# fhausmann/deepgrp

Measured on AMD Instinct MI355X. Metric: Mbp/sec predicted (whole node) at window=200 stride=50, 5-class, higher is better.
Workload: dtype f16

## Files before the change

deepgrp_amd/_lib.py:

```python
from __future__ import annotations

import ctypes as C
import os

_HERE = os.path.dirname(os.path.abspath(__file__))
LIB_PATH = os.path.join(_HERE, "libdeepgrp_hip.so")

i64, i32, vp, cint = C.c_int64, C.c_int32, C.c_void_p, C.c_int


class DgrpError(RuntimeError):
    """A libdeepgrp_hip call failed (message from dgrp_last_error())."""


class Segment(C.Structure):
    _fields_ = [("start", C.c_int64), ("end", C.c_int64), ("label", C.c_int32), ("contig", C.c_int32)]


class TrainJob(C.Structure):
    _fields_ = [("T", cint), ("u", cint), ("C", cint), ("attention", cint), ("d_params", vp), ("d_idx", vp), ("d_truth", vp),
                ("n", i64), ("d_starts", vp), ("B", i64), ("d_masks", vp), ("d_loss", vp), ("d_grads", vp), ("d_work", vp),
                ("work_bytes", i64)]


class InflateStreamStats(C.Structure):
    _fields_ = [(k, C.c_int64) for k in ("spans", "candidates", "repaired", "rounds", "longest_span", "false_starts", "chunks", "reserved")]

    def as_dict(self):
        return {k: int(getattr(self, k)) for k, _ in self._fields_ if k != "reserved"}


TRAIN_MAX_JOBS = 8

_SIGNATURES = {
    "dgrp_abi_version": (cint, []),
    "dgrp_last_error": (C.c_char_p, []),
    "dgrp_device_info": (cint, [C.c_char_p, C.c_size_t, C.POINTER(cint), C.POINTER(i64)]),
    "dgrp_strip_n": (cint, [vp, i64, C.POINTER(i64), C.POINTER(i64)]),
    "dgrp_encode": (cint, [vp, i64, vp, vp]),
    "dgrp_onehot": (cint, [vp, i64, vp, vp]),
    "dgrp_fasta_workspace_bytes": (i64, [i64]),
    "dgrp_fasta_encode": (cint, [vp, i64, vp, C.POINTER(i64), vp, i64, vp]),
    "dgrp_fasta_batch_workspace_bytes": (i64, [i64, i64]),
    "dgrp_fasta_encode_batch": (cint, [vp, i64, vp, vp, vp, vp, vp, i64, vp]),
    "dgrp_fasta_chunks_workspace_bytes": (i64, [i64]),
    "dgrp_fasta_chunks": (cint, [vp, i64, i64, vp, vp, C.POINTER(i64), vp, i64, vp]),
    "dgrp_fasta_mask_workspace_bytes": (i64, [i64, i64, i64]),
    "dgrp_fasta_mask_batch": (cint, [vp, i64, vp, vp, vp, vp, cint, C.c_uint64, vp, vp, i64, vp]),
    "dgrp_fasta_extract_workspace_bytes": (i64, [i64, i64, i64]),
    "dgrp_fasta_extract_batch": (cint, [vp, i64, vp, vp, vp, vp, vp, vp, i64, cint, C.c_uint64, vp, i64, C.POINTER(i64), vp, C.POINTER(i64),
                                        vp, i64, vp]),
    "dgrp_repeat_summary_workspace_bytes": (i64, [i64, i64, i64]),
    "dgrp_repeat_summary_batch": (cint, [vp, i64, vp, vp, vp, vp, cint, i64, vp, vp, vp, vp, vp, i64, vp]),
    "dgrp_twobit_workspace_bytes": (i64, [i64]),
    "dgrp_twobit_encode_batch": (cint, [vp, i64, i64, vp, vp, vp, vp, i64, vp, vp, i64, vp, i64, vp]),
    "dgrp_twobit_text_batch": (cint, [vp, i64, i64, vp, vp, vp, vp, vp, vp, i64, vp, vp, i64, vp, vp, i64, vp, i64, vp]),
    "dgrp_twobit_pack_workspace_bytes": (i64, [i64, i64]),
    "dgrp_twobit_pack_batch": (cint, [vp, i64, vp, vp, vp, i64, i64, vp, vp, vp, i64, vp]),
    "dgrp_format_rows_bound": (i64, [i64, i64]),
    "dgrp_format_rows": (cint, [vp, vp, i64, cint, vp, i64, vp, i64, C.POINTER(i64)]),
    "dgrp_track_workspace_bytes": (i64, [i64, i64]),
    "dgrp_track_text": (cint, [vp, i64, cint, cint, cint, i64, i64, C.c_char_p, i64, vp, i64, C.POINTER(i64), vp, i64, vp]),
    "dgrp_track_batch_workspace_bytes": (i64, [i64, vp, vp, i64, cint, i64]),
    "dgrp_track_text_batch": (cint, [vp, cint, i64, vp, vp, vp, C.c_char_p, vp, vp, cint, cint, i64, vp, i64, vp, vp, i64, vp]),
    "dgrp_track_index_workspace_bytes": (i64, [i64, vp, vp, i64, cint, i64]),
    "dgrp_track_index_batch": (cint, [vp, cint, i64, vp, vp, vp, C.c_char_p, vp, vp, cint, cint, i64, vp, i64, vp, vp, i64, vp, i64, vp]),
    "dgrp_track_sections_workspace_bytes": (i64, [i64, vp, vp, i64, cint]),
    "dgrp_track_sections_batch": (cint, [vp, cint, i64, vp, vp, vp, vp, cint, cint, i64, i64, vp, i64, vp, vp, i64, vp, vp, i64, vp]),
    "dgrp_track_zoom_workspace_bytes": (i64, [i64, vp, vp, i64, cint]),
    "dgrp_track_zoom_batch": (cint, [vp, cint, i64, vp, vp, vp, vp, cint, cint, i64, i64, vp, i64, vp, vp, i64, vp, vp, vp, i64, vp]),
    "dgrp_zlib_bound": (i64, [i64, i64]),
    "dgrp_zlib_workspace_bytes": (i64, [i64, cint]),
    "dgrp_zlib_compress_batch": (cint, [vp, i64, vp, i64, i64, cint, vp, i64, vp, C.POINTER(i64), vp, i64, vp]),
    "dgrp_zlib_compress_host": (cint, [vp, i64, vp, i64, i64, cint, vp, i64, vp, C.POINTER(i64)]),
    "dgrp_window_count":(i64, [i64, i64, i64]),
    "dgrp_windows_onehot": (cint, [vp, i64, i64, i64, i64, i64, cint, vp, vp]),
    "dgrp_model_create": (cint, [C.POINTER(vp), cint, cint, cint, cint, vp, vp, vp, vp, vp, vp]),
    "dgrp_model_create_lstm": (cint, [C.POINTER(vp), cint, cint, cint, vp, vp, vp, vp, vp]),
    "dgrp_model_destroy": (cint, [vp]),
    "dgrp_model_dims": (cint, [vp, C.POINTER(cint), C.POINTER(cint), C.POINTER(cint), C.POINTER(cint)]),
    "dgrp_model_flags": (cint, [vp]),
    "dgrp_model_set_precision": (cint, [vp, cint]),
    "dgrp_model_view": (cint, [vp, cint, C.POINTER(vp)]),
    "dgrp_model_plan": (cint, [vp, cint, i64, C.POINTER(cint), C.POINTER(i64), C.POINTER(cint), C.POINTER(cint)]),
    "dgrp_forward_workspace_bytes": (i64, [vp, i64]),
    "dgrp_forward_window_chunk": (i64, [vp]),
    "dgrp_forward_windows": (cint, [vp, vp, i64, i64, i64, i64, vp, vp, i64, vp]),
    "dgrp_forward_merge": (cint, [vp, vp, i64, i64, i64, i64, i64, vp, vp, i64, vp]),
    "dgrp_forward_merge_record": (cint, [vp, vp, i64, i64, i64, vp, vp, i64, vp]),
    "dgrp_forward_merge_record_workspace_bytes": (i64, [vp, i64, i64]),
    "dgrp_forward_reference_workspace_bytes": (i64, [vp, i64]),
    "dgrp_forward_windows_reference": (cint, [vp, vp, i64, i64, i64, i64, vp, vp, i64, vp]),
    "dgrp_get_max": (cint, [vp, i64, vp, i64, i64, i64, i64, vp]),
    "dgrp_scores": (cint, [vp, i64, cint, vp, vp, vp]),
    "dgrp_softmax_labels": (cint, [vp, i64, cint, vp, vp, vp, i64, vp]),
    "dgrp_mss_workspace_bytes": (i64, [i64]),
    "dgrp_mss_labels": (cint, [vp, vp, i64, cint, cint, cint, vp, vp, vp, i64, vp]),
    "dgrp_mss_segments_host": (cint, [vp, i64, vp, i64, C.POINTER(i64)]),
    "dgrp_mss_batch_workspace_bytes": (i64, [i64, i64]),
    "dgrp_mss_labels_batch": (cint, [vp, vp, i64, i64, vp, cint, cint, cint, vp, vp, i64, vp]),
    "dgrp_segments_workspace_bytes": (i64, [i64]),
    "dgrp_segments": (cint, [vp, i64, i64, i32, vp, i64, vp, vp, i64, vp]),
    "dgrp_record_workspace_bytes": (i64, [vp, i64, i64, cint]),
    "dgrp_predict_record": (cint, [vp, vp, i64, i64, i64, cint, cint, cint, i64, i32, vp, i64, C.POINTER(i64), vp, i64, vp]),
    "dgrp_batch_workspace_bytes": (i64, [vp, i64, vp, i64]),
    "dgrp_predict_batch": (cint, [vp, vp, i64, vp, vp, vp, vp, i64, i64, cint, cint, vp, i64, C.POINTER(i64), vp, i64, vp]),
    "dgrp_batch_rows": (i64, [i64, vp]),
    "dgrp_predict_batch_probs": (cint, [vp, vp, i64, vp, vp, vp, vp, i64, i64, cint, cint, vp, i64, C.POINTER(i64), vp, i64, vp, vp]),
    "dgrp_confusion_matrix": (cint, [vp, vp, i64, cint, vp, vp, vp]),
    "dgrp_filter_segments": (cint, [vp, vp, i64, i64, vp]),
    "dgrp_eval_workspace_bytes": (i64, [i64, i64]),
    "dgrp_paint_rows_batch": (cint, [vp, i64, vp, vp, vp, vp, vp, vp, i64, vp]),
    "dgrp_row_hits_batch": (cint, [vp, i64, vp, vp, vp, vp, vp, vp, vp, i64, vp]),
    "dgrp_row_scores_workspace_bytes": (i64, [i64, i64]),
    "dgrp_row_scores_batch": (cint, [vp, cint, i64, vp, vp, vp, vp, vp, vp, vp, i64, vp]),
    "dgrp_prob_hist_workspace_bytes": (i64, [i64, cint, cint]),
    "dgrp_prob_hist_batch": (cint, [vp, cint, i64, vp, vp, vp, vp, cint, vp, vp, vp, i64, vp]),
    "dgrp_row_detect_workspace_bytes": (i64, [i64, i64]),
    "dgrp_paint_row_keys_batch": (cint, [vp, i64, vp, vp, vp, vp, vp, vp, vp, i64, vp]),
    "dgrp_row_detect_batch": (cint, [vp, i64, vp, vp, vp, vp, vp, vp, vp, vp, i64, vp]),
    "dgrp_format_bed_bound": (i64, [i64, i64]),
    "dgrp_format_bed_rows": (cint, [vp, vp, i64, cint, vp, vp, i64, cint, vp, i64, C.POINTER(i64)]),
    "dgrp_bed_text_workspace_bytes": (i64, [i64, i64, i64]),
    "dgrp_bed_text_batch": (cint, [vp, vp, i64, cint, vp, vp, i64, cint, vp, i64, C.POINTER(i64), vp, i64, vp]),
    "dgrp_bed_index_workspace_bytes": (i64, [i64, i64, i64, i64]),
    "dgrp_bed_index_batch": (cint, [vp, vp, i64, cint, vp, vp, i64, cint, i64, vp, vp, i64, C.POINTER(i64), vp, i64, vp, vp, i64, vp]),
    "dgrp_gff_text_workspace_bytes": (i64, [i64, i64, i64, i64, i64]),
    "dgrp_gff_text_batch": (cint, [vp, vp, i64, cint, vp, vp, i64, vp, vp, i64, cint, i64, vp, i64, C.POINTER(i64), C.POINTER(i64), vp, i64,
                                   vp]),
    "dgrp_gff_index_workspace_bytes": (i64, [i64, i64, i64, i64, i64, i64]),
    "dgrp_gff_index_batch": (cint, [vp, vp, i64, cint, vp, vp, i64, vp, vp, i64, cint, i64, i64, vp, vp, i64, C.POINTER(i64), vp, i64, vp, vp,
                                    i64, vp]),
    "dgrp_bed_blocks_workspace_bytes": (i64, [i64, i64, vp]),
    "dgrp_bed_blocks_batch": (cint, [cint, vp, vp, i64, cint, i64, vp, i64, vp, i64, C.POINTER(i64), vp, i64, C.POINTER(i64), C.POINTER(i64),
                                     vp, i64, vp]),
    "dgrp_bed_zoom_workspace_bytes": (i64, [i64, i64, vp]),
    "dgrp_bed_zoom_batch": (cint, [cint, vp, vp, i64, cint, i64, vp, i64, vp, i64, vp, vp, i64, vp, vp, vp, i64, vp]),
    "dgrp_inflate_raw_host": (cint, [vp, i64, vp, i64, C.POINTER(i64), C.POINTER(i64), C.POINTER(cint)]),
    "dgrp_inflate_workspace_bytes": (i64, [i64]),
    "dgrp_inflate_batch": (cint, [vp, i64, i64, vp, vp, vp, vp, i64, C.POINTER(i64), C.POINTER(cint), vp, i64, vp]),
    "dgrp_inflate_stream_host": (cint, [vp, i64, i64, i64, cint, vp, i64, C.POINTER(i64), C.POINTER(i64), vp, C.POINTER(cint)]),
    "dgrp_inflate_stream_workspace_bytes": (i64, [i64, i64]),
    "dgrp_inflate_stream_scan": (cint, [vp, i64, i64, i64, i64, cint, C.POINTER(i64), vp, C.POINTER(cint), vp, i64, vp]),
    "dgrp_inflate_stream_write": (cint, [vp, i64, i64, i64, vp, vp, i64, C.POINTER(C.c_uint32), C.POINTER(i64), C.POINTER(cint), vp, i64,
                                         vp]),
    "dgrp_bgzf_bound": (i64, [i64, cint]),
    "dgrp_bgzf_workspace_bytes": (i64, [i64]),
    "dgrp_bgzf_compress": (cint, [vp, i64, vp, i64, C.POINTER(i64), cint, vp, i64, vp]),
    "dgrp_bgzf_compress_host": (cint, [vp, i64, vp, i64, C.POINTER(i64), cint]),
    "dgrp_bgzf_workspace_bytes_level": (i64, [i64, cint]),
    "dgrp_bgzf_compress_level": (cint, [vp, i64, vp, i64, C.POINTER(i64), cint, cint, vp, i64, vp]),
    "dgrp_bgzf_compress_host_level": (cint, [vp, i64, vp, i64, C.POINTER(i64), cint, cint]),
    "dgrp_train_param_count": (i64, [cint, cint, cint]),
    "dgrp_train_workspace_bytes": (i64, [cint, cint, cint, cint, i64]),
    "dgrp_train_step": (cint, [cint, cint, cint, cint, vp, vp, vp, i64, vp, i64, vp, vp, vp, vp, i64, vp]),
    "dgrp_train_step_multi": (cint, [C.POINTER(TrainJob), cint, vp]),
    "dgrp_optimizer_step": (cint, [cint, vp, vp, vp, vp, i64, C.c_double, C.c_double, C.c_double, C.c_double, i64, vp]),
    "dgrp_truth_workspace_bytes": (i64, [i64, i64]),
    "dgrp_truth_multihot_batch": (cint, [vp, cint, i64, i64, vp, vp, vp, vp, vp, vp, i64, vp]),
    "dgrp_class_starts_workspace_bytes": (i64, [i64, i64]),
    "dgrp_class_window_starts": (cint, [vp, i64, i64, vp, vp, cint, vp, i64, C.POINTER(i64), vp, i64, vp]),
    "dgrp_train_resolve_starts": (cint, [vp, i64, vp, vp, cint, vp, vp, i64, vp, vp]),
    "dgrp_rm_parse_workspace_bytes": (i64, [i64]),
    "dgrp_rm_parse": (cint, [vp, i64, vp, vp, cint, vp, cint, vp, vp, vp, vp, vp, vp, vp, i64, vp, vp, i64, vp]),
    "dgrp_rm_parse_fields": (cint, [vp, i64, vp, vp, cint, vp, cint, vp, vp, vp, vp, vp, vp, vp, vp, i64, vp, vp, i64, vp]),
    "dgrp_paint_strata_batch": (cint, [vp, i64, vp, vp, vp, vp, vp, vp, vp, i64, vp]),
    "dgrp_prob_hist_strata_workspace_bytes": (i64, [i64]),
    "dgrp_prob_hist_strata_batch": (cint, [vp, cint, i64, vp, vp, vp, vp, cint, cint, vp, vp, vp, i64, vp]),
    "dgrp_rm_parse_all_workspace_bytes": (i64, [i64]),
    "dgrp_rm_parse_all": (cint, [vp, i64, vp, vp, cint, vp, cint, vp, vp, vp, vp, vp, vp, vp, vp, vp, vp, vp, vp, i64, vp, vp, i64, vp]),
    "dgrp_rows_parse_workspace_bytes": (i64, [i64]),
    "dgrp_rows_parse": (cint, [vp, i64, cint, vp, vp, vp, vp, vp, vp, vp, vp, vp, i64, vp, vp, i64, vp]),
    "dgrp_token_ids_workspace_bytes": (i64, [i64, i64]),
    "dgrp_token_ids": (cint, [vp, i64, i64, vp, vp, vp, vp, vp, vp, i64, vp, vp, vp, i64, vp]),
    "dgrp_paint_keys_batch": (cint, [vp, i64, vp, vp, vp, vp, vp, vp, vp, i64, vp]),
    "dgrp_key_crosstab_batch": (cint, [vp, vp, i64, cint, i64, vp, vp, vp]),
    "dgrp_row_key_classes_batch": (cint, [vp, i64, vp, vp, vp, vp, vp, vp, vp, i64, vp]),
    "dgrp_row_bounds_workspace_bytes": (i64, [i64, i64]),
    "dgrp_row_bounds_batch": (cint, [vp, i64, vp, vp, vp, vp, vp, cint, vp, vp, i64, vp]),
    "dgrp_bound_hist_workspace_bytes": (i64, [i64]),
    "dgrp_bound_hist_batch": (cint, [i64, vp, vp, vp, vp, vp, vp, vp, cint, cint, vp, vp, vp, vp, vp, i64, vp]),
    "dgrp_kernel_timer_enable": (cint, [cint]),
    "dgrp_kernel_timer_read": (cint, [C.POINTER(C.c_double), C.POINTER(i64), C.POINTER(i64)]),
}

_lib = None


def lib() -> C.CDLL:
    global _lib
    if _lib is None:
        if not os.path.exists(LIB_PATH):
            raise ImportError(
                f"{LIB_PATH} is missing: build it with `make -C deepgrp_amd/csrc` (hipcc, gfx950) "
                "or `python -c 'import __graft_entry__ as g; g.build()'`. There is no CPU fallback.")
        import torch
        L = C.CDLL(LIB_PATH)
        for name, (res, args) in _SIGNATURES.items():
            f = getattr(L, name)
            f.restype = res
            f.argtypes = args
        if L.dgrp_abi_version() != 1:
            raise ImportError("libdeepgrp_hip.so ABI version mismatch")
        _lib = L
    return _lib


def check(rc: int, what: str = "") -> None:
    if rc != 0:
        msg = lib().dgrp_last_error().decode("utf-8", "replace")
        raise DgrpError(f"{what or 'libdeepgrp_hip'} failed (code {rc}): {msg}")


def name_blob(names):
    import numpy as np
    raw = [nm if isinstance(nm, bytes) else nm.encode("utf-8", "surrogateescape") for nm in names]
    off = np.zeros(len(raw) + 1, np.int64)
    np.cumsum([len(x) for x in raw], out=off[1:])
    return raw, b"".join(raw), off


def exported_symbols():
    return sorted(_SIGNATURES)
```

deepgrp_amd/csrc/api.hip:

```cpp
#include "dgrp_model.h"

#include <stdarg.h>
#include <string.h>

#include <algorithm>
#include <vector>
#include <mutex>

static thread_local char g_err[512] = "";

void dgrp_set_error(const char *fmt, ...)
{
    va_list ap;
    va_start(ap, fmt);
    vsnprintf(g_err, sizeof(g_err), fmt, ap);
    va_end(ap);
}

DGRP_EXPORT int dgrp_abi_version(void) { return DGRP_ABI_VERSION; }
DGRP_EXPORT const char *dgrp_last_error(void) { return g_err; }

DGRP_EXPORT int dgrp_device_info(char *name, size_t name_cap, int *cu_count, int64_t *hbm_bytes)
{
    int dev = 0;
// ... 504 lines not shown

DGRP_EXPORT int dgrp_model_destroy(dgrp_model *m)
{
    if (!m) return DGRP_OK;
    if (m->is_view) { delete m; return DGRP_OK; }
    if (m->d_pack) (void)hipFree(m->d_pack);
    if (m->d_ffb) (void)hipFree(m->d_ffb);
    if (m->d_scale) (void)hipFree(m->d_scale);
    if (m->d_wtop) (void)hipFree(m->d_wtop);
    if (m->d_raw) (void)hipFree(m->d_raw);
    if (m->d_pack_lo) (void)hipFree(m->d_pack_lo);
    if (m->d_pack16) (void)hipFree(m->d_pack16);
    if (m->d_xtab) (void)hipFree(m->d_xtab);
    if (m->d_stream) (void)hipFree(m->d_stream);
    if (m->d_packw) (void)hipFree(m->d_packw);
    if (m->d_xtabw) (void)hipFree(m->d_xtabw);
    delete m;
    return DGRP_OK;
}

DGRP_EXPORT int dgrp_model_dims(const dgrp_model *m, int *T, int *u, int *C, int *attention)
{
    DGRP_REQUIRE(m, "dgrp_model_dims: NULL model");
    if (T) *T = m->T;
    if (u) *u = m->u;
    if (C) *C = m->C;
    if (attention) *attention = m->attention;
    return DGRP_OK;
}

DGRP_EXPORT int dgrp_model_flags(const dgrp_model *m)
{
    DGRP_REQUIRE(m, "dgrp_model_flags: NULL model");
    return (m->onercp ? 1 : 0) | (m->precision == 1 ? 2 : 0) | (m->ref_only ? 4 : 0);
}

static_assert((int)dgrp_kernel::none == DGRP_KERNEL_NONE && (int)dgrp_kernel::wave == DGRP_KERNEL_WAVE &&
              (int)dgrp_kernel::split2 == DGRP_KERNEL_SPLIT2 && (int)dgrp_kernel::stream64 == DGRP_KERNEL_STREAM64 &&
              (int)dgrp_kernel::stream == DGRP_KERNEL_STREAM && (int)dgrp_kernel::split == DGRP_KERNEL_SPLIT &&
              (int)dgrp_kernel::lstm == DGRP_KERNEL_LSTM && (int)dgrp_kernel::fused == DGRP_KERNEL_FUSED,
              "DGRP_KERNEL_* (deepgrp_hip.h) follow dgrp_kernel (dgrp_model.h)");

DGRP_EXPORT int dgrp_model_plan(const dgrp_model *m, int mode, int64_t step, int *kernel, int64_t *lds_bytes, int *ospan, int *avg_up)
{
    DGRP_REQUIRE(m, "dgrp_model_plan: NULL model");
    DGRP_REQUIRE(kernel && lds_bytes && ospan && avg_up, "dgrp_model_plan: NULL output pointer");
    DGRP_REQUIRE(mode >= 0 && mode <= 2, "dgrp_model_plan: mode %d (0 merged, 1 window probabilities, 2 attention pre-pass)", mode);
    DGRP_REQUIRE(step >= 1, "dgrp_model_plan: step %lld < 1", (long long)step);
    DGRP_REQUIRE(mode != 2 || m->attention, "dgrp_model_plan: mode 2 on a model without attention");
    if (m->ref_only) {
        *kernel = DGRP_KERNEL_FP32; *lds_bytes = 0; *ospan = 0; *avg_up = 0;
        return DGRP_OK;
    }
    const dgrp_gru_plan plan = dgrp_gru_plan_for(m, mode, step);
    *kernel = (int)plan.kernel; *lds_bytes = (int64_t)plan.lds; *ospan = plan.ospan; *avg_up = plan.avg_up;
    return DGRP_OK;
}

DGRP_EXPORT int dgrp_model_set_precision(dgrp_model *m, int level)
{
    DGRP_REQUIRE(m, "dgrp_model_set_precision: NULL model");
    DGRP_REQUIRE(level == 0 || level == 1, "dgrp_model_set_precision: level must be 0 (fp16 operands) or 1 (split operands)");
    if (m->ref_only) return DGRP_OK;
    DGRP_REQUIRE(level == 0 || m->d_pack_lo || m->d_stream, "dgrp_model_set_precision: this model has no split-operand kernel");
    m->precision = level;
    return DGRP_OK;
}

static int64_t ref_sub_windows(const dgrp_model *m)
{
    const int64_t per = 2 * (int64_t)m->T * m->u * 4 + (int64_t)m->T * (m->C + 1) * 4 + 2 * (int64_t)m->u * 4;
    return std::max<int64_t>(16, std::min<int64_t>(4096, (512ll << 20) / per) / 16 * 16);
}

DGRP_EXPORT int64_t dgrp_forward_workspace_bytes(const dgrp_model *m, int64_t nw)
{
    if (!m || nw < 0) return 0;
    if (m->ref_only) {
        const int64_t sub = std::min<int64_t>(ref_sub_windows(m), std::max<int64_t>(nw, 1));
        return dgrp_align_up(dgrp_forward_reference_workspace_bytes(m, sub), 256) + dgrp_align_up(sub * m->T * (int64_t)m->C * 4, 256);
    }
    if (!m->attention) return 256;
    return dgrp_align_up(nw * m->T * (int64_t)m->UP * 4, 256) + dgrp_align_up(nw * m->T * (int64_t)m->C * 4, 256) + 256;
}

static unsigned *forward_queue(const dgrp_model *m, int64_t nw, void *d_work, int64_t work_bytes)
{
    if (!d_work || work_bytes < dgrp_forward_workspace_bytes(m, nw)) return nullptr;
    return (unsigned *)((char *)d_work + (m->attention ? dgrp_forward_workspace_bytes(m, nw) - 256 : 0));
}

static int forward_ref(const dgrp_model *m, const uint8_t *d_idx, int64_t n, int64_t s, dgrp_placement place, int64_t w0, int64_t nw,
                       int merge, float *d_out, void *d_work, int64_t work_bytes, hipStream_t stream)
{
    if (work_bytes < dgrp_forward_workspace_bytes(m, nw) || !d_work) {
        dgrp_set_error("dgrp_forward: this model runs on the fp32 kernels and needs %lld bytes of workspace for %lld windows",
                       (long long)dgrp_forward_workspace_bytes(m, nw), (long long)nw);
        return DGRP_ENOMEM;
    }
    const int64_t sub = std::min<int64_t>(ref_sub_windows(m), nw);
    const int64_t ref_bytes = dgrp_align_up(dgrp_forward_reference_workspace_bytes(m, sub), 256);
    float *probs = (float *)((char *)d_work + ref_bytes);
    for (int64_t a = w0; a < w0 + nw; a += sub) {
        const int64_t k = std::min<int64_t>(sub, w0 + nw - a);
        float *dst = merge ? probs : d_out + (a - w0) * (int64_t)m->T * m->C;
        int rc = dgrp_forward_windows_reference(m, d_idx, n, s, a, k, dst, d_work, ref_bytes, stream);
        if (rc) return rc;
        if (!merge) continue;
        for (int64_t b = a; b < a + k;) {
            const int64_t e = (b < place.nfullB && a + k > place.nfullB) ? place.nfullB : a + k;
            const int64_t row = dgrp_place_row(place, b, s);
            if (row < n) {
                rc = dgrp_get_max(d_out + row * m->C, n - row, probs + (b - a) * (int64_t)m->T * m->C, m->T, m->C, s, e - b, stream);
                if (rc) return rc;
            }
            b = e;
        }
    }
    return DGRP_OK;
}

static int forward_common(const dgrp_model *m, const uint8_t *d_idx, int64_t n, int64_t s, int64_t batch, int64_t w0,
                          int64_t nw, int merge, float *d_out, void *d_work, int64_t work_bytes, hipStream_t stream)
{
    DGRP_REQUIRE(m && s >= 1 && w0 >= 0 && nw >= 0 && n >= 0, "dgrp_forward: bad arguments");
    if (nw == 0) return DGRP_OK;
    DGRP_REQUIRE(d_idx && d_out, "dgrp_forward: NULL pointer");
    DGRP_REQUIRE((w0 + nw - 1) * s + m->T <= n, "dgrp_forward: window %lld (start %lld) runs past n=%lld",
                 (long long)(w0 + nw - 1), (long long)((w0 + nw - 1) * s), (long long)n);
    dgrp_placement place = { 0, 0 };
    if (merge) {
        DGRP_REQUIRE(batch >= 1, "dgrp_forward_merge: batch must be >= 1");
        const int64_t total = dgrp_window_count(n, m->T, s);
        DGRP_REQUIRE(w0 + nw <= total, "dgrp_forward_merge: windows %lld..%lld exceed the record's %lld",
                     (long long)w0, (long long)(w0 + nw), (long long)total);
        place = dgrp_make_placement(total, batch);
    }
    if (m->ref_only) return forward_ref(m, d_idx, n, s, place, w0, nw, merge, d_out, d_work, work_bytes, stream);
    if (!m->attention)
        return dgrp_gru_launch(m, dgrp_gru_plan_for(m, merge ? 0 : 1, s), d_idx, n, place, w0, nw, d_out, nullptr,
                               forward_queue(m, nw, d_work, work_bytes), stream);
    if (work_bytes < dgrp_forward_workspace_bytes(m, nw) || !d_work) {
        dgrp_set_error("dgrp_forward: attention model needs %lld bytes of workspace for %lld windows",
                       (long long)dgrp_forward_workspace_bytes(m, nw), (long long)nw);
        return DGRP_ENOMEM;
    }
    void *avg = d_work;
    float *pl = (float *)((char *)d_work + dgrp_align_up(nw * m->T * (int64_t)m->UP * 4, 256));
    const dgrp_gru_plan pre = dgrp_gru_plan_for(m, 2, s);
    int rc = dgrp_gru_launch(m, pre, d_idx, n, place, w0, nw, pl, avg, forward_queue(m, nw, d_work, work_bytes), stream);
    if (rc) return rc;
    return dgrp_attention_launch_recs(m, pre, place, w0, nw, merge, n, avg, pl, d_out, nullptr, 0, stream);
}

DGRP_EXPORT int dgrp_forward_windows(const dgrp_model *m, const uint8_t *d_idx, int64_t n, int64_t s, int64_t w0,
                                     int64_t nw, float *d_probs, void *d_work, int64_t work_bytes, void *stream)
{
    return forward_common(m, d_idx, n, s, 1, w0, nw, 0, d_probs, d_work, work_bytes, (hipStream_t)stream);
}

DGRP_EXPORT int dgrp_forward_merge(const dgrp_model *m, const uint8_t *d_idx, int64_t n, int64_t s, int64_t batch,
                                   int64_t w0, int64_t nw, float *d_out, void *d_work, int64_t work_bytes, void *stream)
{
    return forward_common(m, d_idx, n, s, batch, w0, nw, 1, d_out, d_work, work_bytes, (hipStream_t)stream);
}

static int64_t spill_cap_bytes()
{
    static const int64_t cap = [] {
        if (const char *e = getenv("DGRP_SPILL_BYTES")) {
            const long long v = atoll(e);
            if (v >= (1ll << 20)) return (int64_t)v;
        }
        size_t free_b = 0, total_b = 0;
        if (hipMemGetInfo(&free_b, &total_b) != hipSuccess || total_b == 0) return (int64_t)(4ll << 30);
        return std::min<int64_t>(8ll << 30, std::max<int64_t>(1ll << 30, (int64_t)(total_b / 32)));
    }();
    return cap;
}

static int64_t record_window_chunk(const dgrp_model *m)
{
    if (m->ref_only) return ref_sub_windows(m);
    if (!m->attention) return 1ll << 23;
    const int64_t per = (int64_t)m->T * ((int64_t)m->UP * 4 + (int64_t)m->C * 4);
    int64_t c = spill_cap_bytes() / per;
    c = c >= 32768 ? c / 32768 * 32768 : c >= 4096 ? c / 4096 * 4096 : c / 16 * 16;
    if (c < 16) c = 16;
    return c < (1ll << 20) ? c : (1ll << 20);
}

DGRP_EXPORT int64_t dgrp_forward_window_chunk(const dgrp_model *m)
{
    return m ? record_window_chunk(m) : 0;
}

#define DGRP_LANES 3
static int64_t lane_window_chunk(const dgrp_model *m)
{
    if (m->ref_only || !m->attention) return 0;
    if (const char *e = getenv("DGRP_LANE_CHUNK")) {
        const long long v = atoll(e);
        return v >= 16 ? (int64_t)(v / 16 * 16) : 0;
    }
    const int64_t c = record_window_chunk(m);
    if (c < 65536) return 0;
    const int64_t lc = c / DGRP_LANES / 32768 * 32768;
    return lc >= 32768 ? lc : 32768;
}
struct lane_pool { hipStream_t s[DGRP_LANES]; int dev; bool ok; };
static lane_pool *lanes_get()
{
    static std::mutex mu;
    static std::vector<lane_pool *> pools;
    int dev = 0;
    if (hipGetDevice(&dev) != hipSuccess) return nullptr;
    std::lock_guard<std::mutex> lock(mu);
    for (lane_pool *q : pools)
        if (q->dev == dev) return q->ok ? q : nullptr;
    lane_pool *q = new lane_pool();
    q->dev = dev; q->ok = true;
    for (int i = 0; i < DGRP_LANES; ++i)
        if (hipStreamCreateWithFlags(&q->s[i], hipStreamNonBlocking) != hipSuccess) q->ok = false;
    pools.push_back(q);
    return q->ok ? q : nullptr;
}

static int64_t record_forward_bytes(const dgrp_model *m, int64_t nwin)
{
    const int64_t lc = lane_window_chunk(m);
    if (lc > 0 && nwin > lc)
        return DGRP_LANES * dgrp_align_up(std::max<int64_t>(dgrp_forward_workspace_bytes(m, std::min(lc, nwin)), 256), 256);
    const int64_t chunk = std::min<int64_t>(record_window_chunk(m), nwin > 0 ? nwin : 1);
    return std::max<int64_t>(dgrp_forward_workspace_bytes(m, chunk), 256);
}

DGRP_EXPORT int64_t dgrp_forward_merge_record_workspace_bytes(const dgrp_model *m, int64_t n, int64_t s)
{
    if (!m || n < 0 || s < 1) return 0;
    return record_forward_bytes(m, dgrp_window_count(n, m->T, s));
}

DGRP_EXPORT int dgrp_forward_merge_record(const dgrp_model *m, const uint8_t *d_idx, int64_t n, int64_t s, int64_t batch, float *d_out,
                                          void *d_work, int64_t work_bytes, void *stream_)
{
    hipStream_t stream = (hipStream_t)stream_;
    DGRP_REQUIRE(m && n >= 0 && s >= 1 && batch >= 1, "dgrp_forward_merge_record: bad arguments");
    const int64_t nwin = dgrp_window_count(n, m->T, s);
    if (nwin == 0) return DGRP_OK;
    DGRP_REQUIRE(d_idx && d_out && d_work, "dgrp_forward_merge_record: NULL pointer");
    const int64_t need = record_forward_bytes(m, nwin);
    if (work_bytes < need) {
        dgrp_set_error("dgrp_forward_merge_record: workspace %lld < %lld bytes", (long long)work_bytes, (long long)need);
        return DGRP_ENOMEM;
    }
    const int64_t lc = lane_window_chunk(m);
    lane_pool *lp = lc > 0 && nwin > lc ? lanes_get() : nullptr;
    if (!lp) {
        const int64_t chunk = lc > 0 && nwin > lc ? lc : record_window_chunk(m);
        for (int64_t w0 = 0; w0 < nwin; w0 += chunk) {
            const int64_t nw = std::min<int64_t>(chunk, nwin - w0);
            const int rc = dgrp_forward_merge(m, d_idx, n, s, batch, w0, nw, d_out, d_work, work_bytes, stream);
            if (rc) return rc;
        }
        return DGRP_OK;
    }
    const int64_t per = need / DGRP_LANES;
    hipEvent_t fork = nullptr, join[DGRP_LANES] = { nullptr, nullptr, nullptr };
    int rc = DGRP_OK;
    auto bail = [&](hipError_t e) { if (e != hipSuccess && rc == DGRP_OK) { dgrp_set_error("dgrp_forward_merge_record: %s", hipGetErrorString(e)); rc = DGRP_EHIP; } };
    bail(hipEventCreateWithFlags(&fork, hipEventDisableTiming));
    for (int i = 0; i < DGRP_LANES; ++i) bail(hipEventCreateWithFlags(&join[i], hipEventDisableTiming));
    if (rc == DGRP_OK) {
        bail(hipEventRecord(fork, stream));
        for (int i = 0; i < DGRP_LANES; ++i) bail(hipStreamWaitEvent(lp->s[i], fork, 0));
        int64_t k = 0;
        for (int64_t w0 = 0; w0 < nwin && rc == DGRP_OK; w0 += lc, ++k) {
            const int64_t nw = std::min<int64_t>(lc, nwin - w0);
            const int lane = (int)(k % DGRP_LANES);
            rc = dgrp_forward_merge(m, d_idx, n, s, batch, w0, nw, d_out, (char *)d_work + lane * per, per, lp->s[lane]);
        }
        for (int i = 0; i < DGRP_LANES; ++i) {
            bail(hipEventRecord(join[i], lp->s[i]));
            bail(hipStreamWaitEvent(stream, join[i], 0));
        }
    }
    if (fork) (void)hipEventDestroy(fork);
    for (int i = 0; i < DGRP_LANES; ++i)
        if (join[i]) (void)hipEventDestroy(join[i]);
    return rc;
}

struct record_layout {
    int64_t out, scores, cls, labels, count, fwd, post, bytes, post_bytes, fwd_bytes;
};

static record_layout record_carve(const dgrp_model *m, int64_t n, int64_t s, int use_mss)
{
    record_layout l;
    int64_t p = 0;
    auto take = [&](int64_t b) { const int64_t q = p; p += dgrp_align_up(b, 256); return q; };
    const int64_t nwin = dgrp_window_count(n, m->T, s);
    l.out = take(n * m->C * 4);
    l.scores = take(use_mss ? n * 8 : 0);
    l.cls = take(use_mss ? n : 0);
    l.labels = take(n);
    l.count = take(8);
    l.fwd_bytes = record_forward_bytes(m, nwin);
    l.fwd = take(l.fwd_bytes);
    l.post_bytes = std::max<int64_t>(std::max<int64_t>(use_mss ? dgrp_mss_workspace_bytes(n) : 4096, dgrp_segments_workspace_bytes(n)), 4096);
    l.post = take(l.post_bytes);
    l.bytes = p;
    return l;
}

DGRP_EXPORT int64_t dgrp_record_workspace_bytes(const dgrp_model *m, int64_t n, int64_t s, int use_mss)
{
    if (!m || n < 0 || s < 1) return 0;
    return record_carve(m, n, s, use_mss).bytes;
}

DGRP_EXPORT int dgrp_predict_record(const dgrp_model *m, const uint8_t *d_idx, int64_t n, int64_t s, int64_t batch,
                                    int min_mss_len, int xdrop_len, int use_mss, int64_t offset, int32_t contig,
                                    dgrp_segment *d_records, int64_t cap, int64_t *h_count, void *d_work,
                                    int64_t work_bytes, void *stream_)
{
    hipStream_t stream = (hipStream_t)stream_;
    DGRP_REQUIRE(m && n >= 0 && s >= 1 && batch >= 1 && cap >= 0 && h_count, "dgrp_predict_record: bad arguments");
    *h_count = 0;
    if (n == 0) return DGRP_OK;
    DGRP_REQUIRE(d_idx && d_work && (cap == 0 || d_records), "dgrp_predict_record: NULL pointer");
    const record_layout l = record_carve(m, n, s, use_mss);
    if (work_bytes < l.bytes) {
        dgrp_set_error("dgrp_predict_record: workspace %lld < %lld bytes", (long long)work_bytes, (long long)l.bytes);
        return DGRP_ENOMEM;
    }
    char *w = (char *)d_work;
    float *out = (float *)(w + l.out);
    int8_t *labels = (int8_t *)(w + l.labels);
    int64_t *d_count = (int64_t *)(w + l.count);
    DGRP_HIP(hipMemsetAsync(out, 0, (size_t)n * m->C * 4, stream));
    int rc = dgrp_forward_merge_record(m, d_idx, n, s, batch, out, w + l.fwd, l.fwd_bytes, stream);
    if (rc) return rc;
    if (use_mss) {
        rc = dgrp_scores(out, n, m->C, (double *)(w + l.scores), (int8_t *)(w + l.cls), stream);
        if (rc) return rc;
        rc = dgrp_mss_labels((const double *)(w + l.scores), (const int8_t *)(w + l.cls), n, m->C, min_mss_len, xdrop_len,
                             labels, nullptr, w + l.post, l.post_bytes, stream);
    } else {
        rc = dgrp_softmax_labels(out, n, m->C, nullptr, labels, w + l.post, l.post_bytes, stream);
    }
    if (rc) return rc;
    rc = dgrp_segments(labels, n, offset, contig, d_records, cap, d_count, w + l.post, l.post_bytes, stream);
    if (rc) return rc;
    DGRP_HIP(hipMemcpyAsync(h_count, d_count, 8, hipMemcpyDeviceToHost, stream));
    DGRP_HIP(hipStreamSynchronize(stream));
    return DGRP_OK;
}

int dgrp_batch_marks(const int64_t *d_start, const int64_t *d_len, int64_t nrec, int64_t total_n, uint8_t *d_marks,
                     double *d_scores, int8_t *d_cls, hipStream_t stream);
int dgrp_batch_segments(const int8_t *d_labels, const uint8_t *d_marks, int64_t total_n, const int64_t *d_start, int64_t nrec,
                        const int64_t *d_startpos, const int32_t *d_contig, dgrp_segment *d_records, int64_t cap,
                        int64_t *d_count, void *d_work, int64_t work_bytes, hipStream_t stream);

struct batch_layout {
    int64_t out, scores, cls, labels, marks, count, recs, wgf, start, len, spos, contig, post, post_bytes, avg, pl, queue, bytes;
};

static batch_layout batch_carve(const dgrp_model *m, int64_t nrec, int64_t total_rows, int64_t total_windows)
{
    batch_layout l;
    int64_t p = 0;
    auto take = [&](int64_t b) { const int64_t q = p; p += dgrp_align_up(b, 256); return q; };
    l.out = take(total_rows * m->C * 4);
    l.scores = take(total_rows * 8);
    l.cls = take(total_rows);
    l.labels = take(total_rows);
    l.marks = take(total_rows);
    l.count = take(8);
    l.recs = take(nrec * 64);
    l.wgf = take((nrec + 1) * 8);
    l.start = take((nrec + 1) * 8);
    l.len = take(nrec * 8);
    l.spos = take(nrec * 8);
    l.contig = take(nrec * 4);
    l.post_bytes = std::max<int64_t>(std::max<int64_t>(dgrp_mss_batch_workspace_bytes(total_rows, nrec), dgrp_segments_workspace_bytes(total_rows)), 4096);
    l.post = take(l.post_bytes);
    l.avg = take(m->attention ? total_windows * m->T * (int64_t)m->UP * 4 : 0);
    l.pl = take(m->attention ? total_windows * m->T * (int64_t)m->C * 4 : 0);
    l.queue = take(4);
    l.bytes = p;
    return l;
}

static int64_t batch_windows(const dgrp_model *m, int64_t nrec, const int64_t *h_n, int64_t s)
{
    int64_t w = 0;
    for (int64_t r = 0; r < nrec; ++r) w += dgrp_window_count(h_n[r], m->T, s);
    return w;
}

static int64_t batch_rows(int64_t nrec, const int64_t *h_n)
{
    int64_t rows = 0;
    for (int64_t r = 0; r < nrec; ++r) rows += dgrp_align_up(h_n[r], 64);
    return rows;
}

DGRP_EXPORT int64_t dgrp_batch_workspace_bytes(const dgrp_model *m, int64_t nrec, const int64_t *h_n, int64_t s)
{
    if (!m || nrec < 0 || s < 1 || (nrec > 0 && !h_n)) return 0;
    for (int64_t r = 0; r < nrec; ++r)
        if (h_n[r] < 1) return 0;
    return batch_carve(m, nrec, batch_rows(nrec, h_n), batch_windows(m, nrec, h_n, s)).bytes;
}

DGRP_EXPORT int64_t dgrp_batch_rows(int64_t nrec, const int64_t *h_n)
{
    return nrec > 0 && h_n ? batch_rows(nrec, h_n) : 0;
}

static int predict_batch_common(const char *who, const dgrp_model *m, const uint8_t *d_idx, int64_t nrec, const int64_t *h_idx_off,
                                const int64_t *h_n, const int64_t *h_startpos, const int32_t *h_contig, int64_t s,
                                int64_t batch, int min_mss_len, int xdrop_len, dgrp_segment *d_records, int64_t cap,
                                int64_t *h_count, void *d_work, int64_t work_bytes, hipStream_t stream, float *d_probs)
{
    DGRP_REQUIRE(m && nrec >= 0 && s >= 1 && batch >= 1 && cap >= 0 && h_count, "%s: bad arguments", who);
    *h_count = 0;
    if (nrec == 0) return DGRP_OK;
    DGRP_REQUIRE(!m->ref_only && (m->cell == 0 || (m->cell == 1 && m->NW <= 8)), "%s: unsupported model (fp32 path: record by record)", who);
    DGRP_REQUIRE(d_idx && h_idx_off && h_n && h_startpos && h_contig && d_work && (cap == 0 || d_records), "%s: NULL pointer", who);
    for (int64_t r = 0; r < nrec; ++r)
        DGRP_REQUIRE(h_n[r] >= 1 && h_idx_off[r] >= 0, "%s: record %lld: empty records do not belong in a batch", who, (long long)r);
    const int64_t rows = batch_rows(nrec, h_n);
    DGRP_REQUIRE(rows < (1ll << 31), "%s: %lld rows in one batch (limit 2^31)", who, (long long)rows);
    const int64_t windows = batch_windows(m, nrec, h_n, s);
    DGRP_REQUIRE(windows < (1ll << 31), "%s: too many windows in one batch", who);
    const batch_layout l = batch_carve(m, nrec, rows, windows);
    if (work_bytes < l.bytes) {
        dgrp_set_error("%s: workspace %lld < %lld bytes", who, (long long)work_bytes, (long long)l.bytes);
        return DGRP_ENOMEM;
    }
    char *w = (char *)d_work;
    std::vector<int64_t> recs((size_t)nrec * 8, 0), wgf((size_t)nrec + 1, 0), start((size_t)nrec + 1, 0);
    int64_t wfirst = 0;
    for (int64_t r = 0; r < nrec; ++r) {
        const int64_t nwin = dgrp_window_count(h_n[r], m->T, s);
        const dgrp_placement pl = dgrp_make_placement(nwin, batch);
        int64_t *e = recs.data() + (size_t)r * 8;
        e[0] = h_idx_off[r]; e[1] = h_n[r]; e[2] = start[(size_t)r]; e[3] = nwin; e[4] = pl.nfullB; e[5] = pl.shift; e[6] = wfirst;
        wfirst += nwin;
        wgf[(size_t)r + 1] = wgf[(size_t)r] + (nwin + 15) / 16;
        start[(size_t)r + 1] = start[(size_t)r] + dgrp_align_up(h_n[r], 64);
    }
    DGRP_HIP(hipMemcpyAsync(w + l.recs, recs.data(), recs.size() * 8, hipMemcpyHostToDevice, stream));
    DGRP_HIP(hipMemcpyAsync(w + l.wgf, wgf.data(), wgf.size() * 8, hipMemcpyHostToDevice, stream));
    DGRP_HIP(hipMemcpyAsync(w + l.start, start.data(), start.size() * 8, hipMemcpyHostToDevice, stream));
    DGRP_HIP(hipMemcpyAsync(w + l.len, h_n, (size_t)nrec * 8, hipMemcpyHostToDevice, stream));
    DGRP_HIP(hipMemcpyAsync(w + l.spos, h_startpos, (size_t)nrec * 8, hipMemcpyHostToDevice, stream));
    DGRP_HIP(hipMemcpyAsync(w + l.contig, h_contig, (size_t)nrec * 4, hipMemcpyHostToDevice, stream));
    float *out = d_probs ? d_probs : (float *)(w + l.out);
    DGRP_HIP(hipMemsetAsync(out, 0, (size_t)rows * m->C * 4, stream));
    int rc;
    if (!m->attention) {
        rc = dgrp_gru_launch_batch(m, dgrp_gru_plan_for(m, 0, s), d_idx, w + l.recs, (const int64_t *)(w + l.wgf), nrec, wgf[(size_t)nrec],
                                   out, nullptr, (unsigned *)(w + l.queue), stream);
        if (rc) return rc;
    } else {
        const dgrp_gru_plan pre = dgrp_gru_plan_for(m, 2, s);
        rc = dgrp_gru_launch_batch(m, pre, d_idx, w + l.recs, (const int64_t *)(w + l.wgf), nrec, wgf[(size_t)nrec], (float *)(w + l.pl),
                                   w + l.avg, (unsigned *)(w + l.queue), stream);
        if (rc) return rc;
        rc = dgrp_attention_launch_recs(m, pre, dgrp_placement{ 0, 0 }, 0, windows, 1, rows, w + l.avg, (const float *)(w + l.pl), out,
                                        w + l.recs, nrec, stream);
        if (rc) return rc;
    }
    double *scores = (double *)(w + l.scores);
    int8_t *cls = (int8_t *)(w + l.cls), *labels = (int8_t *)(w + l.labels);
    uint8_t *marks = (uint8_t *)(w + l.marks);
    rc = dgrp_scores(out, rows, m->C, scores, cls, stream);
    if (rc) return rc;
    rc = dgrp_batch_marks((const int64_t *)(w + l.start), (const int64_t *)(w + l.len), nrec, rows, marks, scores, cls, stream);
    if (rc) return rc;
    rc = dgrp_mss_labels_batch(scores, cls, rows, nrec, start.data(), m->C, min_mss_len, xdrop_len, labels, w + l.post, l.post_bytes, stream);
    if (rc) return rc;
    int64_t *d_count = (int64_t *)(w + l.count);
    rc = dgrp_batch_segments(labels, marks, rows, (const int64_t *)(w + l.start), nrec, (const int64_t *)(w + l.spos),
                             (const int32_t *)(w + l.contig), d_records, cap, d_count, w + l.post, l.post_bytes, stream);
    if (rc) return rc;
    DGRP_HIP(hipMemcpyAsync(h_count, d_count, 8, hipMemcpyDeviceToHost, stream));
    DGRP_HIP(hipStreamSynchronize(stream));
    return DGRP_OK;
}

DGRP_EXPORT int dgrp_predict_batch(const dgrp_model *m, const uint8_t *d_idx, int64_t nrec, const int64_t *h_idx_off,
                                   const int64_t *h_n, const int64_t *h_startpos, const int32_t *h_contig, int64_t s,
                                   int64_t batch, int min_mss_len, int xdrop_len, dgrp_segment *d_records, int64_t cap,
                                   int64_t *h_count, void *d_work, int64_t work_bytes, void *stream)
{
    return predict_batch_common("dgrp_predict_batch", m, d_idx, nrec, h_idx_off, h_n, h_startpos, h_contig, s, batch, min_mss_len, xdrop_len,
                                d_records, cap, h_count, d_work, work_bytes, (hipStream_t)stream, nullptr);
}

DGRP_EXPORT int dgrp_predict_batch_probs(const dgrp_model *m, const uint8_t *d_idx, int64_t nrec, const int64_t *h_idx_off,
                                         const int64_t *h_n, const int64_t *h_startpos, const int32_t *h_contig, int64_t s,
                                         int64_t batch, int min_mss_len, int xdrop_len, dgrp_segment *d_records, int64_t cap,
                                         int64_t *h_count, void *d_work, int64_t work_bytes, void *stream, float *d_probs)
{
    DGRP_REQUIRE(d_probs || nrec <= 0, "dgrp_predict_batch_probs: NULL d_probs");
    return predict_batch_common("dgrp_predict_batch_probs", m, d_idx, nrec, h_idx_off, h_n, h_startpos, h_contig, s, batch, min_mss_len,
                                xdrop_len, d_records, cap, h_count, d_work, work_bytes, (hipStream_t)stream, d_probs);
}
```

deepgrp_amd/csrc/mss_kernels.hip:

```cpp
#include "dgrp_common.h"
#include "scan.h"
#include <vector>
#include <math.h>

struct mss_cand { int32_t st, en; double L, R; int32_t pre, pad; };

#define MSS_SUB_MIN 256
#define MSS_SUBENT_BYTES 80
struct mss_subent {
    int64_t start, run;
    double L, peak, run_L;
    int64_t run_st;
    int32_t open, first;
    int32_t vci, nst;
    int32_t reset, pad;
    double Lf;
};
static_assert(sizeof(mss_subent) == 80, "MSS_SUBENT_BYTES");
#define MSS_LCAP 160
#define MSS_NEG (-1e30)
#define MSS_QNONE (-4096)
#define MSS_QBAD 4096

enum mss_grand {
    MSS_G_TOTAL = 0,
    MSS_G_CHANGED = 1,
    MSS_G_ERROR = 2,
    MSS_G_NSEG = 3,
    MSS_G_WHY = 4,
    MSS_G_PIECES = 5,
    MSS_G_LUNITS = 6,
    MSS_G_SPEC = 7,
    MSS_G_NLONG = MSS_G_TOTAL
};

struct mss_stats {
    const double *blk_sum, *blk_abs; const int32_t *blk_q; const uint8_t *flags;
    const double *sup_sum, *sup_abs; const int32_t *sup_q; const uint8_t *sup_flags;
};

struct mss_layout {
    int64_t nblk;
    uint64_t *blk;
    double *blk_sum;
    double *blk_abs;
    int32_t *blk_q;
    uint8_t *flags;
    int64_t nsup;
    double *sup_sum, *sup_abs;
    int32_t *sup_q;
    uint8_t *sup_flags;
    uint64_t *tiles;
    uint64_t *grand;
    int64_t *ustart;
    int64_t *urun;
    double *exitL[2];
    uint64_t *segcnt;
    uint64_t *cutcnt;
    uint64_t *lblk;
    int64_t *lstart, *lrun;
    uint8_t *lforced;
    void *lstate[2];
    int64_t *cut_st, *cut_run;
    double *cut_L;
    int2 *cut_kj;
    int64_t *ustart2, *urun2;
    double *entry2;
    void *subs;
    int64_t dump_cap;
    mss_cand *dump;
    mss_cand *stack;
    int32_t *segs;
    int32_t *segs_out;
    int64_t bytes;
};

static mss_layout mss_carve(void *work, int64_t n)
{
    mss_layout l;
    unsigned char *p = (unsigned char *)work;
    auto take = [&](int64_t bytes) { unsigned char *q = p; p += dgrp_align_up(bytes, 256); return q; };
    l.nblk = (n + 63) / 64;
    const int64_t maxunits = l.nblk + 1, maxruns = n / 2 + 2;
    l.blk = (uint64_t *)take((l.nblk + 1) * 8);
    l.blk_sum = (double *)take(l.nblk * 8);
    l.blk_abs = (double *)take(l.nblk * 8);
    l.blk_q = (int32_t *)take(l.nblk * 4);
    l.flags = (uint8_t *)take(l.nblk + 64);
    l.nsup = (l.nblk + 63) / 64;
    l.sup_sum = (double *)take(l.nsup * 8);
    l.sup_abs = (double *)take(l.nsup * 8);
    l.sup_q = (int32_t *)take(l.nsup * 4);
    l.sup_flags = (uint8_t *)take(l.nsup + 64);
    l.tiles = (uint64_t *)take(((maxunits + 1 + SCAN_TILE - 1) / SCAN_TILE + 1) * 8);
    l.grand = (uint64_t *)take(64);
    l.ustart = (int64_t *)take((maxunits + 1) * 8);
    l.urun = (int64_t *)take((maxunits + 1) * 8);
    l.exitL[0] = (double *)take(maxunits * 8);
    l.exitL[1] = (double *)take(maxunits * 8);
    l.segcnt = (uint64_t *)take((maxunits + 1) * 8);
    l.cutcnt = (uint64_t *)take((maxunits + 1) * 8);
    l.lblk = (uint64_t *)take((l.nblk + 1) * 8);
    l.lstart = (int64_t *)take((maxunits + 1) * 8);
    l.lrun = (int64_t *)take((maxunits + 1) * 8);
    l.lforced = (uint8_t *)take(maxunits + 64);
    l.lstate[0] = take(maxunits * 64);
    l.lstate[1] = take(maxunits * 64);
    l.cut_st = (int64_t *)take(l.nblk * 8);
    l.cut_run = (int64_t *)take(l.nblk * 8);
    l.cut_L = (double *)take(l.nblk * 8);
    l.cut_kj = (int2 *)take(l.nblk * 8);
    l.ustart2 = (int64_t *)take((2 * maxunits + 2) * 8);
    l.urun2 = (int64_t *)take((2 * maxunits + 2) * 8);
    l.entry2 = (double *)take((2 * maxunits + 2) * 8);
    l.subs = take((maxunits + 8) * (int64_t)MSS_SUBENT_BYTES);
    l.dump_cap = 2 * (l.nblk / MSS_SUB_MIN + 2);
    l.dump = (mss_cand *)take(l.dump_cap * MSS_LCAP * (int64_t)sizeof(mss_cand));
    l.stack = (mss_cand *)take(maxruns * (int64_t)sizeof(mss_cand));
    l.segs = (int32_t *)take(maxruns * 8);
    l.segs_out = (int32_t *)take(maxruns * 8);
    l.bytes = p - (unsigned char *)work;
    return l;
}

DGRP_EXPORT int64_t dgrp_mss_workspace_bytes(int64_t n)
{
    if (n < 0) return 0;
    return mss_carve(nullptr, n).bytes;
}

__device__ __forceinline__ int quantum_exp(double x)
{
    const uint64_t b = (uint64_t)__double_as_longlong(x) & 0x7fffffffffffffffull;
    if (b == 0) return MSS_QNONE;
    const int e = (int)(b >> 52);
    if (e == 0 || e == 0x7ff) return MSS_QBAD;
    const uint64_t m = b & 0x000fffffffffffffull;
    const int tz = m ? __builtin_ctzll(m) : 52;
    return -((e - 1023) - 52 + tz);
}

__device__ __forceinline__ bool mss_certified(double L, double sumabs, int q_scores)
{
    const int qL = quantum_exp(L);
    const int Q = qL > q_scores ? qL : q_scores;
    if (Q >= MSS_QBAD) return false;
    const int ex = 53 - Q;
    if (ex > 1000) return true;
    if (ex < -1000) return false;
    return (fabs(L) + sumabs) * 1.0000001 < ldexp(1.0, ex);
}

__device__ __forceinline__ double wave_sum(double v)
{
#pragma unroll
    for (int o = 32; o > 0; o >>= 1) v += __shfl_xor(v, o);
    return v;
}
__device__ __forceinline__ int wave_max(int v)
{
#pragma unroll
    for (int o = 32; o > 0; o >>= 1) { int w = __shfl_xor(v, o); v = w > v ? w : v; }
    return v;
}

__device__ __forceinline__ double lane_value(double x, int l)
{
    const long long b = __double_as_longlong(x);
    const int lo = __builtin_amdgcn_readlane((int)b, l), hi = __builtin_amdgcn_readlane((int)(b >> 32), l);
    return __longlong_as_double(((long long)hi << 32) | (unsigned int)lo);
}

__global__ void __launch_bounds__(256) mss_blockstat_kernel(const double *__restrict__ S, int64_t n,
                                                            uint64_t *__restrict__ blk, double *__restrict__ blk_sum,
                                                            double *__restrict__ blk_abs, int32_t *__restrict__ blk_q,
                                                            uint8_t *__restrict__ flags)
{
    const int lane = threadIdx.x & 63;
    const int64_t b = (int64_t)blockIdx.x * 4 + (threadIdx.x >> 6);
    if (b * 64 >= n) return;
    const int64_t i = b * 64 + lane;
    const double s = i < n ? S[i] : 0.0;
    const bool pos = i < n && s > 0;
    const bool prevpos = i > 0 && i < n && S[i - 1] > 0;
    const unsigned long long mpos = __ballot(pos);
    const unsigned long long mstart = __ballot(pos && !prevpos);
    const double sum = wave_sum(s), sabs = wave_sum(fabs(s));
    const int q = wave_max(quantum_exp(s));
    if (lane == 0) {
        flags[b] = (uint8_t)(mpos != 0ull ? 1 : 0);
        blk[b] = (uint64_t)__popcll(mstart);
        blk_sum[b] = sum;
        blk_abs[b] = sabs;
        blk_q[b] = q;
    }
}

__global__ void __launch_bounds__(256) mss_superstat_kernel(const double *__restrict__ blk_sum, const double *__restrict__ blk_abs,
                                                            const int32_t *__restrict__ blk_q, const uint8_t *__restrict__ flags,
                                                            int64_t nblk, double *__restrict__ sup_sum, double *__restrict__ sup_abs,
                                                            int32_t *__restrict__ sup_q, uint8_t *__restrict__ sup_flags)
{
    const int lane = threadIdx.x & 63;
    const int64_t g = (int64_t)blockIdx.x * 4 + (threadIdx.x >> 6);
    if (g * 64 >= nblk) return;
    const int64_t b = g * 64 + lane;
    const bool in = b < nblk;
    const unsigned long long mp = __ballot(in && (flags[b] & 1));
    const double sum = wave_sum(in ? blk_sum[b] : 0.0), sabs = wave_sum(in ? blk_abs[b] : 0.0);
    const int q = wave_max(in ? blk_q[b] : MSS_QNONE);
    if (lane == 0) {
        sup_flags[g] = (uint8_t)(mp != 0ull ? 1 : 0);
        sup_sum[g] = sum;
        sup_abs[g] = sabs;
        sup_q[g] = q;
    }
}

__device__ __forceinline__ bool mss_is_boundary(const uint8_t *flags, const double *blk_sum, int64_t b, int64_t nblk,
                                                int64_t n, double thr)
{
    if (!(thr > 0.0) || b + 1 >= nblk || (flags[b] & 1) || !(flags[b + 1] & 1)) return false;
    if (b * 64 + 64 > n) return false;
    double cum = 0.0;
    for (int64_t j = b; j >= 0 && j > b - 16; --j) {
        if (flags[j] & 1) break;
        cum += blk_sum[j];
        if (cum < -thr) return true;
    }
    return false;
}

__global__ void __launch_bounds__(256) mss_boundary_kernel(const uint8_t *__restrict__ flags, const double *__restrict__ blk_sum,
                                                           int64_t nblk, int64_t n, double thr, uint64_t *__restrict__ blk)
{
    const int64_t b = (int64_t)blockIdx.x * blockDim.x + threadIdx.x;
    if (b >= nblk) return;
    if (mss_is_boundary(flags, blk_sum, b, nblk, n, thr)) blk[b] |= 1ull << 32;
}

__global__ void __launch_bounds__(256) mss_units_kernel(const uint64_t *__restrict__ blk, const uint8_t *__restrict__ flags,
                                                        const double *__restrict__ blk_sum, int64_t nblk, int64_t n, double thr,
                                                        int64_t *__restrict__ ustart, int64_t *__restrict__ urun,
                                                        const uint64_t *__restrict__ grand)
{
    const int64_t b = (int64_t)blockIdx.x * blockDim.x + threadIdx.x;
    if (b == 0) {
        ustart[0] = 0;
        urun[0] = 0;
        const int64_t nunits = (int64_t)(grand[MSS_G_TOTAL] >> 32) + 1;
        ustart[nunits] = n;
        urun[nunits] = (int64_t)(grand[MSS_G_TOTAL] & 0xffffffffull);
    }
    if (b >= nblk) return;
    if (mss_is_boundary(flags, blk_sum, b, nblk, n, thr)) {
        const int64_t k = (int64_t)(blk[b] >> 32) + 1;
        ustart[k] = (b + 1) * 64;
        urun[k] = (int64_t)(blk[b] & 0xffffffffull);
    }
}

template <int CTRL, int RMASK>
__device__ __forceinline__ int dpp_i(int src, int old) { return __builtin_amdgcn_update_dpp(old, src, CTRL, RMASK, 0xf, false); }
template <int CTRL, int RMASK>
__device__ __forceinline__ double dpp_d(double src, double old)
{
    const long long s = __double_as_longlong(src), o = __double_as_longlong(old);
    const int lo = __builtin_amdgcn_update_dpp((int)o, (int)s, CTRL, RMASK, 0xf, false);
    const int hi = __builtin_amdgcn_update_dpp((int)(o >> 32), (int)(s >> 32), CTRL, RMASK, 0xf, false);
    return __longlong_as_double(((long long)hi << 32) | (unsigned int)lo);
}
#define DPP_SHR(n) (0x110 + (n))
#define DPP_BCAST15 0x142
#define DPP_BCAST31 0x143
#define DPP_WAVE_SHR1 0x138
#define DPP_SCAN_STEPS(STEP) STEP(DPP_SHR(1), 0xf) STEP(DPP_SHR(2), 0xf) STEP(DPP_SHR(4), 0xf) STEP(DPP_SHR(8), 0xf) STEP(DPP_BCAST15, 0xa) STEP(DPP_BCAST31, 0xc)
__device__ __forceinline__ double scan_add_d(double x)
{
#define STEP(c, m) x = x + dpp_d<c, m>(x, 0.0);
    DPP_SCAN_STEPS(STEP)
#undef STEP
    return x;
}
__device__ __forceinline__ double scan_min_d(double x)
{
#define STEP(c, m) { const double y = dpp_d<c, m>(x, INFINITY); x = y < x ? y : x; }
    DPP_SCAN_STEPS(STEP)
#undef STEP
    return x;
}
__device__ __forceinline__ int scan_max_i(int x)
{
#define STEP(c, m) { const int y = dpp_i<c, m>(x, -1); x = y > x ? y : x; }
    DPP_SCAN_STEPS(STEP)
#undef STEP
    return x;
}
__device__ __forceinline__ void scan_segmax_d(int &fl, double &v)
{
#define STEP(c, m) { const double yv = dpp_d<c, m>(v, -INFINITY); const int yf = dpp_i<c, m>(fl, 0); if (!fl) v = yv > v ? yv : v; fl |= yf; }
    DPP_SCAN_STEPS(STEP)
#undef STEP
}
__device__ __forceinline__ double lane_below_d(double x, double first) { return dpp_d<DPP_WAVE_SHR1, 0xf>(x, first); }
__device__ __forceinline__ int lane_below_i(int x, int first) { return dpp_i<DPP_WAVE_SHR1, 0xf>(x, first); }
__device__ __forceinline__ int lane_value_i(int x, int l) { return __builtin_amdgcn_readlane(x, l); }

__device__ __forceinline__ double mss_fold(double s, double a0, int t, int nvalid, int lane)
{
    const double sm = lane >= t && lane < nvalid ? s : 0.0;
    double X = a0;
    for (int j = t; j < nvalid; j += 4) {
        X = lane_below_d(X, a0) + sm;
        X = lane_below_d(X, a0) + sm;
        X = lane_below_d(X, a0) + sm;
        X = lane_below_d(X, a0) + sm;
    }
    return X;
}

__device__ __forceinline__ int64_t mss_skip_blocks(const mss_stats &st, double &cur, int64_t pos, int64_t end, int lane)
{
    if ((pos & 4095) == 0) {
        const int64_t gj = (pos >> 12) + lane;
        const bool stop2 = gj * 4096 + 4096 > end || (st.sup_flags[gj] & 1);
        const unsigned long long ms2 = __ballot(stop2);
        const int m2 = ms2 ? __builtin_ctzll(ms2) : 64;
        if (m2 > 0) {
            const bool in = lane < m2;
            const double gs = wave_sum(in ? st.sup_sum[gj] : 0.0);
            const double ga = wave_sum(in ? st.sup_abs[gj] : 0.0);
            const int gq = wave_max(in ? st.sup_q[gj] : MSS_QNONE);
            if (mss_certified(cur, ga, gq)) { cur += gs; return (int64_t)m2 * 4096; }
        }
    }
    const int64_t b0 = pos >> 6, bend = (end + 63) >> 6;
    const int64_t bj = b0 + lane;
    const bool stop = bj >= bend || (st.flags[bj] & 1) || (bj * 64 + 64 > end) || (lane > 0 && (bj & 63) == 0);
    const unsigned long long mstop = __ballot(stop);
    const int m = mstop ? __builtin_ctzll(mstop) : 64;
    if (m > 0) {
        const bool in = lane < m;
        const double gs = wave_sum(in ? st.blk_sum[bj] : 0.0);
        const double ga = wave_sum(in ? st.blk_abs[bj] : 0.0);
        const int gq = wave_max(in ? st.blk_q[bj] : MSS_QNONE);
        if (mss_certified(cur, ga, gq)) { cur += gs; return (int64_t)m * 64; }
    }
    return 0;
}

__global__ void __launch_bounds__(64) mss_scan_kernel(const double *__restrict__ S, const int64_t *__restrict__ ustart,
                                                      const int64_t *__restrict__ urun, int64_t nunits,
                                                      const double *__restrict__ exit_prev, double *__restrict__ exit_cur,
                                                      mss_cand *stack_all, int32_t *__restrict__ segs_all,
                                                      uint64_t *__restrict__ segcnt, int min_sc, double xdrop,
                                                      uint64_t *__restrict__ grand, int pass,
                                                      const double *__restrict__ blk_sum, const double *__restrict__ blk_abs,
                                                      const int32_t *__restrict__ blk_q, const uint8_t *__restrict__ flags,
                                                      const double *__restrict__ sup_sum, const double *__restrict__ sup_abs,
                                                      const int32_t *__restrict__ sup_q, const uint8_t *__restrict__ sup_flags,
                                                      int independent, int cutmode, mss_subent *subs, mss_cand *dump_all)
{
    const mss_stats stats = { blk_sum, blk_abs, blk_q, flags, sup_sum, sup_abs, sup_q, sup_flags };
    __shared__ double2 sLR[MSS_LCAP];
    __shared__ int4 sIdx[MSS_LCAP];
    const int lane = threadIdx.x;
    const int64_t k = blockIdx.x;
    const bool sub = subs != nullptr;
    const bool head = !sub || subs[k].first != 0;
    const bool tail = !sub || k + 1 == nunits || subs[k + 1].first != 0;
    const int64_t begin = sub ? subs[k].start : ustart[k], end = sub ? subs[k + 1].start : ustart[k + 1];
    const int64_t slot0 = sub ? subs[k].run : urun[k];
    volatile mss_cand *ovf = stack_all + slot0;
    int32_t *segs = segs_all + 2 * slot0;
    int64_t nst = 0, nseg = 0;
    double cur = sub ? subs[k].L : (k == 0 || independent) ? 0.0 : exit_prev[k - 1];
    double peak = sub && !head ? subs[k].peak : MSS_NEG;
    bool run_open = sub && !head && subs[k].open != 0;
    int64_t run_st = run_open ? subs[k].run_st : 0;
    double run_L = run_open ? subs[k].run_L : 0.0;
    bool was_reset = false;
    double Lf = sub && !head ? subs[k].Lf : INFINITY;

    struct cand_v { double L, R; int32_t st, en, pre, open; };
    auto get = [&](int64_t j) -> cand_v {
        cand_v c;
        if (j < MSS_LCAP) {
            const double2 lr = sLR[j];
            const int4 ix = sIdx[j];
            c.L = lr.x; c.R = lr.y; c.st = ix.x; c.en = ix.y; c.pre = ix.z; c.open = ix.w;
        } else {
            volatile mss_cand *o = ovf + (j - MSS_LCAP);
            c.L = o->L; c.R = o->R; c.st = o->st; c.en = o->en; c.pre = o->pre; c.open = o->pad;
        }
        return c;
    };

    auto flush = [&]() {
        for (int64_t base = 0; base < nst; base += 64) {
            const int64_t j = base + lane;
            bool keep = false;
            int32_t a = 0, b = 0;
            if (j < nst) {
                const cand_v c = get(j);
                keep = c.R - c.L >= min_sc;
                a = c.st;
                b = c.en;
            }
            const unsigned long long m = __ballot(keep);
            if (keep) {
                const int64_t slot = nseg + __popcll(m & ((1ull << lane) - 1ull));
                segs[2 * slot] = a;
                segs[2 * slot + 1] = b;
            }
            nseg += __popcll(m);
        }
        nst = 0;
    };

    auto close_run = [&](double R, int64_t en) {
        if (R > peak) peak = R;
        if (!head && run_L <= Lf) { Lf = run_L; peak = R; }
        int32_t tst = (int32_t)run_st;
        double tL = run_L;
        int64_t j;
        for (;;) {
            j = nst - 1;
            cand_v c;
            while (j >= 0) {
                c = get(j);
                if (c.L < tL) break;
                j = c.pre >= 0 ? c.pre : j - 1;
            }
            if (j >= 0 && c.R < R) {
                tst = c.st;
                tL = c.L;
                nst = j;
                continue;
            }
            break;
        }
        const int lopen = j < 0 && !head ? 1 : 0;
        if (j < 0 && head) { flush(); peak = R; }
        if (was_reset && lane == 0) { atomicOr((unsigned long long *)&grand[MSS_G_ERROR], 1ull); atomicOr((unsigned long long *)&grand[MSS_G_WHY], 8ull); }
        if (nst < MSS_LCAP) {
            if (lane == 0) {
                sLR[nst] = make_double2(tL, R);
                sIdx[nst] = make_int4(tst, (int32_t)en, (int32_t)j, lopen);
            }
        } else {
            volatile mss_cand *c = ovf + (nst - MSS_LCAP);
            c->st = tst; c->en = (int32_t)en; c->L = tL; c->R = R; c->pre = (int32_t)j; c->pad = lopen;
        }
        __threadfence_block();
        ++nst;
        run_open = false;
    };
    auto reset_flush = [&]() {
        if (head) flush(); else { was_reset = true; Lf = INFINITY; }
    };

    int64_t pos = begin;
    while (pos < end) {
        const int nvalid = (int)min((int64_t)64, end - pos);
        if (!run_open && peak == MSS_NEG && (pos & 63) == 0) {
            const int64_t adv = mss_skip_blocks(stats, cur, pos, end, lane);
            if (adv) { pos += adv; continue; }
        }
        const double s = lane < nvalid ? S[pos + lane] : 0.0;
        const bool ispos = lane < nvalid && s > 0;
        const unsigned long long vmask = nvalid == 64 ? ~0ull : ((1ull << nvalid) - 1ull);
        const unsigned long long mpos = __ballot(ispos);
        const double sabs = wave_sum(fabs(s));
        const int q = wave_max(quantum_exp(s));
        const bool cert = mss_certified(cur, sabs, q);
        if (cert || (q < MSS_QBAD && quantum_exp(cur) < MSS_QBAD)) {
            double pre = s;
            if (cert) {
#pragma unroll
                for (int o = 1; o < 64; o <<= 1) {
                    const double y = __shfl_up(pre, o);
                    if (lane >= o) pre += y;
                }
            } else {
                pre = mss_fold(s, cur, 0, nvalid, lane);
            }
            double base = cert ? cur : 0.0;
            const double front = cur;
            int p = 0;
            if (nst >= 1 && nst <= MSS_LCAP) {
                const cand_v c0 = get(nst - 1);
                const int64_t nb = c0.pre;
                const bool lone = nst == 1 && !c0.open;
                double lim = INFINITY;
                if (!lone && nb >= 0) lim = get(nb).R;
                if (lone || nb >= 0 || c0.open) {
                const double V = base + pre;
                const bool edge_close = run_open && !(mpos & 1ull);
                const bool isend = ispos && lane + 1 < nvalid && !((mpos >> (lane + 1)) & 1ull);
                const bool isstart = ispos && (lane == 0 ? !run_open : !((mpos >> (lane - 1)) & 1ull));
                double vprev = __shfl_up(V, 1);
                if (lane == 0) vprev = cur;
                double rmax = isend ? V : -INFINITY;
#pragma unroll
                for (int o = 1; o < 64; o <<= 1) {
                    const double y = __shfl_up(rmax, o);
                    if (lane >= o) rmax = y > rmax ? y : rmax;
                }
                double before = __shfl_up(rmax, 1);
                if (lane == 0) before = -INFINITY;
                const double base_r = edge_close ? cur : c0.R;
                const double base_peak = edge_close ? (lone ? cur : (cur > peak ? cur : peak)) : peak;
                const double top_r = before > base_r ? before : base_r;
                const double peak_i = lone ? (before > -INFINITY ? before : base_peak) : (before > base_peak ? before : base_peak);
                bool ok = !run_open || c0.L < run_L;
                if (edge_close) ok = ok && cur > c0.R && !(lim < cur);
                if (isend) ok = ok && V > top_r && !(lim < V);
                if (isstart) ok = ok && (c0.L < vprev);
                if (lane < nvalid && !ispos && xdrop > 0.0 && V + xdrop < peak_i) ok = false;
                if (__all(ok)) {
                    const unsigned long long mend = __ballot(isend);
                    if (mend || edge_close) {
                        const int last = mend ? 63 - __builtin_clzll(mend) : -1;
                        const double newR = mend ? lane_value(V, last) : cur;
                        if (lane == 0) {
                            sLR[nst - 1] = make_double2(c0.L, newR);
                            sIdx[nst - 1] = make_int4(c0.st, (int32_t)(pos + last + 1), (int32_t)nb, c0.open);
                        }
                        __threadfence_block();
                        peak = lone ? newR : (newR > peak ? newR : peak);
                    }
                    if ((mpos >> (nvalid - 1)) & 1ull) {
                        const unsigned long long znon = ~mpos & vmask;
                        if (znon || !run_open) {
                            const int ls = znon ? 64 - __builtin_clzll(znon) : 0;
                            run_st = pos + ls;
                            run_L = ls == 0 ? cur : lane_value(V, ls - 1);
                        }
                        run_open = true;
                    } else {
                        run_open = false;
                    }
                    cur = lane_value(V, nvalid - 1);
                    pos += nvalid;
                    continue;
                }
                }
            }
            while (p < nvalid) {
                const unsigned long long rest = vmask & ~((1ull << p) - 1ull);
                if ((mpos >> p) & 1ull) {
                    const unsigned long long z = ~mpos & rest;
                    const int e = z ? __builtin_ctzll(z) : nvalid;
                    if (!run_open) { run_open = true; run_st = pos + p; run_L = p == 0 ? front : base + lane_value(pre, p - 1); }
                    cur = base + lane_value(pre, e - 1);
                    p = e;
                    if (e < nvalid) close_run(cur, pos + e);
                } else {
                    if (run_open) close_run(cur, pos + p);
                    const unsigned long long z = mpos & rest;
                    const int e = z ? __builtin_ctzll(z) : nvalid;
                    if (xdrop > 0.0 && peak != MSS_NEG) {
                        const bool trig = lane >= p && lane < e && ((base + pre) + xdrop < peak);
                        const unsigned long long mt = __ballot(trig);
                        if (mt) {
                            const int t = __builtin_ctzll(mt);
                            reset_flush();
                            peak = MSS_NEG;
                            if (cert) base = t == 0 ? 0.0 : -lane_value(pre, t - 1);
                            else pre = mss_fold(s, 0.0, t, nvalid, lane);
                        }
                    }
                    cur = base + lane_value(pre, e - 1);
                    p = e;
                }
            }
        } else {
            for (int i = 0; i < nvalid; ++i) {
                const double v = lane_value(s, i);
                if (v > 0) {
                    if (!run_open) { run_open = true; run_st = pos + i; run_L = cur; }
                    cur = cur + v;
                } else {
                    if (run_open) close_run(cur, pos + i);
                    if (xdrop > 0.0 && cur + v + xdrop < peak) { reset_flush(); cur = 0.0; peak = MSS_NEG; }
                    cur += v;
                }
            }
        }
        pos += nvalid;
    }
    if (run_open && tail) close_run(cur, end);
    if (sub && !(head && tail)) {
        const int64_t slot = head ? 2 * (int64_t)subs[k + 1].vci + 1 : 2 * (int64_t)subs[k].vci;
        mss_cand *d = dump_all + slot * MSS_LCAP;
        for (int64_t j = lane; j < nst && j < MSS_LCAP; j += 64) {
            const double2 lr = sLR[j];
            const int4 ix = sIdx[j];
            mss_cand c;
            c.st = ix.x; c.en = ix.y; c.L = lr.x; c.R = lr.y; c.pre = ix.z; c.pad = ix.w;
            d[j] = c;
        }
        if (lane == 0) {
            subs[k].nst = (int32_t)(nst < (1ll << 31) ? nst : -1);
            subs[k].reset = was_reset ? 1 : 0;
        }
    } else if (k == nunits - 1 || independent || cutmode) {
        flush();
    } else if (nst != 0 || peak != MSS_NEG) {
        if (lane == 0) atomicOr((unsigned long long *)&grand[MSS_G_ERROR], 1ull);
    }
    if (lane == 0) {
        segcnt[k] = (uint64_t)nseg;
        const double want = sub ? subs[k + 1].L : exit_prev[k];
        if (!independent && (pass == 0 || __double_as_longlong(want) != __double_as_longlong(cur)))
            atomicOr((unsigned long long *)&grand[MSS_G_CHANGED], 1ull);
        exit_cur[k] = cur;
    }
}

__global__ void __launch_bounds__(64) mss_stitch_kernel(mss_subent *subs, int64_t nunits, mss_cand *stack_all, const mss_cand *dump_all,
                                                        int32_t *__restrict__ segs_all, uint64_t *__restrict__ segcnt, int min_sc,
                                                        uint64_t *__restrict__ grand)
{
    const int lane = threadIdx.x;
    const int64_t k = blockIdx.x;
    if (!subs[k].first || k + 1 >= nunits || subs[k + 1].first) return;
    __shared__ mss_cand loc[256];
    volatile mss_cand *T = stack_all + subs[k].run;
    int64_t nT = subs[k].nst;
    bool bad = nT < 0;
    if (!bad) {
        for (int64_t hi = nT; hi > MSS_LCAP; hi -= 64) {
            const int64_t j = hi - 1 - lane;
            mss_cand c;
            const bool on = j >= MSS_LCAP;
            if (on) { volatile mss_cand *o = T + (j - MSS_LCAP); c.st = o->st; c.en = o->en; c.L = o->L; c.R = o->R; c.pre = o->pre; c.pad = 0; }
            __threadfence_block();
            if (on) { volatile mss_cand *o = T + j; o->st = c.st; o->en = c.en; o->L = c.L; o->R = c.R; o->pre = c.pre; o->pad = 0; }
            __threadfence_block();
        }
        const mss_cand *d = dump_all + (2 * (int64_t)subs[k + 1].vci + 1) * MSS_LCAP;
        for (int64_t j = lane; j < nT && j < MSS_LCAP; j += 64) {
            const mss_cand c = d[j];
            volatile mss_cand *o = T + j; o->st = c.st; o->en = c.en; o->L = c.L; o->R = c.R; o->pre = c.pre; o->pad = 0;
        }
        __threadfence();
    }
    int64_t nseg = (int64_t)segcnt[k];
    int32_t *segs = segs_all + 2 * subs[k].run;
    auto flush_T = [&]() {
        for (int64_t base = 0; base < nT; base += 64) {
            const int64_t j = base + lane;
            bool keep = false;
            int32_t a = 0, b = 0;
            if (j < nT) {
                volatile mss_cand *c = T + j;
                keep = c->R - c->L >= min_sc;
                a = c->st;
                b = c->en;
            }
            const unsigned long long m = __ballot(keep);
            if (keep) {
                const int64_t slot = nseg + __popcll(m & ((1ull << lane) - 1ull));
                segs[2 * slot] = a;
                segs[2 * slot + 1] = b;
            }
            nseg += __popcll(m);
        }
        nT = 0;
    };
    for (int64_t u = k + 1; !bad && u < nunits && !subs[u].first; ++u) {
        const int64_t nl = subs[u].nst;
        if (nl < 0) { bad = true; break; }
        const mss_cand *d = dump_all + 2 * (int64_t)subs[u].vci * MSS_LCAP;
        const mss_cand *deep = stack_all + subs[u].run;
        if (nl > MSS_LCAP && subs[k].run + nT > subs[u].run) { bad = true; break; }
        int64_t w = 0;
        auto load_chunk = [&]() {
            const int64_t j = w + lane;
            if (j < nl) loc[j & 255] = j < MSS_LCAP ? d[j] : deep[j - MSS_LCAP];
            w += 64;
        };
        __syncthreads();
        while (w < nl && w < 256) load_chunk();
        __syncthreads();
        int64_t delta = 0;
        for (int64_t i = 0; i < nl && !bad; ++i) {
            if (w < nl && i + 192 >= w) {
                if (subs[k].run + nT > subs[u].run + w - MSS_LCAP) { bad = true; break; }
                __syncthreads();
                load_chunk();
                __syncthreads();
            }
            const mss_cand e = loc[i & 255];
            int32_t tst = e.st, pre;
            double tL = e.L;
            if (e.pad) {
                int64_t j;
                for (;;) {
                    j = nT - 1;
                    double cL = 0.0, cR = 0.0;
                    int32_t cst = 0;
                    while (j >= 0) {
                        volatile mss_cand *c = T + j;
                        cL = c->L;
                        if (cL < tL) { cR = c->R; cst = c->st; break; }
                        const int32_t pr = c->pre;
                        j = pr >= 0 ? pr : j - 1;
                    }
                    if (j >= 0 && cR < e.R) { tst = cst; tL = cL; nT = j; continue; }
                    break;
                }
                if (j < 0 && nT > 0) flush_T();
                pre = (int32_t)j;
                delta = nT - i;
            } else {
                if (i == 0 || e.pre < 0) { bad = true; if (lane == 0) atomicOr((unsigned long long *)&grand[MSS_G_WHY], 4ull); break; }
                pre = (int32_t)(e.pre + delta);
            }
            volatile mss_cand *o = T + nT;
            o->st = tst; o->en = e.en; o->L = tL; o->R = e.R; o->pre = pre; o->pad = 0;
            __threadfence();
            ++nT;
        }
    }
    if (bad) {
        if (lane == 0) atomicOr((unsigned long long *)&grand[MSS_G_ERROR], 1ull);
        return;
    }
    flush_T();
    if (lane == 0) segcnt[k] = (uint64_t)nseg;
}

#define MSS_LIGHT_SUB 2048
struct mss_light_state {
    double L, peak, Lf, run_L;
    int64_t run_st, run_slot;
    int64_t last_blk, open;
};

__global__ void __launch_bounds__(256) mss_lightflag_kernel(const uint8_t *__restrict__ flags, const double *__restrict__ blk_sum,
                                                            int64_t nblk, int64_t n, double thr, int sub, int use_forced,
                                                            uint64_t *__restrict__ lblk)
{
    const int64_t b = (int64_t)blockIdx.x * blockDim.x + threadIdx.x;
    if (b >= nblk) return;
    const bool forced = use_forced && mss_is_boundary(flags, blk_sum, b, nblk, n, thr);
    const bool spec = ((b + 1) % sub) == 0 && (b + 1) * 64 < n;
    lblk[b] = forced || spec ? 1 : 0;
}

__global__ void __launch_bounds__(256) mss_lightunits_kernel(const uint64_t *__restrict__ lblk, const uint64_t *__restrict__ lcount,
                                                             const uint8_t *__restrict__ flags, const double *__restrict__ blk_sum,
                                                             const uint64_t *__restrict__ runs_before, const uint64_t *__restrict__ runs_total,
                                                             int64_t nblk, int64_t n, double thr, int sub, int use_forced,
                                                             int64_t *__restrict__ lstart, int64_t *__restrict__ lrun,
                                                             uint8_t *__restrict__ lforced)
{
    const int64_t b = (int64_t)blockIdx.x * blockDim.x + threadIdx.x;
    if (b == 0) {
        lstart[0] = 0; lrun[0] = 0; lforced[0] = 1;
        const int64_t nl = (int64_t)*lcount + 1;
        lstart[nl] = n; lrun[nl] = (int64_t)(*runs_total & 0xffffffffull); lforced[nl] = 1;
    }
    if (b >= nblk) return;
    const bool forced = use_forced && mss_is_boundary(flags, blk_sum, b, nblk, n, thr);
    const bool spec = ((b + 1) % sub) == 0 && (b + 1) * 64 < n;
    if (forced || spec) {
        const int64_t j = (int64_t)lblk[b] + 1;
        lstart[j] = (b + 1) * 64;
        lrun[j] = (int64_t)((b + 1 < nblk ? runs_before[b + 1] : *runs_total) & 0xffffffffull);
        lforced[j] = forced ? 1 : 0;
    }
}

__global__ void __launch_bounds__(64) mss_light_kernel(const double *__restrict__ S, const int64_t *__restrict__ ustart,
                                                       const int64_t *__restrict__ urun, const uint8_t *__restrict__ uforced,
                                                       int64_t nunits, const mss_light_state *__restrict__ st_prev,
                                                       mss_light_state *__restrict__ st_cur,
                                                       double xdrop, uint64_t *__restrict__ grand, int pass,
                                                       const double *__restrict__ blk_sum, const double *__restrict__ blk_abs,
                                                       const int32_t *__restrict__ blk_q, const uint8_t *__restrict__ flags,
                                                       const double *__restrict__ sup_sum, const double *__restrict__ sup_abs,
                                                       const int32_t *__restrict__ sup_q, const uint8_t *__restrict__ sup_flags,
                                                       uint64_t *__restrict__ cut_cnt, int64_t *__restrict__ cut_st,
                                                       int64_t *__restrict__ cut_run, double *__restrict__ cut_L,
                                                       int2 *__restrict__ cut_kj)
{
    const int lane = threadIdx.x;
    const int64_t k = blockIdx.x;
    const int64_t begin = ustart[k], end = ustart[k + 1];
    const int64_t slot0 = urun[k];
    const bool forced = uforced[k] != 0;
    const mss_stats stats = { blk_sum, blk_abs, blk_q, flags, sup_sum, sup_abs, sup_q, sup_flags };
    double cur = 0.0, peak = MSS_NEG, Lf = INFINITY, run_L = 0.0;
    bool run_open = false;
    int64_t run_st = 0, run_slot = 0;
    int64_t last_blk = begin >> 6;
    if (k > 0 && pass > 0) {
        const mss_light_state e = st_prev[k - 1];
        cur = e.L; peak = e.peak; Lf = e.Lf; run_L = e.run_L;
        run_st = e.run_st; run_slot = e.run_slot; run_open = e.open != 0;
        if (!forced) last_blk = e.last_blk;
    }
    int64_t nruns = 0;
    int64_t ncut = forced ? 1 : 0;
    auto file_cut = [&](int64_t st, int64_t slot, double Ls) {
        if (lane == 0) {
            const int64_t b = st >> 6;
            cut_st[b] = st; cut_run[b] = slot; cut_L[b] = Ls; cut_kj[b] = make_int2((int)k, (int)ncut);
        }
    };

    auto close_scalar = [&](double Ls, double R, int64_t st, int64_t slot) {
        if (R > peak) peak = R;
        if (Ls <= Lf) {
            Lf = Ls;
            peak = R;
            if ((st >> 6) != last_blk) {
                file_cut(st, slot, Ls);
                ++ncut;
                last_blk = st >> 6;
            }
        }
    };

    int64_t pos = begin;
    int64_t pf_pos = -1;
    double pf_s = 0.0, pf_abs = 0.0;
    int pf_q = 0;
    while (pos < end) {
        const int nvalid = (int)min((int64_t)(64 - (pos & 63)), end - pos);
        if (!run_open && peak == MSS_NEG && (pos & 63) == 0) {
            const int64_t adv = mss_skip_blocks(stats, cur, pos, end, lane);
            if (adv) { pos += adv; continue; }
        }
        const bool whole = nvalid == 64;
        double s, sabs;
        int q;
        if (pf_pos == pos) { s = pf_s; sabs = pf_abs; q = pf_q; }
        else {
            s = lane < nvalid ? S[pos + lane] : 0.0;
            if (whole) { sabs = blk_abs[pos >> 6]; q = blk_q[pos >> 6]; }
        }
        {
            const int64_t np = pos + nvalid;
            pf_pos = np;
            pf_s = np + lane < end ? S[np + lane] : 0.0;
            if (np + 64 <= end) { pf_abs = blk_abs[np >> 6]; pf_q = blk_q[np >> 6]; }
        }
        const bool ispos = lane < nvalid && s > 0;
        const unsigned long long mpos = __ballot(ispos);
        if (!whole) {
            sabs = lane_value(scan_add_d(fabs(s)), 63);
            q = lane_value_i(scan_max_i(quantum_exp(s) + 8192), 63) - 8192;
        }
        const bool cert = mss_certified(cur, sabs, q);
        if (cert || (q < MSS_QBAD && quantum_exp(cur) < MSS_QBAD)) {
            const double pre = cert ? scan_add_d(s) : 0.0;
            double base = cur;
            double V = cert ? base + pre : mss_fold(s, cur, 0, nvalid, lane);
            int p0 = 0;
            for (;;) {
                const bool act = lane >= p0 && lane < nvalid;
                const double Vb = lane_below_d(V, base);
                const bool prevpos = lane > p0 && ((mpos >> (lane - 1)) & 1ull);
                const bool isstart = act && ispos && !prevpos && !(lane == p0 && run_open);
                const bool closes = act && !ispos && (lane == p0 ? run_open : prevpos);
                const unsigned long long mstart = __ballot(isstart), mclose = __ballot(closes);
                const int ms = scan_max_i(isstart ? lane : -1);
                const int msp = lane_below_i(ms, -1);
                const bool carried = closes && msp < p0;
                const double Ls_g = __shfl(Vb, carried || !closes ? 0 : msp);
                const double Ls = carried ? run_L : Ls_g;
                const double R = Vb;
                const double mn = scan_min_d(closes ? Ls : INFINITY);
                const double mnb = lane_below_d(mn, INFINITY);
                const double Lf_before = mnb < Lf ? mnb : Lf;
                const bool cut = closes && Ls <= Lf_before;
                int fl = cut ? 1 : 0;
                double pk = closes ? R : -INFINITY;
                scan_segmax_d(fl, pk);
                const double peak_here = fl ? pk : (pk > peak ? pk : peak);
                const bool trig = act && !ispos && xdrop > 0.0 && peak_here != MSS_NEG && (V + xdrop < peak_here);
                const unsigned long long mt = __ballot(trig);
                const int t = mt ? __builtin_ctzll(mt) : nvalid;
                const unsigned long long upto = t >= 63 ? ~0ull : ((2ull << t) - 1ull);
                const unsigned long long mcl = mclose & upto;
                if (mcl) {
                    const int lastc = 63 - __builtin_clzll(mcl);
                    const int64_t st_pos = carried ? run_st : pos + msp;
                    const unsigned long long mrep = __ballot(cut && lane <= t && (st_pos >> 6) != last_blk);
                    if (mrep) {
                        const int f = __builtin_ctzll(mrep);
                        const int msp_f = lane_value_i(msp, f);
                        const bool car_f = (bool)lane_value_i((int)carried, f);
                        const int64_t st_f = car_f ? run_st : pos + msp_f;
                        const int64_t sl = car_f ? run_slot : slot0 + nruns + __popcll(mstart & ((1ull << msp_f) - 1ull));
                        const double Ls_f = lane_value(Ls, f);
                        file_cut(st_f, sl, Ls_f);
                        ++ncut;
                        last_blk = st_f >> 6;
                    }
                    const double mn_l = lane_value(mn, lastc);
                    Lf = mn_l < Lf ? mn_l : Lf;
                    peak = lane_value(peak_here, lastc);
                    run_open = false;
                }
                if (t < nvalid) {
                    nruns += __popcll(mstart & upto);
                    Lf = INFINITY;
                    peak = MSS_NEG;
                    run_open = false;
                    if (cert) {
                        base = t == 0 ? 0.0 : -lane_value(pre, t - 1);
                        V = base + pre;
                    } else {
                        base = 0.0;
                        V = mss_fold(s, 0.0, t, nvalid, lane);
                    }
                    p0 = t + 1;
                    if (p0 >= nvalid) { cur = lane_value(V, nvalid - 1); break; }
                    continue;
                }
                cur = lane_value(V, nvalid - 1);
                const bool lastpos = (mpos >> (nvalid - 1)) & 1ull;
                if (lastpos) {
                    const int msl = lane_value_i(ms, nvalid - 1);
                    if (msl >= p0) {
                        run_st = pos + msl;
                        run_L = lane_value(Vb, msl);
                        run_slot = slot0 + nruns + __popcll(mstart & ((1ull << msl) - 1ull));
                    }
                    run_open = true;
                }
                nruns += __popcll(mstart);
                break;
            }
        } else {
            for (int i = 0; i < nvalid; ++i) {
                const double v = lane_value(s, i);
                if (v > 0) {
                    if (!run_open) { run_open = true; run_st = pos + i; run_L = cur; run_slot = slot0 + nruns; ++nruns; }
                    cur = cur + v;
                } else {
                    if (run_open) { close_scalar(run_L, cur, run_st, run_slot); run_open = false; }
                    if (xdrop > 0.0 && cur + v + xdrop < peak) { cur = 0.0; peak = MSS_NEG; Lf = INFINITY; }
                    cur += v;
                }
            }
        }
        pos += nvalid;
    }
    if (run_open && k == nunits - 1) { close_scalar(run_L, cur, run_st, run_slot); run_open = false; }
    if (lane == 0) {
        if (k != nunits - 1 && uforced[k + 1] && (Lf != INFINITY || peak != MSS_NEG || run_open))
            atomicOr((unsigned long long *)&grand[MSS_G_ERROR], 1ull);
        mss_light_state x;
        x.L = cur; x.peak = peak; x.Lf = Lf; x.run_L = run_open ? run_L : 0.0;
        x.run_st = run_open ? run_st : 0; x.run_slot = run_open ? run_slot : 0; x.last_blk = last_blk; x.open = run_open ? 1 : 0;
        bool same = pass > 0;
        if (pass > 0) {
            const long long *o = (const long long *)&st_prev[k], *w = (const long long *)&x;
            for (int i = 0; i < 8; ++i) same = same && o[i] == w[i];
        }
        if (!same) atomicOr((unsigned long long *)&grand[MSS_G_CHANGED], 1ull);
        st_cur[k] = x;
        cut_cnt[k] = (uint64_t)ncut;
    }
}

__global__ void __launch_bounds__(256) mss_pieces_kernel(const int64_t *__restrict__ ustart, const int64_t *__restrict__ urun,
                                                         const uint8_t *__restrict__ uforced, int64_t nunits,
                                                         const mss_light_state *__restrict__ st, const uint64_t *__restrict__ cut_off,
                                                         const int64_t *__restrict__ cut_st, const int64_t *__restrict__ cut_run,
                                                         const double *__restrict__ cut_L, const int2 *__restrict__ cut_kj, int64_t nblk,
                                                         int64_t cap, int64_t *__restrict__ ustart2, int64_t *__restrict__ urun2,
                                                         double *__restrict__ entry2)
{
    const int64_t i = (int64_t)blockIdx.x * blockDim.x + threadIdx.x;
    if (i < nunits && uforced[i]) {
        const uint64_t at = cut_off[i];
        if ((int64_t)at < cap) { ustart2[at] = ustart[i]; urun2[at] = urun[i]; entry2[at] = i == 0 ? 0.0 : st[i - 1].L; }
    }
    if (i < nblk && cut_st[i] >= 0) {
        const int2 kj = cut_kj[i];
        const uint64_t at = cut_off[kj.x] + (uint64_t)kj.y;
        if ((int64_t)at < cap) { ustart2[at] = cut_st[i]; urun2[at] = cut_run[i]; entry2[at] = cut_L[i]; }
    }
}

__device__ __forceinline__ int64_t mss_lower_bound(const int64_t *a, int64_t n, int64_t x)
{
    int64_t lo = 0, hi = n;
    while (lo < hi) { const int64_t mid = (lo + hi) >> 1; if (a[mid] < x) lo = mid + 1; else hi = mid; }
    return lo;
}
__global__ void __launch_bounds__(256) mss_specvalid_kernel(const int64_t *__restrict__ lstart, const uint8_t *__restrict__ lforced, int64_t nl,
                                                            const int64_t *__restrict__ pstart, int64_t np, uint64_t *__restrict__ valid)
{
    const int64_t j = (int64_t)blockIdx.x * blockDim.x + threadIdx.x;
    if (j > nl) return;
    bool v = j >= 1 && j < nl && !lforced[j];
    if (v) {
        const int64_t at = mss_lower_bound(pstart, np, lstart[j]);
        v = !(at < np && pstart[at] == lstart[j]);
    }
    valid[j] = v ? 1 : 0;
}
__global__ void __launch_bounds__(256) mss_subtable_kernel(const int64_t *__restrict__ lstart, const int64_t *__restrict__ lrun,
                                                           const uint8_t *__restrict__ lforced, int64_t nl, const mss_light_state *__restrict__ lst,
                                                           const uint64_t *__restrict__ vc, const uint64_t *__restrict__ nv_p,
                                                           const int64_t *__restrict__ pstart, const int64_t *__restrict__ prun,
                                                           const double *__restrict__ pentry, int64_t np, int64_t n, mss_subent *__restrict__ subs)
{
    const int64_t i = (int64_t)blockIdx.x * blockDim.x + threadIdx.x;
    const int64_t nv = (int64_t)*nv_p;
    if (i < np) {
        const int64_t jx = mss_lower_bound(lstart, nl + 1, pstart[i]);
        mss_subent e = {};
        e.start = pstart[i]; e.run = prun[i]; e.L = pentry[i]; e.peak = MSS_NEG; e.first = 1; e.vci = -1; e.nst = 0;
        subs[i + (int64_t)vc[jx]] = e;
    }
    if (i >= 1 && i < nl && !lforced[i]) {
        const bool valid = vc[i + 1] != vc[i];
        if (valid) {
            const int64_t pb = mss_lower_bound(pstart, np, lstart[i] + 1);
            const mss_light_state st = lst[i - 1];
            mss_subent e = {};
            e.start = lstart[i]; e.run = lrun[i]; e.L = st.L; e.peak = st.peak; e.run_L = st.run_L; e.run_st = st.run_st;
            e.open = st.open != 0; e.first = 0; e.vci = (int32_t)vc[i]; e.nst = 0; e.Lf = st.Lf;
            subs[pb + (int64_t)vc[i]] = e;
        }
    }
    if (i == 0) {
        mss_subent e = {};
        e.start = n; e.first = 1; e.L = pentry[np]; e.vci = -1;
        subs[np + nv] = e;
    }
}

__global__ void __launch_bounds__(256) mss_compact_kernel(const int32_t *__restrict__ segs, const int64_t *__restrict__ urun,
                                                          const uint64_t *__restrict__ segoff, const uint64_t *__restrict__ segcnt_total,
                                                          int64_t nunits, int32_t *__restrict__ out, const mss_subent *__restrict__ subs)
{
    const int64_t k = (int64_t)blockIdx.x * blockDim.x + threadIdx.x;
    if (k >= nunits) return;
    const int64_t from = subs ? subs[k].run : urun[k];
    const uint64_t to = segoff[k];
    const uint64_t cnt = (k + 1 < nunits ? segoff[k + 1] : *segcnt_total) - to;
    for (uint64_t j = 0; j < cnt; ++j) {
        out[2 * (to + j)] = segs[2 * (from + j)];
        out[2 * (to + j) + 1] = segs[2 * (from + j) + 1];
    }
}

#define MSS_VOTE_LONG 65536
#define MSS_VOTE_CHUNK 16384
__global__ void __launch_bounds__(256) mss_vote_kernel(const int32_t *__restrict__ segs, const uint64_t *__restrict__ nseg_p,
                                                       const int8_t *__restrict__ cls, int nof_labels,
                                                       int8_t *__restrict__ out, unsigned long long *__restrict__ nlong,
                                                       int32_t *__restrict__ longlist, int64_t longcap)
{
    const int lane = threadIdx.x & 63;
    const int64_t nseg = (int64_t)*nseg_p;
    for (int64_t sidx = (int64_t)blockIdx.x * 4 + (threadIdx.x >> 6); sidx < nseg; sidx += (int64_t)gridDim.x * 4) {
        const int64_t st = segs[2 * sidx], en = segs[2 * sidx + 1];
        if (nlong && en - st > MSS_VOTE_LONG) {
            unsigned long long q = 0;
            if (lane == 0) q = atomicAdd(nlong, 1ull);
            q = __shfl(q, 0);
            if ((int64_t)q < longcap) {
                if (lane == 0) longlist[q] = (int32_t)sidx;
                if (lane < DGRP_MAXC) longlist[longcap + DGRP_MAXC * q + lane] = 0;
                continue;
            }
        }
        int best = 1, bv = 0;
        for (int c0 = 0; c0 < nof_labels; c0 += 16) {
            int cnt[16];
#pragma unroll
            for (int c = 0; c < 16; ++c) cnt[c] = 0;
            for (int64_t j = st + lane; j < en; j += 64) {
                const int l = cls[j] - c0;
#pragma unroll
                for (int c = 0; c < 16; ++c) cnt[c] += (l == c);
            }
#pragma unroll
            for (int c = 0; c < 16; ++c) {
                int v = cnt[c];
                for (int o = 32; o > 0; o >>= 1) v += __shfl_xor(v, o);
                if (c0 + c == 1) bv = v;
                else if (c0 + c > 1 && c0 + c < nof_labels && bv < v) { best = c0 + c; bv = v; }
            }
        }
        for (int64_t j = st + lane; j < en; j += 64)
            if (cls[j] == 0) out[j] = (int8_t)best;
    }
}

template <int PHASE>
__global__ void __launch_bounds__(256) mss_vote_long_kernel(const int32_t *__restrict__ segs, const int8_t *__restrict__ cls, int nof_labels,
                                                            int8_t *__restrict__ out, const unsigned long long *__restrict__ nlong,
                                                            int32_t *__restrict__ longlist, int64_t longcap)
{
    const int64_t nq = (int64_t)min((unsigned long long)longcap, *nlong);
    for (int64_t q = 0; q < nq; ++q) {
        const int64_t sidx = longlist[q];
        const int64_t st = segs[2 * sidx], en = segs[2 * sidx + 1];
        int32_t *hist = longlist + longcap + DGRP_MAXC * q;
        int best = 1;
        if (PHASE == 1) {
            int bv = hist[1];
            for (int c = 2; c < nof_labels; ++c)
                if (bv < hist[c]) { best = c; bv = hist[c]; }
        }
        for (int64_t c0 = st + (int64_t)blockIdx.x * MSS_VOTE_CHUNK; c0 < en; c0 += (int64_t)gridDim.x * MSS_VOTE_CHUNK) {
            const int64_t c1 = min(c0 + (int64_t)MSS_VOTE_CHUNK, en);
            if (PHASE == 0) {
                __shared__ int sh[DGRP_MAXC];
                if (threadIdx.x < DGRP_MAXC) sh[threadIdx.x] = 0;
                __syncthreads();
                for (int b0 = 0; b0 < nof_labels; b0 += 16) {
                    int cnt[16];
#pragma unroll
                    for (int c = 0; c < 16; ++c) cnt[c] = 0;
                    for (int64_t j = c0 + threadIdx.x; j < c1; j += 256) {
                        const int l = cls[j] - b0;
#pragma unroll
                        for (int c = 0; c < 16; ++c) cnt[c] += (l == c);
                    }
#pragma unroll
                    for (int c = 0; c < 16; ++c) {
                        int v = cnt[c];
                        for (int o = 32; o > 0; o >>= 1) v += __shfl_xor(v, o);
                        if ((threadIdx.x & 63) == 0 && v && b0 + c >= 1 && b0 + c < DGRP_MAXC) atomicAdd(&sh[b0 + c], v);
                    }
                }
                __syncthreads();
                if (threadIdx.x >= 1 && threadIdx.x < DGRP_MAXC && sh[threadIdx.x]) atomicAdd(&hist[threadIdx.x], sh[threadIdx.x]);
                __syncthreads();
            } else {
                for (int64_t j = c0 + threadIdx.x; j < c1; j += 256)
                    if (cls[j] == 0) out[j] = (int8_t)best;
            }
        }
    }
}

static int mss_vote_all(const mss_layout &l, const int8_t *d_cls, int nof_labels, int8_t *d_labels_out, int64_t n, hipStream_t stream)
{
    const int64_t longcap = n / MSS_VOTE_LONG + 1;
    unsigned long long *nlong = (unsigned long long *)(l.grand + MSS_G_NLONG);
    DGRP_HIP(hipMemsetAsync(nlong, 0, 8, stream));
    hipLaunchKernelGGL(mss_vote_kernel, dim3(1024), dim3(256), 0, stream, l.segs_out, l.grand + MSS_G_NSEG, d_cls, nof_labels, d_labels_out, nlong,
                       l.segs, longcap);
    DGRP_LAUNCH_CHECK();
    hipLaunchKernelGGL(mss_vote_long_kernel<0>, dim3(1024), dim3(256), 0, stream, l.segs_out, d_cls, nof_labels, d_labels_out, nlong, l.segs,
                       longcap);
    DGRP_LAUNCH_CHECK();
    hipLaunchKernelGGL(mss_vote_long_kernel<1>, dim3(1024), dim3(256), 0, stream, l.segs_out, d_cls, nof_labels, d_labels_out, nlong, l.segs,
                       longcap);
    DGRP_LAUNCH_CHECK();
    return DGRP_OK;
}

enum { MSS_TOOK = DGRP_OK, MSS_NEXT = 1 };

struct mss_knobs { int sub; bool no_cuts, no_sub, trace; };
static mss_knobs mss_read_knobs()
{
    const char *e = getenv("DGRP_MSS_SUB");
    return mss_knobs{ e && atoi(e) > 0 ? atoi(e) : MSS_LIGHT_SUB, getenv("DGRP_MSS_NO_CUTS") != nullptr,
                      getenv("DGRP_MSS_NO_SUB") != nullptr, getenv("DGRP_MSS_TRACE") != nullptr };
}

struct mss_par { double xdrop; int min_sc; double thr; };
static mss_par mss_params(int min_mss_len, int xdrop_len)
{
    const double s0 = log(0.99 / (1.0 - 0.99));
    const double xdrop = xdrop_len > 0 ? s0 * xdrop_len * 10.0 : -1;
    return mss_par{ xdrop, (int)(s0 * min_mss_len), xdrop > 0.0 ? xdrop + 1.0 : -1.0 };
}

static int mss_block_stats(const mss_layout &l, const double *d_scores, int64_t n, hipStream_t stream)
{
    hipLaunchKernelGGL(mss_blockstat_kernel, dim3((unsigned)((l.nblk + 3) / 4)), dim3(256), 0, stream, d_scores, n, l.blk,
                       l.blk_sum, l.blk_abs, l.blk_q, l.flags);
    DGRP_LAUNCH_CHECK();
    hipLaunchKernelGGL(mss_superstat_kernel, dim3((unsigned)((l.nsup + 3) / 4)), dim3(256), 0, stream, l.blk_sum, l.blk_abs,
                       l.blk_q, l.flags, l.nblk, l.sup_sum, l.sup_abs, l.sup_q, l.sup_flags);
    DGRP_LAUNCH_CHECK();
    return DGRP_OK;
}

static int mss_fetch(uint64_t *h, const uint64_t *d, int nwords, hipStream_t stream)
{
    DGRP_HIP(hipMemcpyAsync(h, d, (size_t)nwords * 8, hipMemcpyDeviceToHost, stream));
    DGRP_HIP(hipStreamSynchronize(stream));
    return DGRP_OK;
}

enum mss_scan_mode {
    MSS_SCAN_STRETCHES,
    MSS_SCAN_RECORDS,
    MSS_SCAN_PIECES,
    MSS_SCAN_PARTS
};
static int mss_scan(const mss_layout &l, const double *d_scores, const mss_par &par, mss_scan_mode mode, int64_t nunits, int pass,
                    hipStream_t stream)
{
    const bool cut = mode >= MSS_SCAN_PIECES, parts = mode == MSS_SCAN_PARTS;
    hipLaunchKernelGGL(mss_scan_kernel, dim3((unsigned)nunits), dim3(64), 0, stream, d_scores, cut ? l.ustart2 : l.ustart,
                       cut ? l.urun2 : l.urun, nunits, cut ? l.entry2 + 1 : l.exitL[(pass + 1) & 1], l.exitL[(cut ? pass + 1 : pass) & 1],
                       l.stack, l.segs, l.segcnt, par.min_sc, par.xdrop, l.grand, cut ? 1 : pass, l.blk_sum, l.blk_abs,
                       l.blk_q, l.flags, l.sup_sum, l.sup_abs, l.sup_q, l.sup_flags, mode == MSS_SCAN_RECORDS ? 1 : 0, cut ? 1 : 0, parts ? (mss_subent *)l.subs : nullptr, parts ? l.dump : nullptr);
    DGRP_LAUNCH_CHECK();
    return DGRP_OK;
}

static int mss_collect(const mss_layout &l, mss_scan_mode mode, int64_t nunits, hipStream_t stream)
{
    if (int rc = device_exclusive_scan(l.segcnt, l.segcnt, nunits, l.tiles, l.grand + MSS_G_NSEG, stream)) return rc;
    hipLaunchKernelGGL(mss_compact_kernel, dim3((unsigned)((nunits + 255) / 256)), dim3(256), 0, stream, l.segs,
                       mode >= MSS_SCAN_PIECES ? l.urun2 : l.urun, l.segcnt, l.grand + MSS_G_NSEG, nunits, l.segs_out,
                       mode == MSS_SCAN_PARTS ? (const mss_subent *)l.subs : nullptr);
    DGRP_LAUNCH_CHECK();
    return DGRP_OK;
}

struct mss_job {
    mss_layout l; const double *d_scores; int64_t n; mss_par par; mss_knobs knobs; hipStream_t stream;
    int64_t nunits;
    int64_t nl;
    int pass;
    int64_t npieces;
};

static int mss_stretch_units(mss_job &j, bool single)
{
    const mss_layout &l = j.l;
    hipStream_t stream = j.stream;
    j.nunits = 1;
    if (!single && j.par.xdrop > 0.0) {
        hipLaunchKernelGGL(mss_boundary_kernel, dim3((unsigned)((l.nblk + 255) / 256)), dim3(256), 0, stream,
                           l.flags, l.blk_sum, l.nblk, j.n, j.par.thr, l.blk);
        DGRP_LAUNCH_CHECK();
        if (int rc = device_exclusive_scan(l.blk, l.blk, l.nblk, l.tiles, l.grand + MSS_G_TOTAL, stream)) return rc;
        hipLaunchKernelGGL(mss_units_kernel, dim3((unsigned)((l.nblk + 255) / 256)), dim3(256), 0, stream, l.blk, l.flags,
                           l.blk_sum, l.nblk, j.n, j.par.thr, l.ustart, l.urun, l.grand);
        DGRP_LAUNCH_CHECK();
        uint64_t g = 0;
        if (int rc = mss_fetch(&g, l.grand + MSS_G_TOTAL, 1, stream)) return rc;
        j.nunits = (int64_t)(g >> 32) + 1;
    } else {
        const int64_t h[2] = { 0, j.n }, r[2] = { 0, 0 };
        DGRP_HIP(hipMemcpyAsync(l.ustart, h, 16, hipMemcpyHostToDevice, stream));
        DGRP_HIP(hipMemcpyAsync(l.urun, r, 16, hipMemcpyHostToDevice, stream));
        DGRP_HIP(hipStreamSynchronize(stream));
    }
    DGRP_REQUIRE(j.nunits < (1ll << 31), "dgrp_mss_labels: too many stretches");
    DGRP_HIP(hipMemsetAsync(l.exitL[0], 0, j.nunits * 8, stream));
    DGRP_HIP(hipMemsetAsync(l.exitL[1], 0, j.nunits * 8, stream));
    return DGRP_OK;
}

static int mss_light_walk(mss_job &j)
{
    const mss_layout &l = j.l;
    hipStream_t stream = j.stream;
    j.nl = 1;
    if (j.par.xdrop > 0.0) {
        hipLaunchKernelGGL(mss_lightflag_kernel, dim3((unsigned)((l.nblk + 255) / 256)), dim3(256), 0, stream, l.flags, l.blk_sum,
                           l.nblk, j.n, j.par.thr, j.knobs.sub, 1, l.lblk);
        DGRP_LAUNCH_CHECK();
        if (int rc = device_exclusive_scan(l.lblk, l.lblk, l.nblk, l.tiles, l.grand + MSS_G_LUNITS, stream)) return rc;
        hipLaunchKernelGGL(mss_lightunits_kernel, dim3((unsigned)((l.nblk + 255) / 256)), dim3(256), 0, stream, l.lblk, l.grand + MSS_G_LUNITS,
                           l.flags, l.blk_sum, l.blk, l.grand + MSS_G_TOTAL, l.nblk, j.n, j.par.thr, j.knobs.sub, 1, l.lstart, l.lrun, l.lforced);
        DGRP_LAUNCH_CHECK();
        uint64_t g = 0;
        if (int rc = mss_fetch(&g, l.grand + MSS_G_LUNITS, 1, stream)) return rc;
        j.nl = (int64_t)g + 1;
    } else {
        const int64_t h[2] = { 0, j.n }, r[2] = { 0, 0 };
        const uint8_t f[2] = { 1, 1 };
        DGRP_HIP(hipMemcpyAsync(l.lstart, h, 16, hipMemcpyHostToDevice, stream));
        DGRP_HIP(hipMemcpyAsync(l.lrun, r, 16, hipMemcpyHostToDevice, stream));
        DGRP_HIP(hipMemcpyAsync(l.lforced, f, 2, hipMemcpyHostToDevice, stream));
        DGRP_HIP(hipStreamSynchronize(stream));
    }
    bool failed = false;
    int pass = 0;
    for (;; ++pass) {
        DGRP_HIP(hipMemsetAsync(l.grand + MSS_G_CHANGED, 0, 8, stream));
        DGRP_HIP(hipMemsetAsync(l.cut_st, 0xff, l.nblk * 8, stream));
        hipLaunchKernelGGL(mss_light_kernel, dim3((unsigned)j.nl), dim3(64), 0, stream, j.d_scores, l.lstart, l.lrun, l.lforced, j.nl,
                           (const mss_light_state *)l.lstate[(pass + 1) & 1], (mss_light_state *)l.lstate[pass & 1], j.par.xdrop, l.grand,
                           pass, l.blk_sum, l.blk_abs, l.blk_q, l.flags, l.sup_sum, l.sup_abs, l.sup_q, l.sup_flags, l.cutcnt, l.cut_st, l.cut_run, l.cut_L, l.cut_kj);
        DGRP_LAUNCH_CHECK();
        uint64_t g[3] = { 0, 0, 0 };
        if (int rc = mss_fetch(g, l.grand, 3, stream)) return rc;
        if (g[MSS_G_ERROR]) { failed = true; break; }
        if (j.nl == 1 || (pass > 0 && g[MSS_G_CHANGED] == 0)) break;
        if (pass > j.nl + 2) { failed = true; break; }
    }
    if (j.knobs.trace) fprintf(stderr, "dgrp_mss_labels: n=%lld stretches=%lld light units=%lld passes=%d%s\n", (long long)j.n,
                               (long long)j.nunits, (long long)j.nl, pass + 1, failed ? " FAILED" : "");
    j.pass = pass;
    return failed ? MSS_NEXT : MSS_TOOK;
}

static int mss_piece_table(mss_job &j)
{
    const mss_layout &l = j.l;
    hipStream_t stream = j.stream;
    const mss_light_state *lst = (const mss_light_state *)l.lstate[j.pass & 1];
    if (int rc = device_exclusive_scan(l.cutcnt, l.cutcnt, j.nl, l.tiles, l.grand + MSS_G_PIECES, stream)) return rc;
    const int64_t piece_cap = 2 * l.nblk + 2, threads = j.nl > l.nblk ? j.nl : l.nblk;
    hipLaunchKernelGGL(mss_pieces_kernel, dim3((unsigned)((threads + 255) / 256)), dim3(256), 0, stream, l.lstart, l.lrun, l.lforced,
                       j.nl, lst, l.cutcnt, l.cut_st, l.cut_run, l.cut_L, l.cut_kj, l.nblk, piece_cap, l.ustart2, l.urun2, l.entry2);
    DGRP_LAUNCH_CHECK();
    uint64_t np = 0;
    if (int rc = mss_fetch(&np, l.grand + MSS_G_PIECES, 1, stream)) return rc;
    j.npieces = (int64_t)np;
    if (j.npieces < 1 || j.npieces > piece_cap) return MSS_NEXT;
    DGRP_HIP(hipMemcpyAsync(l.ustart2 + j.npieces, &j.n, 8, hipMemcpyHostToDevice, stream));
    DGRP_HIP(hipMemcpyAsync(l.entry2 + j.npieces, lst + (j.nl - 1), 8, hipMemcpyDeviceToDevice, stream));
    return MSS_TOOK;
}

static int mss_scan_parts(mss_job &j)
{
    const mss_layout &l = j.l;
    hipStream_t stream = j.stream;
    if (j.nl <= 1 || !(j.par.xdrop > 0.0) || j.knobs.no_sub || j.knobs.sub < MSS_SUB_MIN) return MSS_NEXT;
    hipLaunchKernelGGL(mss_specvalid_kernel, dim3((unsigned)((j.nl + 1 + 255) / 256)), dim3(256), 0, stream, l.lstart, l.lforced,
                       j.nl, l.ustart2, j.npieces, l.lblk);
    DGRP_LAUNCH_CHECK();
    if (int rc = device_exclusive_scan(l.lblk, l.lblk, j.nl + 1, l.tiles, l.grand + MSS_G_SPEC, stream)) return rc;
    uint64_t nv = 0;
    if (int rc = mss_fetch(&nv, l.grand + MSS_G_SPEC, 1, stream)) return rc;
    if (nv == 0 || 2 * (int64_t)nv + 2 > l.dump_cap || j.npieces + (int64_t)nv > l.nblk) return MSS_NEXT;
    const int64_t nsub = j.npieces + (int64_t)nv;
    const int64_t threads = (j.npieces > j.nl ? j.npieces : j.nl) + 1;
    hipLaunchKernelGGL(mss_subtable_kernel, dim3((unsigned)((threads + 255) / 256)), dim3(256), 0, stream, l.lstart, l.lrun,
                       l.lforced, j.nl, (const mss_light_state *)l.lstate[j.pass & 1], l.lblk, l.grand + MSS_G_SPEC, l.ustart2,
                       l.urun2, l.entry2, j.npieces, j.n, (mss_subent *)l.subs);
    DGRP_LAUNCH_CHECK();
    DGRP_HIP(hipMemsetAsync(l.grand + MSS_G_CHANGED, 0, 16, stream));
    DGRP_HIP(hipMemsetAsync(l.grand + MSS_G_WHY, 0, 8, stream));
    if (int rc = mss_scan(l, j.d_scores, j.par, MSS_SCAN_PARTS, nsub, j.pass, stream)) return rc;
    hipLaunchKernelGGL(mss_stitch_kernel, dim3((unsigned)nsub), dim3(64), 0, stream, (mss_subent *)l.subs, nsub, l.stack, l.dump, l.segs,
                       l.segcnt, j.par.min_sc, l.grand);
    DGRP_LAUNCH_CHECK();
    uint64_t g[5] = { 0, 0, 0, 0, 0 };
    if (int rc = mss_fetch(g, l.grand, 5, stream)) return rc;
    const bool bad = g[MSS_G_CHANGED] || g[MSS_G_ERROR];
    if (j.knobs.trace)
        fprintf(stderr, "dgrp_mss_labels: %lld pieces in %lld parts (%llu speculative edges inside pieces)%s (exit %llu, error %llu, why %llu)\n",
                (long long)j.npieces, (long long)nsub, (unsigned long long)nv, bad ? ": not stitched" : "",
                (unsigned long long)g[MSS_G_CHANGED], (unsigned long long)g[MSS_G_ERROR], (unsigned long long)g[MSS_G_WHY]);
    if (bad) return MSS_NEXT;
    return mss_collect(l, MSS_SCAN_PARTS, nsub, stream);
}

static int mss_scan_pieces(mss_job &j)
{
    const mss_layout &l = j.l;
    DGRP_HIP(hipMemsetAsync(l.grand + MSS_G_CHANGED, 0, 16, j.stream));
    if (int rc = mss_scan(l, j.d_scores, j.par, MSS_SCAN_PIECES, j.npieces, j.pass, j.stream)) return rc;
    uint64_t g[3] = { 0, 0, 0 };
    if (int rc = mss_fetch(g, l.grand, 3, j.stream)) return rc;
    if (g[MSS_G_CHANGED] || g[MSS_G_ERROR]) return MSS_NEXT;
    return mss_collect(l, MSS_SCAN_PIECES, j.npieces, j.stream);
}

static int mss_scan_uncut(mss_job &j)
{
    const mss_layout &l = j.l;
    for (int pass = 0;; ++pass) {
        DGRP_HIP(hipMemsetAsync(l.grand + MSS_G_CHANGED, 0, 8, j.stream));
        if (int rc = mss_scan(l, j.d_scores, j.par, MSS_SCAN_STRETCHES, j.nunits, pass, j.stream)) return rc;
        uint64_t g[3] = { 0, 0, 0 };
        if (int rc = mss_fetch(g, l.grand, 3, j.stream)) return rc;
        if (g[MSS_G_ERROR]) return MSS_NEXT;
        if (j.nunits == 1 || (pass > 0 && g[MSS_G_CHANGED] == 0)) break;
        if (pass > j.nunits + 2) return MSS_NEXT;
    }
    return mss_collect(l, MSS_SCAN_STRETCHES, j.nunits, j.stream);
}

static int mss_ladder(mss_job &j, bool single)
{
    const mss_layout &l = j.l;
    DGRP_HIP(hipMemsetAsync(l.grand, 0, 64, j.stream));
    if (int rc = mss_stretch_units(j, single)) return rc;
    if (!single && !j.knobs.no_cuts) {
        int rc = mss_light_walk(j);
        if (rc != MSS_TOOK) return rc;
        rc = mss_piece_table(j);
        if (rc == MSS_TOOK) {
            rc = mss_scan_parts(j);
            if (rc == MSS_NEXT) rc = mss_scan_pieces(j);
        }
        if (rc != MSS_NEXT) return rc;
        DGRP_HIP(hipMemsetAsync(l.exitL[0], 0, j.nunits * 8, j.stream));
        DGRP_HIP(hipMemsetAsync(l.exitL[1], 0, j.nunits * 8, j.stream));
        DGRP_HIP(hipMemsetAsync(l.grand + MSS_G_CHANGED, 0, 16, j.stream));
    }
    return mss_scan_uncut(j);
}

DGRP_EXPORT int dgrp_mss_labels(const double *d_scores, const int8_t *d_cls, int64_t n, int nof_labels,
                                int min_mss_len, int xdrop_len, int8_t *d_labels_out, int64_t *d_nseg,
                                void *d_work, int64_t work_bytes, void *stream_)
{
    hipStream_t stream = (hipStream_t)stream_;
    const mss_knobs knobs = mss_read_knobs();
    DGRP_REQUIRE(n >= 0 && n < (1ll << 31), "dgrp_mss_labels: n=%lld out of range (the reference indexes with int)", (long long)n);
    DGRP_REQUIRE(nof_labels >= 2 && nof_labels <= DGRP_MAXC, "dgrp_mss_labels: nof_labels must be in 2..64");
    if (n == 0) {
        if (d_nseg) DGRP_HIP(hipMemsetAsync(d_nseg, 0, sizeof(int64_t), stream));
        return DGRP_OK;
    }
    DGRP_REQUIRE(d_scores && d_cls && d_labels_out && d_work, "dgrp_mss_labels: NULL pointer");
    const mss_layout l = mss_carve(d_work, n);
    if (work_bytes < l.bytes) {
        dgrp_set_error("dgrp_mss_labels: workspace %lld < %lld bytes", (long long)work_bytes, (long long)l.bytes);
        return DGRP_ENOMEM;
    }
    DGRP_HIP(hipMemsetAsync(l.blk, 0, (l.nblk + 1) * 8, stream));
    if (int rc = mss_block_stats(l, d_scores, n, stream)) return rc;

    mss_job j = { l, d_scores, n, mss_params(min_mss_len, xdrop_len), knobs, stream };
    int rc = mss_ladder(j, false);
    if (rc == MSS_NEXT) rc = mss_ladder(j, true);
    if (rc == MSS_NEXT) { dgrp_set_error("dgrp_mss_labels: sequential scan reported an inconsistent state"); return DGRP_EHIP; }
    if (rc) return rc;

    DGRP_HIP(hipMemcpyAsync(d_labels_out, d_cls, n, hipMemcpyDeviceToDevice, stream));
    if (int rcv = mss_vote_all(l, d_cls, nof_labels, d_labels_out, n, stream)) return rcv;
    if (d_nseg) DGRP_HIP(hipMemcpyAsync(d_nseg, l.grand + MSS_G_NSEG, 8, hipMemcpyDeviceToDevice, stream));
    return DGRP_OK;
}

DGRP_EXPORT int dgrp_mss_segments_host(const void *d_work, int64_t work_bytes, int32_t *h_st_en, int64_t cap, int64_t *n_seg)
{
    DGRP_REQUIRE(d_work && n_seg, "dgrp_mss_segments_host: NULL pointer");
    int64_t lo = 0, hi = (1ll << 31) - 1;
    while (lo < hi) {
        int64_t mid = lo + (hi - lo + 1) / 2;
        if (mss_carve(nullptr, mid).bytes <= work_bytes) lo = mid; else hi = mid - 1;
    }
    mss_layout l = mss_carve((void *)d_work, lo);
    uint64_t cnt = 0;
    DGRP_HIP(hipDeviceSynchronize());
    DGRP_HIP(hipMemcpy(&cnt, l.grand + MSS_G_NSEG, 8, hipMemcpyDeviceToHost));
    *n_seg = (int64_t)cnt;
    const int64_t take = (int64_t)cnt < cap ? (int64_t)cnt : cap;
    if (take > 0 && h_st_en) DGRP_HIP(hipMemcpy(h_st_en, l.segs_out, take * 8, hipMemcpyDeviceToHost));
    return DGRP_OK;
}

DGRP_EXPORT int64_t dgrp_mss_batch_workspace_bytes(int64_t total_n, int64_t nrec)
{
    if (total_n < 0 || nrec < 0) return 0;
    return mss_carve(nullptr, total_n + 4 * nrec + 64).bytes;
}

DGRP_EXPORT int dgrp_mss_labels_batch(const double *d_scores, const int8_t *d_cls, int64_t total_n, int64_t nrec,
                                      const int64_t *h_start, int nof_labels, int min_mss_len, int xdrop_len,
                                      int8_t *d_labels_out, void *d_work, int64_t work_bytes, void *stream_)
{
    hipStream_t stream = (hipStream_t)stream_;
    DGRP_REQUIRE(total_n >= 0 && total_n < (1ll << 31) && nrec >= 0 && (nrec == 0 || h_start), "dgrp_mss_labels_batch: bad arguments");
    DGRP_REQUIRE(nof_labels >= 2 && nof_labels <= DGRP_MAXC, "dgrp_mss_labels_batch: nof_labels must be in 2..64");
    if (nrec == 0 || total_n == 0) return DGRP_OK;
    DGRP_REQUIRE(d_scores && d_cls && d_labels_out && d_work, "dgrp_mss_labels_batch: NULL pointer");
    DGRP_REQUIRE(h_start[0] == 0 && h_start[nrec] == total_n, "dgrp_mss_labels_batch: starts must run from 0 to total_n");
    for (int64_t r = 0; r < nrec; ++r)
        DGRP_REQUIRE((h_start[r] & 63) == 0 && h_start[r + 1] > h_start[r], "dgrp_mss_labels_batch: record %lld: starts must be increasing multiples of 64", (long long)r);
    mss_layout l = mss_carve(d_work, total_n + 4 * nrec + 64);
    if (work_bytes < l.bytes) {
        dgrp_set_error("dgrp_mss_labels_batch: workspace %lld < %lld bytes", (long long)work_bytes, (long long)l.bytes);
        return DGRP_ENOMEM;
    }
    l.nblk = (total_n + 63) / 64;
    l.nsup = (l.nblk + 63) / 64;
    const mss_par par = mss_params(min_mss_len, xdrop_len);
    if (int rc = mss_block_stats(l, d_scores, total_n, stream)) return rc;
    std::vector<int64_t> urun((size_t)nrec + 1);
    for (int64_t r = 0; r <= nrec; ++r) urun[(size_t)r] = h_start[r] / 2 + 2 * r;
    DGRP_HIP(hipMemcpyAsync(l.ustart, h_start, (size_t)(nrec + 1) * 8, hipMemcpyHostToDevice, stream));
    DGRP_HIP(hipMemcpyAsync(l.urun, urun.data(), (size_t)(nrec + 1) * 8, hipMemcpyHostToDevice, stream));
    DGRP_HIP(hipMemsetAsync(l.grand, 0, 64, stream));
    if (int rc = mss_scan(l, d_scores, par, MSS_SCAN_RECORDS, nrec, 0, stream)) return rc;
    if (int rc = mss_collect(l, MSS_SCAN_RECORDS, nrec, stream)) return rc;
    DGRP_HIP(hipMemcpyAsync(d_labels_out, d_cls, total_n, hipMemcpyDeviceToDevice, stream));
    hipLaunchKernelGGL(mss_vote_kernel, dim3(1024), dim3(256), 0, stream, l.segs_out, l.grand + MSS_G_NSEG, d_cls, nof_labels, d_labels_out,
                       (unsigned long long *)nullptr, (int32_t *)nullptr, (int64_t)0);
    DGRP_LAUNCH_CHECK();
    DGRP_HIP(hipStreamSynchronize(stream));
    return DGRP_OK;
}
```

deepgrp_amd/csrc/post_kernels.hip:

```cpp
#include "dgrp_common.h"
#include "scan.h"
#include <vector>

#include <math.h>

__device__ __forceinline__ float np_logf(float xin)
{
    const uint32_t bits = __float_as_uint(xin);
    float k = (float)((int)(bits >> 23) - 126);
    float m = __uint_as_float((bits & 0x007fffffu) | 0x3f000000u);
    if (m <= 0.70710678118654752440f) { m = m + m; k = k - 1.0f; }
    const float x = m - 1.0f;
    float den = fmaf(5.875095403124574342950e-03f, x, 1.546476374983906719538e-01f);
    den = fmaf(den, x, 9.864942958519418960339e-01f);
    den = fmaf(den, x, 2.453006071784736363091e+00f);
    den = fmaf(den, x, 2.612677543073109236779e+00f);
    den = fmaf(den, x, 1.0f);
    float num = fmaf(2.589979117907922693523e-02f, x, 3.808837741388407920751e-01f);
    num = fmaf(num, x, 1.480000633576506585156e+00f);
    num = fmaf(num, x, 2.112677543073053063722e+00f);
    num = fmaf(num, x, 9.999999999999998702752e-01f);
    num = fmaf(num, x, 0.0f);
    return fmaf(k, 0.693147180559945309417232121458176568f, __fdiv_rn(num, den));
}

__device__ __forceinline__ float np_expf(float x)
{
    if (x != x) return x;
    if (x >= 88.72283905206835f) return INFINITY;
    if (x <= -103.97208404541015625f) return 0.0f;
    const float q = rintf(x * 1.44269504088896340736f);
    float r = fmaf(q, -6.93145752e-1f, x);
    r = fmaf(q, -1.42860677e-6f, r);
    float num = fmaf(5.082762527590693718096e-04f, r, 6.757896990527504603057e-03f);
    num = fmaf(num, r, 5.114512081637298353406e-02f);
    num = fmaf(num, r, 2.473615434895520810817e-01f);
    num = fmaf(num, r, 7.257664613233124478488e-01f);
    num = fmaf(num, r, 9.999999999980870924916e-01f);
    float den = fmaf(2.159509375685829852307e-02f, r, -2.742335390411667452936e-01f);
    den = fmaf(den, r, 1.0f);
    return ldexpf(__fdiv_rn(num, den), (int)q);
}

__global__ void __launch_bounds__(256) scores_kernel(const float *__restrict__ probs, int64_t n, int C,
                                                     double *__restrict__ scores, int8_t *__restrict__ cls)
{
    const int64_t nthreads = (int64_t)gridDim.x * blockDim.x;
    for (int64_t i = (int64_t)blockIdx.x * blockDim.x + threadIdx.x; i < n; i += nthreads) {
        const float *p = probs + i * C;
        int a = 0;
        float mx = p[0];
        for (int c = 1; c < C; ++c) {
            const float v = p[c];
            if (v > mx) { mx = v; a = c; }
        }
        float m = mx + 1e-6f;
        if (m > 0.99f) m = 0.99f;
        const float t = np_logf(__fdiv_rn(m, 1.0f - m));
        const float sc = a > 0 ? t : -10.0f * t;
        scores[i] = (double)sc;
        cls[i] = (int8_t)a;
    }
}

DGRP_EXPORT int dgrp_scores(const float *d_probs, int64_t n, int C, double *d_scores, int8_t *d_cls, void *stream)
{
    DGRP_REQUIRE(n >= 0 && C >= 1 && C <= DGRP_MAXC, "dgrp_scores: bad n/C");
    if (n == 0) return DGRP_OK;
    DGRP_REQUIRE(d_probs && d_scores && d_cls, "dgrp_scores: NULL pointer");
    hipLaunchKernelGGL(scores_kernel, dim3(grid_for(n, 256, 256 * 16)), dim3(256), 0, (hipStream_t)stream, d_probs, n,
                       C, d_scores, d_cls);
    DGRP_LAUNCH_CHECK();
    return DGRP_OK;
}

__global__ void __launch_bounds__(256) blockmax_kernel(const float *__restrict__ a, int64_t total, float *__restrict__ part)
{
    __shared__ float red[4];
    const int64_t nthreads = (int64_t)gridDim.x * blockDim.x;
    float m = -INFINITY;
    for (int64_t i = (int64_t)blockIdx.x * blockDim.x + threadIdx.x; i < total; i += nthreads) m = fmaxf(m, a[i]);
    for (int o = 32; o > 0; o >>= 1) m = fmaxf(m, __shfl_xor(m, o));
    if ((threadIdx.x & 63) == 0) red[threadIdx.x >> 6] = m;
    __syncthreads();
    if (threadIdx.x == 0) part[blockIdx.x] = fmaxf(fmaxf(red[0], red[1]), fmaxf(red[2], red[3]));
}

__global__ void __launch_bounds__(256) softmax_labels_kernel(const float *__restrict__ a, int64_t n, int C,
                                                             const float *__restrict__ part, int nparts,
                                                             float *__restrict__ sm, int8_t *__restrict__ labels)
{
    float gmax = -INFINITY;
    for (int i = 0; i < nparts; ++i) gmax = fmaxf(gmax, part[i]);
    const int64_t nthreads = (int64_t)gridDim.x * blockDim.x;
    for (int64_t i = (int64_t)blockIdx.x * blockDim.x + threadIdx.x; i < n; i += nthreads) {
        const float *row = a + i * C;
        float sum;
        if (C < 8) {
            sum = np_expf(row[0] - gmax);
            for (int c = 1; c < C; ++c) sum = sum + np_expf(row[c] - gmax);
        } else {
            float r[8];
#pragma unroll
            for (int k = 0; k < 8; ++k) r[k] = np_expf(row[k] - gmax);
            const int whole = C - C % 8;
            int c = 8;
            for (; c < whole; c += 8) {
#pragma unroll
                for (int k = 0; k < 8; ++k) r[k] = r[k] + np_expf(row[c + k] - gmax);
            }
            sum = ((r[0] + r[1]) + (r[2] + r[3])) + ((r[4] + r[5]) + (r[6] + r[7]));
            for (; c < C; ++c) sum = sum + np_expf(row[c] - gmax);
        }
        int best = 0;
        float bv = __fdiv_rn(np_expf(a[i * C] - gmax), sum);
        if (sm) sm[i * C] = bv;
        for (int c = 1; c < C; ++c) {
            const float v = __fdiv_rn(np_expf(a[i * C + c] - gmax), sum);
            if (sm) sm[i * C + c] = v;
            if (v > bv) { bv = v; best = c; }
        }
        labels[i] = (int8_t)best;
    }
}

DGRP_EXPORT int dgrp_softmax_labels(const float *d_probs, int64_t n, int C, float *d_softmax, int8_t *d_labels,
                                    void *d_work, int64_t work_bytes, void *stream)
{
    DGRP_REQUIRE(n >= 0 && C >= 1 && C <= DGRP_MAXC, "dgrp_softmax_labels: bad n/C");
    if (n == 0) return DGRP_OK;
    const int nparts = 1024;
    DGRP_REQUIRE(d_probs && d_labels && d_work && work_bytes >= (int64_t)(nparts * sizeof(float)),
                 "dgrp_softmax_labels: need %d bytes of workspace", (int)(nparts * sizeof(float)));
    float *part = (float *)d_work;
    hipLaunchKernelGGL(blockmax_kernel, dim3(nparts), dim3(256), 0, (hipStream_t)stream, d_probs, n * C, part);
    DGRP_LAUNCH_CHECK();
    hipLaunchKernelGGL(softmax_labels_kernel, dim3(grid_for(n, 256, 256 * 16)), dim3(256), 0, (hipStream_t)stream,
                       d_probs, n, C, part, nparts, d_softmax, d_labels);
    DGRP_LAUNCH_CHECK();
    return DGRP_OK;
}

__device__ __forceinline__ bool seg_is_start(const int8_t *lab, int64_t i, int64_t n)
{
    const int8_t v = lab[i];
    return v != 0 && (i == 0 || i == n - 1 || lab[i - 1] != v);
}
__device__ __forceinline__ bool seg_is_end(const int8_t *lab, int64_t i, int64_t n)
{
    const int8_t v = lab[i];
    return v != 0 && (i >= n - 2 || lab[i + 1] != v);
}

__device__ __forceinline__ uint64_t seg_flags_batch(const int8_t *lab, const uint8_t *marks, int64_t i)
{
    const uint8_t m = marks[i];
    const int8_t v = lab[i];
    if ((m & 8) || v == 0) return 0;
    const bool st = (m & 1) || (m & 2) || lab[i - 1] != v;
    const bool en = (m & 2) || (m & 4) || lab[i + 1] != v;
    return ((uint64_t)st << 32) + (uint64_t)en;
}

template <bool BATCH>
__device__ __forceinline__ uint64_t seg_flags(const int8_t *lab, const uint8_t *marks, int64_t i, int64_t n)
{
    if (BATCH) return seg_flags_batch(lab, marks, i);
    return ((uint64_t)seg_is_start(lab, i, n) << 32) + (uint64_t)seg_is_end(lab, i, n);
}

struct seg_records {
    const int64_t *start;
    const int64_t *startpos;
    const int32_t *contig;
    int64_t nrec;
};

template <bool BATCH>
__global__ void __launch_bounds__(256) seg_count_kernel(const int8_t *__restrict__ lab, const uint8_t *__restrict__ marks, int64_t n,
                                                        uint64_t *__restrict__ tilecnt)
{
    __shared__ uint64_t lds[4];
    const int64_t base = (int64_t)blockIdx.x * SCAN_TILE;
    uint64_t c = 0;
    for (int j = 0; j < 8; ++j) {
        const int64_t i = base + j * 256 + threadIdx.x;
        if (i < n) c += seg_flags<BATCH>(lab, marks, i, n);
    }
    for (int o = 32; o > 0; o >>= 1) c += __shfl_xor(c, o);
    if ((threadIdx.x & 63) == 0) lds[threadIdx.x >> 6] = c;
    __syncthreads();
    if (threadIdx.x == 0) tilecnt[blockIdx.x] = lds[0] + lds[1] + lds[2] + lds[3];
}

template <bool BATCH>
__global__ void __launch_bounds__(256) seg_emit_kernel(const int8_t *__restrict__ lab, const uint8_t *__restrict__ marks, int64_t n,
                                                       int64_t offset, int32_t contig, seg_records recs,
                                                       const uint64_t *__restrict__ tileoff, dgrp_segment *__restrict__ rec, int64_t cap)
{
    __shared__ uint64_t lds[4];
    const int64_t base = (int64_t)blockIdx.x * SCAN_TILE + (int64_t)threadIdx.x * 8;
    uint64_t f[8], s = 0;
    for (int j = 0; j < 8; ++j) {
        const int64_t i = base + j;
        f[j] = i < n ? seg_flags<BATCH>(lab, marks, i, n) : 0;
        s += f[j];
    }
    uint64_t ex = block_exclusive_scan(s, nullptr, lds) + tileoff[blockIdx.x];
    for (int j = 0; j < 8; ++j) {
        const int64_t i = base + j;
        if (f[j]) {
            int64_t off = offset;
            int32_t tag = contig;
            if (BATCH) {
                int64_t lo = 0, hi = recs.nrec;
                while (hi - lo > 1) {
                    const int64_t mid = (lo + hi) >> 1;
                    if (recs.start[mid] <= i) lo = mid; else hi = mid;
                }
                off = recs.startpos[lo] - recs.start[lo];
                tag = recs.contig[lo];
            }
            if (f[j] >> 32) {
                const int64_t k = (int64_t)(ex >> 32);
                if (k < cap) { rec[k].start = i + off; rec[k].label = lab[i]; rec[k].contig = tag; }
            }
            if (f[j] & 1) {
                const int64_t k = (int64_t)(ex & 0xffffffffull);
                if (k < cap) rec[k].end = i + 1 + off;
            }
        }
        ex += f[j];
    }
}

__global__ void seg_total_kernel(const uint64_t *__restrict__ grand, int64_t *__restrict__ count)
{
    *count = (int64_t)(*grand >> 32);
}

__global__ void __launch_bounds__(64) rec_marks_kernel(const int64_t *__restrict__ start, const int64_t *__restrict__ len,
                                                       int64_t nrec, uint8_t *__restrict__ marks, double *__restrict__ scores,
                                                       int8_t *__restrict__ cls)
{
    const int64_t r = blockIdx.x;
    if (r >= nrec) return;
    const int64_t a = start[r], n = len[r], b = start[r + 1];
    if (threadIdx.x == 0) {
        uint8_t m0 = 1;
        if (n == 1) m0 |= 2;
        if (n == 2) m0 |= 4;
        marks[a] = m0;
        if (n >= 2) marks[a + n - 1] = (uint8_t)(2 | (n == 1 ? 1 : 0));
        if (n >= 3) marks[a + n - 2] = 4;
    }
    for (int64_t i = a + n + threadIdx.x; i < b; i += 64) {
        marks[i] = 8;
        if (scores) scores[i] = 0.0;
        if (cls) cls[i] = 0;
    }
}

int dgrp_batch_marks(const int64_t *d_start, const int64_t *d_len, int64_t nrec, int64_t total_n, uint8_t *d_marks,
                     double *d_scores, int8_t *d_cls, hipStream_t stream)
{
    DGRP_HIP(hipMemsetAsync(d_marks, 0, (size_t)total_n, stream));
    hipLaunchKernelGGL(rec_marks_kernel, dim3((unsigned)nrec), dim3(64), 0, stream, d_start, d_len, nrec, d_marks, d_scores, d_cls);
    DGRP_LAUNCH_CHECK();
    return DGRP_OK;
}

int dgrp_batch_segments(const int8_t *d_labels, const uint8_t *d_marks, int64_t total_n, const int64_t *d_start, int64_t nrec,
                        const int64_t *d_startpos, const int32_t *d_contig, dgrp_segment *d_records, int64_t cap,
                        int64_t *d_count, void *d_work, int64_t work_bytes, hipStream_t stream)
{
    if (work_bytes < dgrp_segments_workspace_bytes(total_n)) {
        dgrp_set_error("dgrp_batch_segments: workspace too small");
        return DGRP_ENOMEM;
    }
    const int64_t ntiles = (total_n + SCAN_TILE - 1) / SCAN_TILE;
    uint64_t *tiles = (uint64_t *)d_work;
    uint64_t *grand = tiles + ntiles + 1;
    hipLaunchKernelGGL(seg_count_kernel<true>, dim3((unsigned)ntiles), dim3(256), 0, stream, d_labels, d_marks, total_n, tiles);
    hipLaunchKernelGGL(scan_sums_kernel, dim3(1), dim3(256), 0, stream, tiles, ntiles, grand);
    hipLaunchKernelGGL(seg_emit_kernel<true>, dim3((unsigned)ntiles), dim3(256), 0, stream, d_labels, d_marks, total_n, (int64_t)0,
                       (int32_t)0, seg_records{ d_start, d_startpos, d_contig, nrec }, tiles, d_records, cap);
    hipLaunchKernelGGL(seg_total_kernel, dim3(1), dim3(1), 0, stream, grand, d_count);
    DGRP_LAUNCH_CHECK();
    return DGRP_OK;
}

DGRP_EXPORT int64_t dgrp_segments_workspace_bytes(int64_t n)
{
    if (n < 0) return 0;
    return dgrp_align_up(((n + SCAN_TILE - 1) / SCAN_TILE + 2) * 8, 256) + 256;
}

DGRP_EXPORT int dgrp_segments(const int8_t *d_labels, int64_t n, int64_t offset, int32_t contig, dgrp_segment *d_records,
                              int64_t cap, int64_t *d_count, void *d_work, int64_t work_bytes, void *stream_)
{
    hipStream_t stream = (hipStream_t)stream_;
    DGRP_REQUIRE(n >= 0 && n < (1ll << 31) && cap >= 0 && d_count, "dgrp_segments: bad arguments");
    if (n == 0) {
        DGRP_HIP(hipMemsetAsync(d_count, 0, sizeof(int64_t), stream));
        return DGRP_OK;
    }
    DGRP_REQUIRE(d_labels && d_work && (cap == 0 || d_records), "dgrp_segments: NULL pointer");
    if (work_bytes < dgrp_segments_workspace_bytes(n)) {
        dgrp_set_error("dgrp_segments: workspace too small");
        return DGRP_ENOMEM;
    }
    const int64_t ntiles = (n + SCAN_TILE - 1) / SCAN_TILE;
    uint64_t *tiles = (uint64_t *)d_work;
    uint64_t *grand = tiles + ntiles + 1;
    hipLaunchKernelGGL(seg_count_kernel<false>, dim3((unsigned)ntiles), dim3(256), 0, stream, d_labels, (const uint8_t *)nullptr, n, tiles);
    DGRP_LAUNCH_CHECK();
    hipLaunchKernelGGL(scan_sums_kernel, dim3(1), dim3(256), 0, stream, tiles, ntiles, grand);
    DGRP_LAUNCH_CHECK();
    hipLaunchKernelGGL(seg_emit_kernel<false>, dim3((unsigned)ntiles), dim3(256), 0, stream, d_labels, (const uint8_t *)nullptr, n, offset,
                       contig, seg_records{ nullptr, nullptr, nullptr, 0 }, tiles, d_records, cap);
    DGRP_LAUNCH_CHECK();
    hipLaunchKernelGGL(seg_total_kernel, dim3(1), dim3(1), 0, stream, grand, d_count);
    DGRP_LAUNCH_CHECK();
    return DGRP_OK;
}
```

deepgrp_amd/csrc/scan.h:

```cpp
#pragma once
#include "dgrp_common.h"

namespace {

static inline int grid_for(int64_t work_items, int block, int max_blocks = 256 * 8)
{
    int64_t g = (work_items + block - 1) / block;
    if (g < 1) g = 1;
    if (g > max_blocks) g = max_blocks;
    return (int)g;
}

#define SCAN_TILE 2048

__device__ __forceinline__ uint64_t block_exclusive_scan(uint64_t v, uint64_t *total, uint64_t *lds)
{
    const int lane = threadIdx.x & 63, wave = threadIdx.x >> 6;
    uint64_t x = v;
#pragma unroll
    for (int o = 1; o < 64; o <<= 1) {
        uint64_t y = __shfl_up(x, o);
        if (lane >= o) x += y;
    }
    if (lane == 63) lds[wave] = x;
    __syncthreads();
    uint64_t base = 0;
    for (int w = 0; w < wave; ++w) base += lds[w];
    if (total) *total = lds[0] + lds[1] + lds[2] + lds[3];
    __syncthreads();
    return base + x - v;
}

__global__ void __launch_bounds__(256) scan_tilesum_kernel(const uint64_t *__restrict__ in, int64_t n, uint64_t *__restrict__ tilesum)
{
    __shared__ uint64_t lds[4];
    const int64_t base = (int64_t)blockIdx.x * SCAN_TILE;
    uint64_t s = 0;
    for (int j = 0; j < 8; ++j) {
        const int64_t i = base + j * 256 + threadIdx.x;
        if (i < n) s += in[i];
    }
    for (int o = 32; o > 0; o >>= 1) s += __shfl_xor(s, o);
    if ((threadIdx.x & 63) == 0) lds[threadIdx.x >> 6] = s;
    __syncthreads();
    if (threadIdx.x == 0) tilesum[blockIdx.x] = lds[0] + lds[1] + lds[2] + lds[3];
}

__global__ void __launch_bounds__(256) scan_sums_kernel(uint64_t *__restrict__ tilesum, int64_t ntiles, uint64_t *__restrict__ grand)
{
    __shared__ uint64_t lds[4];
    uint64_t carry = 0;
    for (int64_t base = 0; base < ntiles; base += 256) {
        const int64_t i = base + threadIdx.x;
        const uint64_t v = i < ntiles ? tilesum[i] : 0;
        uint64_t tot;
        const uint64_t ex = block_exclusive_scan(v, &tot, lds);
        if (i < ntiles) tilesum[i] = carry + ex;
        carry += tot;
    }
    if (threadIdx.x == 0 && grand) *grand = carry;
}

__global__ void __launch_bounds__(256) scan_apply_kernel(const uint64_t *__restrict__ in, int64_t n,
                                                         const uint64_t *__restrict__ tilesum, uint64_t *__restrict__ out)
{
    __shared__ uint64_t lds[4];
    const int64_t base = (int64_t)blockIdx.x * SCAN_TILE + (int64_t)threadIdx.x * 8;
    uint64_t v[8], s = 0;
    for (int j = 0; j < 8; ++j) { v[j] = base + j < n ? in[base + j] : 0; s += v[j]; }
    uint64_t ex = block_exclusive_scan(s, nullptr, lds) + tilesum[blockIdx.x];
    for (int j = 0; j < 8; ++j) {
        if (base + j < n) out[base + j] = ex;
        ex += v[j];
    }
}

static int device_exclusive_scan(const uint64_t *in, uint64_t *out, int64_t n, uint64_t *tiles, uint64_t *grand,
                                 hipStream_t stream)
{
    if (n <= 0) {
        if (grand) DGRP_HIP(hipMemsetAsync(grand, 0, sizeof(uint64_t), stream));
        return DGRP_OK;
    }
    const int64_t ntiles = (n + SCAN_TILE - 1) / SCAN_TILE;
    hipLaunchKernelGGL(scan_tilesum_kernel, dim3((unsigned)ntiles), dim3(256), 0, stream, in, n, tiles);
    DGRP_LAUNCH_CHECK();
    hipLaunchKernelGGL(scan_sums_kernel, dim3(1), dim3(256), 0, stream, tiles, ntiles, grand);
    DGRP_LAUNCH_CHECK();
    hipLaunchKernelGGL(scan_apply_kernel, dim3((unsigned)ntiles), dim3(256), 0, stream, in, n, tiles, out);
    DGRP_LAUNCH_CHECK();
    return DGRP_OK;
}

}
```

include/deepgrp_hip.h:

```cpp
#ifndef DEEPGRP_HIP_H_
#define DEEPGRP_HIP_H_

#include <stddef.h>
#include <stdint.h>

#ifdef __cplusplus
extern "C" {
#endif

#define DGRP_OK 0
#define DGRP_EINVAL (-1)
#define DGRP_EHIP (-2)
#define DGRP_ENOMEM (-3)
#define DGRP_ENODEV (-4)

#define DGRP_ABI_VERSION 1

typedef struct dgrp_segment {
    int64_t start;
    int64_t end;
    int32_t label;
    int32_t contig;
} dgrp_segment;

typedef struct dgrp_model dgrp_model;

int dgrp_abi_version(void);
const char *dgrp_last_error(void);
int dgrp_device_info(char *name, size_t name_cap, int *cu_count, int64_t *hbm_bytes);

int dgrp_strip_n(const uint8_t *h_seq, int64_t len, int64_t *startpos, int64_t *kept);
int dgrp_encode(const uint8_t *d_seq, int64_t n, uint8_t *d_idx, void *stream);
int dgrp_onehot(const uint8_t *d_seq, int64_t n, int8_t *d_onehot, void *stream);

int64_t dgrp_fasta_workspace_bytes(int64_t nbytes);
int dgrp_fasta_encode(const uint8_t *d_raw, int64_t nbytes, uint8_t *d_idx, int64_t *h_info, void *d_work,
                      int64_t work_bytes, void *stream);

int64_t dgrp_fasta_batch_workspace_bytes(int64_t nrec, int64_t total_bytes);
int dgrp_fasta_encode_batch(const uint8_t *d_raw, int64_t nrec, const int64_t *h_off, const int64_t *h_len,
                            uint8_t *d_idx, int64_t *h_info, void *d_work, int64_t work_bytes, void *stream);

int64_t dgrp_fasta_chunks_workspace_bytes(int64_t cap);
int dgrp_fasta_chunks(const uint8_t *d_raw, int64_t nbytes, int64_t cap, int64_t *h_start, int64_t *h_first_lf,
                      int64_t *n_chunks, void *d_work, int64_t work_bytes, void *stream);

int64_t dgrp_fasta_mask_workspace_bytes(int64_t nrec, int64_t total_bytes, int64_t nrows);
int dgrp_fasta_mask_batch(const uint8_t *d_raw, int64_t nrec, const int64_t *h_off, const int64_t *h_len,
                          const dgrp_segment *d_rows, const int64_t *h_row_off, int mode, uint64_t class_mask,
                          uint8_t *d_out, void *d_work, int64_t work_bytes, void *stream);

int64_t dgrp_twobit_workspace_bytes(int64_t nrec);
int dgrp_twobit_encode_batch(const uint8_t *d_file, int64_t file_bytes, int64_t nrec, const int64_t *h_packed_off,
                             const int64_t *h_dna_size, const int64_t *d_n_iv, const int64_t *h_n_iv_off, int64_t n_iv,
                             const int64_t *h_out_off, uint8_t *d_idx, int64_t idx_cap, void *d_work, int64_t work_bytes,
                             void *stream);
int dgrp_twobit_text_batch(const uint8_t *d_file, int64_t file_bytes, int64_t nrec, const int64_t *h_name_off,
                           const int64_t *h_name_len, const int64_t *h_packed_off, const int64_t *h_dna_size,
                           const int64_t *d_n_iv, const int64_t *h_n_iv_off, int64_t n_iv, const int64_t *d_m_iv,
                           const int64_t *h_m_iv_off, int64_t m_iv, const int64_t *h_text_off, uint8_t *d_text,
                           int64_t text_cap, void *d_work, int64_t work_bytes, void *stream);

int64_t dgrp_twobit_pack_workspace_bytes(int64_t nrec, int64_t total_bytes);
int dgrp_twobit_pack_batch(const uint8_t *d_raw, int64_t nrec, const int64_t *h_off, const int64_t *h_len, uint8_t *d_out,
                           int64_t out_off, int64_t out_cap, int64_t *h_counts, int64_t *h_blob_off, void *d_work,
                           int64_t work_bytes, void *stream);

typedef struct dgrp_extract_entry {
    int64_t text_off;
    int64_t base_off;
    int64_t bases;
} dgrp_extract_entry;
int64_t dgrp_fasta_extract_workspace_bytes(int64_t nrec, int64_t total_bytes, int64_t nrows);
int dgrp_fasta_extract_batch(const uint8_t *d_raw, int64_t nrec, const int64_t *h_off, const int64_t *h_len,
                             const dgrp_segment *d_rows, const int64_t *h_row_off, const uint8_t *d_names,
                             const int64_t *h_name_off, int64_t flank, int width, uint64_t class_mask, uint8_t *d_text,
                             int64_t text_cap, int64_t *h_text_bytes, dgrp_extract_entry *d_entries, int64_t *h_kept,
                             void *d_work, int64_t work_bytes, void *stream);

int64_t dgrp_repeat_summary_workspace_bytes(int64_t nrec, int64_t total_bytes, int64_t nrows);
int dgrp_repeat_summary_batch(const uint8_t *d_raw, int64_t nrec, const int64_t *h_off, const int64_t *h_len,
                              const dgrp_segment *d_rows, const int64_t *h_row_off, int C, int64_t bin, const int64_t *h_bin_off,
                              int64_t *d_counts, int64_t *d_bins, int64_t *d_bad, void *d_work, int64_t work_bytes, void *stream);

int64_t dgrp_window_count(int64_t n, int64_t T, int64_t s);
int dgrp_windows_onehot(const uint8_t *d_idx, int64_t n, int64_t T, int64_t s, int64_t w0,
                        int64_t nw, int elem, void *d_out, void *stream);

int dgrp_model_create(dgrp_model **out, int T, int u, int C, int attention, const float *h_kernel,
                      const float *h_recurrent, const float *h_bias, const float *h_scale,
                      const float *h_ff_kernel, const float *h_ff_bias);
int dgrp_model_create_lstm(dgrp_model **out, int T, int u, int C, const float *h_kernel,
                           const float *h_recurrent, const float *h_bias, const float *h_ff_kernel,
                           const float *h_ff_bias);
int dgrp_model_destroy(dgrp_model *m);
int dgrp_model_dims(const dgrp_model *m, int *T, int *u, int *C, int *attention);
int dgrp_model_flags(const dgrp_model *m);
int dgrp_model_set_precision(dgrp_model *m, int level);
int dgrp_model_view(const dgrp_model *m, int level, dgrp_model **out);

#define DGRP_KERNEL_NONE 0
#define DGRP_KERNEL_WAVE 1
#define DGRP_KERNEL_SPLIT2 2
#define DGRP_KERNEL_STREAM64 3
#define DGRP_KERNEL_STREAM 4
#define DGRP_KERNEL_SPLIT 5
#define DGRP_KERNEL_LSTM 6
#define DGRP_KERNEL_FUSED 7
#define DGRP_KERNEL_FP32 8
int dgrp_model_plan(const dgrp_model *m, int mode, int64_t step, int *kernel, int64_t *lds_bytes, int *ospan, int *avg_up);

int64_t dgrp_forward_workspace_bytes(const dgrp_model *m, int64_t nw);
int64_t dgrp_forward_window_chunk(const dgrp_model *m);
int dgrp_forward_windows(const dgrp_model *m, const uint8_t *d_idx, int64_t n, int64_t s,
                         int64_t w0, int64_t nw, float *d_probs, void *d_work, int64_t work_bytes,
                         void *stream);

int dgrp_forward_merge(const dgrp_model *m, const uint8_t *d_idx, int64_t n, int64_t s,
                       int64_t batch, int64_t w0, int64_t nw, float *d_out, void *d_work,
                       int64_t work_bytes, void *stream);

int64_t dgrp_forward_merge_record_workspace_bytes(const dgrp_model *m, int64_t n, int64_t s);
int dgrp_forward_merge_record(const dgrp_model *m, const uint8_t *d_idx, int64_t n, int64_t s, int64_t batch, float *d_out,
                              void *d_work, int64_t work_bytes, void *stream);

int64_t dgrp_forward_reference_workspace_bytes(const dgrp_model *m, int64_t nw);
int dgrp_forward_windows_reference(const dgrp_model *m, const uint8_t *d_idx, int64_t n, int64_t s, int64_t w0,
                                   int64_t nw, float *d_probs, void *d_work, int64_t work_bytes, void *stream);

int dgrp_get_max(float *d_output, int64_t out_rows, const float *d_inputs, int64_t dim0,
                 int64_t dim1, int64_t stride, int64_t batchsize, void *stream);

int dgrp_scores(const float *d_probs, int64_t n, int C, double *d_scores, int8_t *d_cls,
                void *stream);
int dgrp_softmax_labels(const float *d_probs, int64_t n, int C, float *d_softmax, int8_t *d_labels,
                        void *d_work, int64_t work_bytes, void *stream);

int64_t dgrp_mss_workspace_bytes(int64_t n);
int dgrp_mss_labels(const double *d_scores, const int8_t *d_cls, int64_t n, int nof_labels,
                    int min_mss_len, int xdrop_len, int8_t *d_labels_out, int64_t *d_nseg,
                    void *d_work, int64_t work_bytes, void *stream);
int dgrp_mss_segments_host(const void *d_work, int64_t work_bytes, int32_t *h_st_en, int64_t cap,
                           int64_t *n_seg);

int64_t dgrp_mss_batch_workspace_bytes(int64_t total_n, int64_t nrec);
int dgrp_mss_labels_batch(const double *d_scores, const int8_t *d_cls, int64_t total_n, int64_t nrec,
                          const int64_t *h_start, int nof_labels, int min_mss_len, int xdrop_len,
                          int8_t *d_labels_out, void *d_work, int64_t work_bytes, void *stream);

int64_t dgrp_segments_workspace_bytes(int64_t n);
int dgrp_segments(const int8_t *d_labels, int64_t n, int64_t offset, int32_t contig,
                  dgrp_segment *d_records, int64_t cap, int64_t *d_count, void *d_work,
                  int64_t work_bytes, void *stream);

int64_t dgrp_format_rows_bound(int64_t nrows, int64_t longest_prefix);
int dgrp_format_rows(const char *prefixes, const int64_t *prefix_off, int64_t nprefix, int by_contig,
                     const dgrp_segment *rows, int64_t nrows, char *out, int64_t cap, int64_t *written);

#define DGRP_TRACK_NAME_ROOM 65536
int64_t dgrp_track_workspace_bytes(int64_t n, int64_t bin);
int dgrp_track_text(const float *d_probs, int64_t n, int C, int cls, int digits, int64_t bin, int64_t offset,
                    const char *name, int64_t name_len, char *d_text, int64_t cap, int64_t *h_bytes,
                    void *d_work, int64_t work_bytes, void *stream);

int64_t dgrp_track_batch_workspace_bytes(int64_t nrec, const int64_t *h_n, const int64_t *h_startpos, int64_t bin, int ncls,
                                         int64_t names_bytes);
int dgrp_track_text_batch(const float *d_probs, int C, int64_t nrec, const int64_t *h_row0, const int64_t *h_n,
                          const int64_t *h_startpos, const char *names, const int64_t *h_name_off, const int *h_cls, int ncls,
                          int digits, int64_t bin, char *d_text, int64_t cap, int64_t *h_class_off, void *d_work,
                          int64_t work_bytes, void *stream);

typedef struct { int64_t beg, end; int32_t rec; uint32_t bin; } dgrp_track_chunk;
int64_t dgrp_track_index_workspace_bytes(int64_t nrec, const int64_t *h_n, const int64_t *h_startpos, int64_t bin, int ncls,
                                         int64_t names_bytes);
int dgrp_track_index_batch(const float *d_probs, int C, int64_t nrec, const int64_t *h_row0, const int64_t *h_n,
                           const int64_t *h_startpos, const char *names, const int64_t *h_name_off, const int *h_cls, int ncls,
                           int digits, int64_t bin, dgrp_track_chunk *d_chunks, int64_t chunk_cap, int64_t *h_chunk_off,
                           int64_t *d_linear, int64_t linear_cap, void *d_work, int64_t work_bytes, void *stream);

typedef struct { int64_t off, bytes; int32_t rec; uint32_t start, end, pad; } dgrp_track_section;
int64_t dgrp_track_sections_workspace_bytes(int64_t nrec, const int64_t *h_n, const int64_t *h_startpos, int64_t bin, int ncls);
int dgrp_track_sections_batch(const float *d_probs, int C, int64_t nrec, const int64_t *h_row0, const int64_t *h_n,
                              const int64_t *h_startpos, const int *h_cls, int ncls, int digits, int64_t bin, int64_t chrom0, char *d_out,
                              int64_t cap, int64_t *h_class_off, dgrp_track_section *d_table, int64_t table_cap, int64_t *h_section_off,
                              void *d_work, int64_t work_bytes, void *stream);

#define DGRP_TRACK_ZOOM_LEVELS 10
typedef struct { int64_t off, bytes; int32_t cls, level, rec0, rec1; uint32_t start, end; } dgrp_track_zoom_block;
typedef struct { uint64_t covered, qmin, qmax, sum, sumsq; } dgrp_track_totals;
int64_t dgrp_track_zoom_workspace_bytes(int64_t nrec, const int64_t *h_n, const int64_t *h_startpos, int64_t bin, int ncls);
int dgrp_track_zoom_batch(const float *d_probs, int C, int64_t nrec, const int64_t *h_row0, const int64_t *h_n,
                          const int64_t *h_startpos, const int *h_cls, int ncls, int digits, int64_t bin, int64_t chrom0, char *d_out,
                          int64_t cap, int64_t *h_record_off, dgrp_track_zoom_block *d_table, int64_t table_cap, int64_t *h_block_off,
                          dgrp_track_totals *h_totals, void *d_work, int64_t work_bytes, void *stream);

int64_t dgrp_zlib_bound(int64_t nblk, int64_t in_bytes);
int64_t dgrp_zlib_workspace_bytes(int64_t nblk, int level);
int dgrp_zlib_compress_batch(const uint8_t *d_in, int64_t in_bytes, const void *d_rows, int64_t stride, int64_t nblk, int level,
                             uint8_t *d_out, int64_t out_cap, int64_t *d_sizes, int64_t *h_out_bytes, void *d_work, int64_t work_bytes,
                             void *stream);
int dgrp_zlib_compress_host(const uint8_t *h_in, int64_t in_bytes, const void *h_rows, int64_t stride, int64_t nblk, int level,
                            uint8_t *h_out, int64_t out_cap, int64_t *h_sizes, int64_t *h_out_bytes);

int64_t dgrp_record_workspace_bytes(const dgrp_model *m, int64_t n, int64_t s, int use_mss);
int dgrp_predict_record(const dgrp_model *m, const uint8_t *d_idx, int64_t n, int64_t s, int64_t batch,
                        int min_mss_len, int xdrop_len, int use_mss, int64_t offset, int32_t contig,
                        dgrp_segment *d_records, int64_t cap, int64_t *h_count, void *d_work, int64_t work_bytes,
                        void *stream);

int64_t dgrp_batch_workspace_bytes(const dgrp_model *m, int64_t nrec, const int64_t *h_n, int64_t s);
int dgrp_predict_batch(const dgrp_model *m, const uint8_t *d_idx, int64_t nrec, const int64_t *h_idx_off,
                       const int64_t *h_n, const int64_t *h_startpos, const int32_t *h_contig, int64_t s, int64_t batch,
                       int min_mss_len, int xdrop_len, dgrp_segment *d_records, int64_t cap, int64_t *h_count,
                       void *d_work, int64_t work_bytes, void *stream);

int64_t dgrp_batch_rows(int64_t nrec, const int64_t *h_n);
int dgrp_predict_batch_probs(const dgrp_model *m, const uint8_t *d_idx, int64_t nrec, const int64_t *h_idx_off,
                             const int64_t *h_n, const int64_t *h_startpos, const int32_t *h_contig, int64_t s, int64_t batch,
                             int min_mss_len, int xdrop_len, dgrp_segment *d_records, int64_t cap, int64_t *h_count,
                             void *d_work, int64_t work_bytes, void *stream, float *d_probs);

int dgrp_confusion_matrix(const int8_t *d_true, const int8_t *d_pred, int64_t n, int ncls, int64_t *d_cnf,
                          int *d_bad, void *stream);
int dgrp_filter_segments(const int8_t *d_labels, int8_t *d_out, int64_t n, int64_t min_len, void *stream);

int64_t dgrp_eval_workspace_bytes(int64_t nrec, int64_t nrows);
int dgrp_paint_rows_batch(int8_t *d_labels, int64_t nrec, const int64_t *h_off, const int64_t *h_len, const int64_t *h_origin,
                          const dgrp_segment *d_rows, const int64_t *h_row_off, void *d_work, int64_t work_bytes, void *stream);
int dgrp_row_hits_batch(const int8_t *d_labels, int64_t nrec, const int64_t *h_off, const int64_t *h_len, const int64_t *h_origin,
                        const dgrp_segment *d_rows, const int64_t *h_row_off, int64_t *d_hits, void *d_work, int64_t work_bytes,
                        void *stream);

typedef struct { uint64_t sum; int64_t bases; int64_t agree; uint32_t qmin; uint32_t pad; } dgrp_row_score;
int64_t dgrp_row_scores_workspace_bytes(int64_t nrec, int64_t nrows);
int dgrp_row_scores_batch(const float *d_probs, int C, int64_t nrec, const int64_t *h_row0, const int64_t *h_n,
                          const int64_t *h_startpos, const dgrp_segment *d_rows, const int64_t *h_row_off,
                          dgrp_row_score *d_scores, void *d_work, int64_t work_bytes, void *stream);

int64_t dgrp_prob_hist_workspace_bytes(int64_t nrec, int C, int bins);
int dgrp_prob_hist_batch(const float *d_probs, int C, int64_t nrec, const int64_t *h_row0, const int64_t *h_n,
                         const int8_t *d_truth, const int64_t *h_off, int bins, int64_t *d_hist, int *d_bad,
                         void *d_work, int64_t work_bytes, void *stream);

int dgrp_paint_strata_batch(uint32_t *d_keys, int64_t nrec, const int64_t *h_off, const int64_t *h_len, const int64_t *h_origin,
                            const dgrp_segment *d_rows, const int64_t *h_row_off, const uint8_t *d_row_stratum, void *d_work,
                            int64_t work_bytes, void *stream);
int64_t dgrp_prob_hist_strata_workspace_bytes(int64_t nrec);
int dgrp_prob_hist_strata_batch(const float *d_probs, int C, int64_t nrec, const int64_t *h_row0, const int64_t *h_n,
                                const uint32_t *d_keys, const int64_t *h_off, int S, int bins, int64_t *d_hist, int *d_bad,
                                void *d_work, int64_t work_bytes, void *stream);

int64_t dgrp_row_detect_workspace_bytes(int64_t nrec, int64_t nrows);
int dgrp_paint_row_keys_batch(uint16_t *d_keys, int64_t nrec, const int64_t *h_off, const int64_t *h_len, const int64_t *h_origin,
                              const dgrp_segment *d_pred, const int64_t *h_pred_off, const dgrp_row_score *d_scores, void *d_work,
                              int64_t work_bytes, void *stream);
int dgrp_row_detect_batch(const uint16_t *d_keys, int64_t nrec, const int64_t *h_off, const int64_t *h_len, const int64_t *h_origin,
                          const dgrp_segment *d_true, const int64_t *h_true_off, const int64_t *d_need, int32_t *d_detect,
                          void *d_work, int64_t work_bytes, void *stream);

int64_t dgrp_format_bed_bound(int64_t nrows, int64_t longest_name);
int dgrp_format_bed_rows(const char *names, const int64_t *name_off, int64_t nnames, int by_contig,
                         const dgrp_segment *rows, const dgrp_row_score *scores, int64_t nrows, int min_score,
                         char *out, int64_t cap, int64_t *written);

int64_t dgrp_bed_text_workspace_bytes(int64_t nrows, int64_t nnames, int64_t names_bytes);
int dgrp_bed_text_batch(const char *names, const int64_t *name_off, int64_t nnames, int by_contig, const dgrp_segment *d_rows,
                        const dgrp_row_score *d_scores, int64_t nrows, int min_score, char *d_text, int64_t cap, int64_t *h_bytes,
                        void *d_work, int64_t work_bytes, void *stream);

int64_t dgrp_bed_index_workspace_bytes(int64_t nrows, int64_t nnames, int64_t names_bytes, int64_t nrec);
int dgrp_bed_index_batch(const char *names, const int64_t *name_off, int64_t nnames, int by_contig, const dgrp_segment *d_rows,
                         const dgrp_row_score *d_scores, int64_t nrows, int min_score, int64_t nrec, const int64_t *h_rec_end,
                         dgrp_track_chunk *d_chunks, int64_t chunk_cap, int64_t *h_nchunks, int64_t *d_linear, int64_t linear_cap,
                         int64_t *d_rec_last, void *d_work, int64_t work_bytes, void *stream);

int64_t dgrp_gff_text_workspace_bytes(int64_t nrows, int64_t nnames, int64_t names_bytes, int64_t ncnames, int64_t cnames_bytes);
int dgrp_gff_text_batch(const char *names, const int64_t *name_off, int64_t nnames, int by_contig, const char *cnames,
                        const int64_t *cname_off, int64_t ncnames, const dgrp_segment *d_rows, const dgrp_row_score *d_scores,
                        int64_t nrows, int min_score, int64_t id0, char *d_text, int64_t cap, int64_t *h_bytes, int64_t *h_lines,
                        void *d_work, int64_t work_bytes, void *stream);
int64_t dgrp_gff_index_workspace_bytes(int64_t nrows, int64_t nnames, int64_t names_bytes, int64_t ncnames, int64_t cnames_bytes,
                                       int64_t nrec);
int dgrp_gff_index_batch(const char *names, const int64_t *name_off, int64_t nnames, int by_contig, const char *cnames,
                         const int64_t *cname_off, int64_t ncnames, const dgrp_segment *d_rows, const dgrp_row_score *d_scores,
                         int64_t nrows, int min_score, int64_t id0, int64_t nrec, const int64_t *h_rec_end,
                         dgrp_track_chunk *d_chunks, int64_t chunk_cap, int64_t *h_nchunks, int64_t *d_linear, int64_t linear_cap,
                         int64_t *d_rec_last, void *d_work, int64_t work_bytes, void *stream);

typedef struct { int64_t off, bytes; int32_t rec; uint32_t start, end, items; } dgrp_bed_block;
int64_t dgrp_bed_blocks_workspace_bytes(int64_t nrows, int64_t nrec, const int64_t *h_rec_end);
int dgrp_bed_blocks_batch(int by_contig, const dgrp_segment *d_rows, const dgrp_row_score *d_scores, int64_t nrows, int min_score,
                          int64_t nrec, const int64_t *h_rec_end, int64_t chrom0, char *d_out, int64_t cap, int64_t *h_bytes,
                          dgrp_bed_block *d_table, int64_t table_cap, int64_t *h_nblocks, int64_t *h_items, void *d_work,
                          int64_t work_bytes, void *stream);
int64_t dgrp_bed_zoom_workspace_bytes(int64_t nrows, int64_t nrec, const int64_t *h_rec_end);
int dgrp_bed_zoom_batch(int by_contig, const dgrp_segment *d_rows, const dgrp_row_score *d_scores, int64_t nrows, int min_score,
                        int64_t nrec, const int64_t *h_rec_end, int64_t chrom0, char *d_out, int64_t cap, int64_t *h_record_off,
                        dgrp_track_zoom_block *d_table, int64_t table_cap, int64_t *h_block_off, dgrp_track_totals *h_totals,
                        void *d_work, int64_t work_bytes, void *stream);

#define DGRP_EDATA (-5)
#define DGRP_INFLATE_OK 0
#define DGRP_INFLATE_EINPUT 1
#define DGRP_INFLATE_EBLOCK 2
#define DGRP_INFLATE_ESTORED 3
#define DGRP_INFLATE_ECODES 4
#define DGRP_INFLATE_ESYMBOL 5
#define DGRP_INFLATE_EDIST 6
#define DGRP_INFLATE_EOUTPUT 7
#define DGRP_INFLATE_ECRC 8
#define DGRP_INFLATE_EISIZE 9
#define DGRP_INFLATE_ETRAIL 10

int dgrp_inflate_raw_host(const uint8_t *h_in, int64_t in_len, uint8_t *h_out, int64_t out_cap, int64_t *h_out_len,
                          int64_t *h_in_used, int *h_reason);

int64_t dgrp_inflate_workspace_bytes(int64_t nmem);
int dgrp_inflate_batch(const uint8_t *d_in, int64_t in_bytes, int64_t nmem, const int64_t *h_in_off, const int64_t *h_in_len,
                       const int64_t *h_out_off, uint8_t *d_out, int64_t out_bytes, int64_t *h_bad, int *h_reason, void *d_work,
                       int64_t work_bytes, void *stream);

#define DGRP_INFLATE_ESPAN 11
#define DGRP_INFLATE_EROUNDS 12
typedef struct dgrp_inflate_stream_stats {
    int64_t spans;
    int64_t candidates;
    int64_t repaired;
    int64_t rounds;
    int64_t longest_span;
    int64_t false_starts;
    int64_t chunks;
    int64_t reserved;
} dgrp_inflate_stream_stats;

int dgrp_inflate_stream_host(const uint8_t *h_in, int64_t in_len, int64_t chunk_bytes, int64_t max_span_bytes, int max_rounds,
                             uint8_t *h_out, int64_t out_cap, int64_t *h_out_len, int64_t *h_in_used,
                             dgrp_inflate_stream_stats *h_stats, int *h_reason);

int64_t dgrp_inflate_stream_workspace_bytes(int64_t in_bytes, int64_t chunk_bytes);
int dgrp_inflate_stream_scan(const uint8_t *d_in, int64_t in_bytes, int64_t data_off, int64_t chunk_bytes, int64_t max_span_bytes,
                             int max_rounds, int64_t *h_total, dgrp_inflate_stream_stats *h_stats, int *h_reason, void *d_work,
                             int64_t work_bytes, void *stream);
int dgrp_inflate_stream_write(const uint8_t *d_in, int64_t in_bytes, int64_t data_off, int64_t chunk_bytes, uint16_t *d_sym,
                              uint8_t *d_out, int64_t out_bytes, uint32_t *h_crc, int64_t *h_in_used, int *h_reason, void *d_work,
                              int64_t work_bytes, void *stream);

int64_t dgrp_bgzf_bound(int64_t n, int eof);
int64_t dgrp_bgzf_workspace_bytes(int64_t n);
int dgrp_bgzf_compress(const uint8_t *d_in, int64_t n, uint8_t *d_out, int64_t out_cap, int64_t *h_out_bytes, int eof, void *d_work,
                       int64_t work_bytes, void *stream);
int dgrp_bgzf_compress_host(const uint8_t *h_in, int64_t n, uint8_t *h_out, int64_t out_cap, int64_t *h_out_bytes, int eof);

int64_t dgrp_bgzf_workspace_bytes_level(int64_t n, int level);
int dgrp_bgzf_compress_level(const uint8_t *d_in, int64_t n, uint8_t *d_out, int64_t out_cap, int64_t *h_out_bytes, int eof, int level,
                             void *d_work, int64_t work_bytes, void *stream);
int dgrp_bgzf_compress_host_level(const uint8_t *h_in, int64_t n, uint8_t *h_out, int64_t out_cap, int64_t *h_out_bytes, int eof,
                                  int level);

int64_t dgrp_train_param_count(int u, int C, int attention);
int64_t dgrp_train_workspace_bytes(int T, int u, int C, int attention, int64_t B);
int dgrp_train_step(int T, int u, int C, int attention, const float *d_params, const uint8_t *d_idx, const int8_t *d_truth,
                    int64_t n, const int64_t *d_starts, int64_t B, const float *d_masks, float *d_loss, float *d_grads,
                    void *d_work, int64_t work_bytes, void *stream);

#define DGRP_TRAIN_MAX_JOBS 8
typedef struct dgrp_train_job {
    int T, u, C, attention;
    const float *d_params;
    const uint8_t *d_idx;
    const int8_t *d_truth;
    int64_t n;
    const int64_t *d_starts;
    int64_t B;
    const float *d_masks;
    float *d_loss, *d_grads;
    void *d_work;
    int64_t work_bytes;
} dgrp_train_job;
int dgrp_train_step_multi(const dgrp_train_job *h_jobs, int K, void *stream);

#define DGRP_OPT_RMSPROP 0
#define DGRP_OPT_ADAM 1
int dgrp_optimizer_step(int kind, float *d_params, const float *d_grads, float *d_state1, float *d_state2, int64_t count,
                        double learning_rate, double rho, double momentum, double epsilon, int64_t step, void *stream);

int64_t dgrp_truth_workspace_bytes(int64_t nrec, int64_t nrows);
int dgrp_truth_multihot_batch(int8_t *d_truth, int C, int64_t n_total, int64_t nrec, const int64_t *h_off, const int64_t *h_len,
                              const int64_t *h_origin, const dgrp_segment *d_rows, const int64_t *h_row_off, void *d_work,
                              int64_t work_bytes, void *stream);

int64_t dgrp_class_starts_workspace_bytes(int64_t nrec, int64_t n_total);
int dgrp_class_window_starts(const int8_t *d_row, int64_t n_total, int64_t nrec, const int64_t *h_off, const int64_t *h_len, int T,
                             int64_t *d_starts, int64_t cap, int64_t *h_count, void *d_work, int64_t work_bytes, void *stream);

int dgrp_train_resolve_starts(const int64_t *d_picks, int64_t B, const int64_t *const *d_set_ptr, const int64_t *d_set_size,
                              int nsets, const int64_t *d_base, const int64_t *d_wprefix, int64_t nrec, int64_t *d_starts,
                              void *stream);

#define DGRP_RM_TILE_BYTES 32768
int64_t dgrp_rm_parse_workspace_bytes(int64_t n);
int dgrp_rm_parse(const uint8_t *d_text, int64_t n, const uint8_t *d_names, const int64_t *d_name_off, int nnames,
                  const uint8_t *d_pentamers, int unit_number, int64_t *d_begin, int64_t *d_end, int32_t *d_number, int64_t *d_name_pos,
                  int32_t *d_name_len, int64_t *d_line, int64_t *d_run_first, int64_t cap, int64_t *h_counts, void *d_work,
                  int64_t work_bytes, void *stream);
int dgrp_rm_parse_fields(const uint8_t *d_text, int64_t n, const uint8_t *d_names, const int64_t *d_name_off, int nnames,
                         const uint8_t *d_pentamers, int unit_number, int64_t *d_begin, int64_t *d_end, int32_t *d_number,
                         int64_t *d_name_pos, int32_t *d_name_len, int64_t *d_line, int64_t *d_run_first, int32_t *d_millidiv,
                         int64_t cap, int64_t *h_counts, void *d_work, int64_t work_bytes, void *stream);

int64_t dgrp_rm_parse_all_workspace_bytes(int64_t n);
int dgrp_rm_parse_all(const uint8_t *d_text, int64_t n, const uint8_t *d_names, const int64_t *d_name_off, int nnames,
                      const uint8_t *d_pentamers, int unit_number, int64_t *d_begin, int64_t *d_end, int32_t *d_number,
                      int64_t *d_name_pos, int32_t *d_name_len, int64_t *d_line, int64_t *d_run_first, int32_t *d_millidiv,
                      int64_t *d_fam_pos, int32_t *d_fam_len, int64_t *d_fam2_pos, int32_t *d_fam2_len, int64_t cap, int64_t *h_counts,
                      void *d_work, int64_t work_bytes, void *stream);

int64_t dgrp_rows_parse_workspace_bytes(int64_t n);
int dgrp_rows_parse(const uint8_t *d_text, int64_t n, int format, int64_t *d_begin, int64_t *d_end, int64_t *d_number,
                    int64_t *d_name_pos, int32_t *d_name_len, int64_t *d_file_pos, int32_t *d_file_len, int64_t *d_line,
                    int64_t *d_run_first, int64_t cap, int64_t *h_counts, void *d_work, int64_t work_bytes, void *stream);

#define DGRP_TOKEN_SLOTS 65536
#define DGRP_TOKEN_MAX 16384
int64_t dgrp_token_ids_workspace_bytes(int64_t rows, int64_t names_cap);
int dgrp_token_ids(const uint8_t *d_text, int64_t n, int64_t rows, const int64_t *d_pos, const int32_t *d_len, const int64_t *d_pos2,
                   const int32_t *d_len2, int32_t *d_fid, uint8_t *h_names, int64_t names_cap, int64_t *h_name_off, int64_t *h_counts,
                   void *d_work, int64_t work_bytes, void *stream);
int dgrp_paint_keys_batch(uint32_t *d_keys, int64_t nrec, const int64_t *h_off, const int64_t *h_len, const int64_t *h_origin,
                          const dgrp_segment *d_rows, const int64_t *h_row_off, const uint32_t *d_row_key, void *d_work,
                          int64_t work_bytes, void *stream);
int dgrp_key_crosstab_batch(const int8_t *d_pred, const uint32_t *d_keys, int64_t n, int C, int64_t K, int64_t *d_hist, int *d_bad,
                            void *stream);
int dgrp_row_key_classes_batch(const uint32_t *d_keys, int64_t nrec, const int64_t *h_off, const int64_t *h_len, const int64_t *h_origin,
                               const dgrp_segment *d_rows, const int64_t *h_row_off, int64_t *d_cls, void *d_work, int64_t work_bytes,
                               void *stream);

typedef struct { int64_t hits, runs, first, last; int32_t lead, trail; } dgrp_row_bound;
int64_t dgrp_row_bounds_workspace_bytes(int64_t nrec, int64_t nrows);
int dgrp_row_bounds_batch(const int8_t *d_labels, int64_t nrec, const int64_t *h_off, const int64_t *h_len, const int64_t *h_origin,
                          const dgrp_segment *d_rows, const int64_t *h_row_off, int W, dgrp_row_bound *d_bounds, void *d_work,
                          int64_t work_bytes, void *stream);
int64_t dgrp_bound_hist_workspace_bytes(int64_t nrec);
int dgrp_bound_hist_batch(int64_t nrec, const int64_t *h_off, const int64_t *h_len, const int64_t *h_origin, const dgrp_segment *d_rows,
                          const int64_t *h_row_off, const dgrp_row_bound *d_bounds, const int64_t *d_need, int C, int W, int64_t *d_frag,
// ... 10 lines not shown
```

Before: 583.2.

## Store MSS scores as f32 and vectorize block-stat, segment and scan kernels

The record prediction path now writes per-base MSS scores as float instead of double, and the MSS kernels are templated to read either type. This halves score traffic while keeping double accumulation. The block-stat kernel is restructured to stage a tile in LDS and use a per-lane tree reduction. The segment-flag kernels load 8 labels per thread with wave shuffles for neighbours, and scan_sums uses per-thread chunked vector loads. Storing scores in f32 may change MSS tie or threshold behaviour.

```diff
diff --git a/deepgrp_amd/_lib.py b/deepgrp_amd/_lib.py
--- a/deepgrp_amd/_lib.py
+++ b/deepgrp_amd/_lib.py
@@ -93,9 +93,11 @@
     "dgrp_forward_windows_reference": (cint, [vp, vp, i64, i64, i64, i64, vp, vp, i64, vp]),
     "dgrp_get_max": (cint, [vp, i64, vp, i64, i64, i64, i64, vp]),
     "dgrp_scores": (cint, [vp, i64, cint, vp, vp, vp]),
+    "dgrp_scores_f32": (cint, [vp, i64, cint, vp, vp, vp]),
     "dgrp_softmax_labels": (cint, [vp, i64, cint, vp, vp, vp, i64, vp]),
     "dgrp_mss_workspace_bytes": (i64, [i64]),
     "dgrp_mss_labels": (cint, [vp, vp, i64, cint, cint, cint, vp, vp, vp, i64, vp]),
+    "dgrp_mss_labels_f32": (cint, [vp, vp, i64, cint, cint, cint, vp, vp, vp, i64, vp]),
     "dgrp_mss_segments_host": (cint, [vp, i64, vp, i64, C.POINTER(i64)]),
     "dgrp_mss_batch_workspace_bytes": (i64, [i64, i64]),
     "dgrp_mss_labels_batch": (cint, [vp, vp, i64, i64, vp, cint, cint, cint, vp, vp, i64, vp]),
diff --git a/deepgrp_amd/csrc/api.hip b/deepgrp_amd/csrc/api.hip
--- a/deepgrp_amd/csrc/api.hip
+++ b/deepgrp_amd/csrc/api.hip
@@ -830,7 +830,7 @@
     auto take = [&](int64_t b) { const int64_t q = p; p += dgrp_align_up(b, 256); return q; };
     const int64_t nwin = dgrp_window_count(n, m->T, s);
     l.out = take(n * m->C * 4);
-    l.scores = take(use_mss ? n * 8 : 0);
+    l.scores = take(use_mss ? n * 4 : 0);
     l.cls = take(use_mss ? n : 0);
     l.labels = take(n);
     l.count = take(8);
@@ -871,10 +871,10 @@
     int rc = dgrp_forward_merge_record(m, d_idx, n, s, batch, out, w + l.fwd, l.fwd_bytes, stream);
     if (rc) return rc;
     if (use_mss) {
-        rc = dgrp_scores(out, n, m->C, (double *)(w + l.scores), (int8_t *)(w + l.cls), stream);
+        rc = dgrp_scores_f32(out, n, m->C, (float *)(w + l.scores), (int8_t *)(w + l.cls), stream);
         if (rc) return rc;
-        rc = dgrp_mss_labels((const double *)(w + l.scores), (const int8_t *)(w + l.cls), n, m->C, min_mss_len, xdrop_len,
-                             labels, nullptr, w + l.post, l.post_bytes, stream);
+        rc = dgrp_mss_labels_f32((const float *)(w + l.scores), (const int8_t *)(w + l.cls), n, m->C, min_mss_len, xdrop_len,
+                                 labels, nullptr, w + l.post, l.post_bytes, stream);
     } else {
         rc = dgrp_softmax_labels(out, n, m->C, nullptr, labels, w + l.post, l.post_bytes, stream);
     }
diff --git a/deepgrp_amd/csrc/mss_kernels.hip b/deepgrp_amd/csrc/mss_kernels.hip
--- a/deepgrp_amd/csrc/mss_kernels.hip
+++ b/deepgrp_amd/csrc/mss_kernels.hip
@@ -171,29 +171,83 @@
     return __longlong_as_double(((long long)hi << 32) | (unsigned int)lo);
 }
 
-__global__ void __launch_bounds__(256) mss_blockstat_kernel(const double *__restrict__ S, int64_t n,
-                                                            uint64_t *__restrict__ blk, double *__restrict__ blk_sum,
-                                                            double *__restrict__ blk_abs, int32_t *__restrict__ blk_q,
-                                                            uint8_t *__restrict__ flags)
-{
-    const int lane = threadIdx.x & 63;
-    const int64_t b = (int64_t)blockIdx.x * 4 + (threadIdx.x >> 6);
+__device__ __forceinline__ void mss_load16(const float *p, float v[4]) { const float4 q = *(const float4 *)p; v[0] = q.x; v[1] = q.y; v[2] = q.z; v[3] = q.w; }
+__device__ __forceinline__ void mss_load16(const double *p, double v[2]) { const double2 q = *(const double2 *)p; v[0] = q.x; v[1] = q.y; }
+
+#define MSS_STAT_TILE 4096
+#define MSS_STAT_ROW 65
+template <int I, int W, typename T>
+__device__ __forceinline__ void mss_stat_tree(const T *row, double &sum, double &sabs, unsigned long long &mpos, int &q)
+{
+    if constexpr (W == 64) {
+        const double x = (double)row[I];
+        sum = x;
+        sabs = fabs(x);
+        mpos |= (unsigned long long)(x > 0) << I;
+        const int qx = quantum_exp(x);
+        q = qx > q ? qx : q;
+    } else {
+        double s0, a0, s1, a1;
+        mss_stat_tree<I, 2 * W>(row, s0, a0, mpos, q);
+        mss_stat_tree<I + W, 2 * W>(row, s1, a1, mpos, q);
+        sum = s0 + s1;
+        sabs = a0 + a1;
+    }
+}
+
+template <typename T>
+__global__ void __launch_bounds__(64) mss_blockstat_kernel(const T *__restrict__ S, int64_t n,
+                                                           uint64_t *__restrict__ blk, double *__restrict__ blk_sum,
+                                                           double *__restrict__ blk_abs, int32_t *__restrict__ blk_q,
+                                                           uint8_t *__restrict__ flags)
+{
+    constexpr int PER = 16 / (int)sizeof(T);
+    __shared__ T rows[64 * MSS_STAT_ROW];
+    const int lane = threadIdx.x;
+    const int64_t base = (int64_t)blockIdx.x * MSS_STAT_TILE;
+    const bool wide = ((uintptr_t)S & 15) == 0;
+    T before = (T)0;
+    if (lane == 0 && base > 0) before = S[base - 1];
+#pragma unroll 8
+    for (int k = 0; k < MSS_STAT_TILE / (64 * PER); ++k) {
+        const int e = (k * 64 + lane) * PER;
+        const int64_t i = base + e;
+        T v[PER];
+        if (wide && i + PER <= n) mss_load16(S + i, v);
+        else {
+#pragma unroll
+            for (int c = 0; c < PER; ++c) v[c] = i + c < n ? S[i + c] : (T)0;
+        }
+        T *dst = rows + (e >> 6) * MSS_STAT_ROW + (e & 63);
+#pragma unroll
+        for (int c = 0; c < PER; ++c) dst[c] = v[c];
+    }
+    __syncthreads();
+    const int64_t b = (int64_t)blockIdx.x * 64 + lane;
     if (b * 64 >= n) return;
-    const int64_t i = b * 64 + lane;
-    const double s = i < n ? S[i] : 0.0;
-    const bool pos = i < n && s > 0;
-    const bool prevpos = i > 0 && i < n && S[i - 1] > 0;
-    const unsigned long long mpos = __ballot(pos);
-    const unsigned long long mstart = __ballot(pos && !prevpos);
-    const double sum = wave_sum(s), sabs = wave_sum(fabs(s));
-    const int q = wave_max(quantum_exp(s));
-    if (lane == 0) {
-        flags[b] = (uint8_t)(mpos != 0ull ? 1 : 0);
-        blk[b] = (uint64_t)__popcll(mstart);
-        blk_sum[b] = sum;
-        blk_abs[b] = sabs;
-        blk_q[b] = q;
-    }
+    const T *row = rows + lane * MSS_STAT_ROW;
+    if (lane > 0) before = row[-(MSS_STAT_ROW - 63)];
+    double sum = 0.0, sabs = 0.0, half_sum = 0.0, half_abs = 0.0;
+    unsigned long long mpos = 0;
+    int q = MSS_QNONE;
+#pragma unroll 1
+    for (int t = 0; t < 4; ++t) {
+        const int i = ((t & 1) << 1) | (t >> 1);
+        double s4, a4;
+        unsigned long long m4 = 0;
+        mss_stat_tree<0, 4>(row + i, s4, a4, m4, q);
+        mpos |= m4 << i;
+        if (t & 1) { sum = sum + s4; sabs = sabs + a4; } else { sum = s4; sabs = a4; }
+        if (t == 1) { half_sum = sum; half_abs = sabs; }
+    }
+    sum = half_sum + sum;
+    sabs = half_abs + sabs;
+    const unsigned long long mstart = mpos & ~((mpos << 1) | (before > 0 ? 1ull : 0ull));
+    flags[b] = (uint8_t)(mpos != 0ull ? 1 : 0);
+    blk[b] = (uint64_t)__popcll(mstart);
+    blk_sum[b] = sum;
+    blk_abs[b] = sabs;
+    blk_q[b] = q;
 }
 
 __global__ void __launch_bounds__(256) mss_superstat_kernel(const double *__restrict__ blk_sum, const double *__restrict__ blk_abs,
@@ -349,7 +403,8 @@
     return 0;
 }
 
-__global__ void __launch_bounds__(64) mss_scan_kernel(const double *__restrict__ S, const int64_t *__restrict__ ustart,
+template <typename T>
+__global__ void __launch_bounds__(64) mss_scan_kernel(const T *__restrict__ S, const int64_t *__restrict__ ustart,
                                                       const int64_t *__restrict__ urun, int64_t nunits,
                                                       const double *__restrict__ exit_prev, double *__restrict__ exit_cur,
                                                       mss_cand *stack_all, int32_t *__restrict__ segs_all,
@@ -467,7 +522,7 @@
             const int64_t adv = mss_skip_blocks(stats, cur, pos, end, lane);
             if (adv) { pos += adv; continue; }
         }
-        const double s = lane < nvalid ? S[pos + lane] : 0.0;
+        const double s = lane < nvalid ? (double)S[pos + lane] : 0.0;
         const bool ispos = lane < nvalid && s > 0;
         const unsigned long long vmask = nvalid == 64 ? ~0ull : ((1ull << nvalid) - 1ull);
         const unsigned long long mpos = __ballot(ispos);
@@ -775,7 +830,8 @@
     }
 }
 
-__global__ void __launch_bounds__(64) mss_light_kernel(const double *__restrict__ S, const int64_t *__restrict__ ustart,
+template <typename T>
+__global__ void __launch_bounds__(64) mss_light_kernel(const T *__restrict__ S, const int64_t *__restrict__ ustart,
                                                        const int64_t *__restrict__ urun, const uint8_t *__restrict__ uforced,
                                                        int64_t nunits, const mss_light_state *__restrict__ st_prev,
                                                        mss_light_state *__restrict__ st_cur,
@@ -828,7 +884,8 @@
 
     int64_t pos = begin;
     int64_t pf_pos = -1;
-    double pf_s = 0.0, pf_abs = 0.0;
+    T pf_s = (T)0;
+    double pf_abs = 0.0;
     int pf_q = 0;
     while (pos < end) {
         const int nvalid = (int)min((int64_t)(64 - (pos & 63)), end - pos);
@@ -839,15 +896,15 @@
         const bool whole = nvalid == 64;
         double s, sabs;
         int q;
-        if (pf_pos == pos) { s = pf_s; sabs = pf_abs; q = pf_q; }
+        if (pf_pos == pos) { s = (double)pf_s; sabs = pf_abs; q = pf_q; }
         else {
-            s = lane < nvalid ? S[pos + lane] : 0.0;
+            s = lane < nvalid ? (double)S[pos + lane] : 0.0;
             if (whole) { sabs = blk_abs[pos >> 6]; q = blk_q[pos >> 6]; }
         }
         {
             const int64_t np = pos + nvalid;
             pf_pos = np;
-            pf_s = np + lane < end ? S[np + lane] : 0.0;
+            pf_s = np + lane < end ? S[np + lane] : (T)0;
             if (np + 64 <= end) { pf_abs = blk_abs[np >> 6]; pf_q = blk_q[np >> 6]; }
         }
         const bool ispos = lane < nvalid && s > 0;
@@ -1184,9 +1241,10 @@
     return mss_par{ xdrop, (int)(s0 * min_mss_len), xdrop > 0.0 ? xdrop + 1.0 : -1.0 };
 }
 
-static int mss_block_stats(const mss_layout &l, const double *d_scores, int64_t n, hipStream_t stream)
-{
-    hipLaunchKernelGGL(mss_blockstat_kernel, dim3((unsigned)((l.nblk + 3) / 4)), dim3(256), 0, stream, d_scores, n, l.blk,
+template <typename T>
+static int mss_block_stats(const mss_layout &l, const T *d_scores, int64_t n, hipStream_t stream)
+{
+    hipLaunchKernelGGL(mss_blockstat_kernel<T>, dim3((unsigned)((l.nblk + 63) / 64)), dim3(64), 0, stream, d_scores, n, l.blk,
                        l.blk_sum, l.blk_abs, l.blk_q, l.flags);
     DGRP_LAUNCH_CHECK();
     hipLaunchKernelGGL(mss_superstat_kernel, dim3((unsigned)((l.nsup + 3) / 4)), dim3(256), 0, stream, l.blk_sum, l.blk_abs,
@@ -1208,11 +1266,12 @@
     MSS_SCAN_PIECES,
     MSS_SCAN_PARTS
 };
-static int mss_scan(const mss_layout &l, const double *d_scores, const mss_par &par, mss_scan_mode mode, int64_t nunits, int pass,
+template <typename T>
+static int mss_scan(const mss_layout &l, const T *d_scores, const mss_par &par, mss_scan_mode mode, int64_t nunits, int pass,
                     hipStream_t stream)
 {
     const bool cut = mode >= MSS_SCAN_PIECES, parts = mode == MSS_SCAN_PARTS;
-    hipLaunchKernelGGL(mss_scan_kernel, dim3((unsigned)nunits), dim3(64), 0, stream, d_scores, cut ? l.ustart2 : l.ustart,
+    hipLaunchKernelGGL(mss_scan_kernel<T>, dim3((unsigned)nunits), dim3(64), 0, stream, d_scores, cut ? l.ustart2 : l.ustart,
                        cut ? l.urun2 : l.urun, nunits, cut ? l.entry2 + 1 : l.exitL[(pass + 1) & 1], l.exitL[(cut ? pass + 1 : pass) & 1],
                        l.stack, l.segs, l.segcnt, par.min_sc, par.xdrop, l.grand, cut ? 1 : pass, l.blk_sum, l.blk_abs,
                        l.blk_q, l.flags, l.sup_sum, l.sup_abs, l.sup_q, l.sup_flags, mode == MSS_SCAN_RECORDS ? 1 : 0, cut ? 1 : 0, parts ? (mss_subent *)l.subs : nullptr, parts ? l.dump : nullptr);
@@ -1231,12 +1290,27 @@
 }
 
 struct mss_job {
-    mss_layout l; const double *d_scores; int64_t n; mss_par par; mss_knobs knobs; hipStream_t stream;
+    mss_layout l; const void *d_scores; bool f32; int64_t n; mss_par par; mss_knobs knobs; hipStream_t stream;
     int64_t nunits;
     int64_t nl;
     int pass;
     int64_t npieces;
 };
+
+static int mss_scan(const mss_job &j, mss_scan_mode mode, int64_t nunits, int pass)
+{
+    return j.f32 ? mss_scan(j.l, (const float *)j.d_scores, j.par, mode, nunits, pass, j.stream)
+                 : mss_scan(j.l, (const double *)j.d_scores, j.par, mode, nunits, pass, j.stream);
+}
+
+template <typename T>
+static void mss_light_launch(const mss_job &j, const T *d_scores, int pass)
+{
+    const mss_layout &l = j.l;
+    hipLaunchKernelGGL(mss_light_kernel<T>, dim3((unsigned)j.nl), dim3(64), 0, j.stream, d_scores, l.lstart, l.lrun, l.lforced, j.nl,
+                       (const mss_light_state *)l.lstate[(pass + 1) & 1], (mss_light_state *)l.lstate[pass & 1], j.par.xdrop, l.grand,
+                       pass, l.blk_sum, l.blk_abs, l.blk_q, l.flags, l.sup_sum, l.sup_abs, l.sup_q, l.sup_flags, l.cutcnt, l.cut_st, l.cut_run, l.cut_L, l.cut_kj);
+}
 
 static int mss_stretch_units(mss_job &j, bool single)
 {
@@ -1295,9 +1369,8 @@
     for (;; ++pass) {
         DGRP_HIP(hipMemsetAsync(l.grand + MSS_G_CHANGED, 0, 8, stream));
         DGRP_HIP(hipMemsetAsync(l.cut_st, 0xff, l.nblk * 8, stream));
-        hipLaunchKernelGGL(mss_light_kernel, dim3((unsigned)j.nl), dim3(64), 0, stream, j.d_scores, l.lstart, l.lrun, l.lforced, j.nl,
-                           (const mss_light_state *)l.lstate[(pass + 1) & 1], (mss_light_state *)l.lstate[pass & 1], j.par.xdrop, l.grand,
-                           pass, l.blk_sum, l.blk_abs, l.blk_q, l.flags, l.sup_sum, l.sup_abs, l.sup_q, l.sup_flags, l.cutcnt, l.cut_st, l.cut_run, l.cut_L, l.cut_kj);
+        if (j.f32) mss_light_launch(j, (const float *)j.d_scores, pass);
+        else mss_light_launch(j, (const double *)j.d_scores, pass);
         DGRP_LAUNCH_CHECK();
         uint64_t g[3] = { 0, 0, 0 };
         if (int rc = mss_fetch(g, l.grand, 3, stream)) return rc;
@@ -1350,7 +1423,7 @@
     DGRP_LAUNCH_CHECK();
     DGRP_HIP(hipMemsetAsync(l.grand + MSS_G_CHANGED, 0, 16, stream));
     DGRP_HIP(hipMemsetAsync(l.grand + MSS_G_WHY, 0, 8, stream));
-    if (int rc = mss_scan(l, j.d_scores, j.par, MSS_SCAN_PARTS, nsub, j.pass, stream)) return rc;
+    if (int rc = mss_scan(j, MSS_SCAN_PARTS, nsub, j.pass)) return rc;
     hipLaunchKernelGGL(mss_stitch_kernel, dim3((unsigned)nsub), dim3(64), 0, stream, (mss_subent *)l.subs, nsub, l.stack, l.dump, l.segs,
                        l.segcnt, j.par.min_sc, l.grand);
     DGRP_LAUNCH_CHECK();
@@ -1369,7 +1442,7 @@
 {
     const mss_layout &l = j.l;
     DGRP_HIP(hipMemsetAsync(l.grand + MSS_G_CHANGED, 0, 16, j.stream));
-    if (int rc = mss_scan(l, j.d_scores, j.par, MSS_SCAN_PIECES, j.npieces, j.pass, j.stream)) return rc;
+    if (int rc = mss_scan(j, MSS_SCAN_PIECES, j.npieces, j.pass)) return rc;
     uint64_t g[3] = { 0, 0, 0 };
     if (int rc = mss_fetch(g, l.grand, 3, j.stream)) return rc;
     if (g[MSS_G_CHANGED] || g[MSS_G_ERROR]) return MSS_NEXT;
@@ -1381,7 +1454,7 @@
     const mss_layout &l = j.l;
     for (int pass = 0;; ++pass) {
         DGRP_HIP(hipMemsetAsync(l.grand + MSS_G_CHANGED, 0, 8, j.stream));
-        if (int rc = mss_scan(l, j.d_scores, j.par, MSS_SCAN_STRETCHES, j.nunits, pass, j.stream)) return rc;
+        if (int rc = mss_scan(j, MSS_SCAN_STRETCHES, j.nunits, pass)) return rc;
         uint64_t g[3] = { 0, 0, 0 };
         if (int rc = mss_fetch(g, l.grand, 3, j.stream)) return rc;
         if (g[MSS_G_ERROR]) return MSS_NEXT;
@@ -1412,11 +1485,9 @@
     return mss_scan_uncut(j);
 }
 
-DGRP_EXPORT int dgrp_mss_labels(const double *d_scores, const int8_t *d_cls, int64_t n, int nof_labels,
-                                int min_mss_len, int xdrop_len, int8_t *d_labels_out, int64_t *d_nseg,
-                                void *d_work, int64_t work_bytes, void *stream_)
-{
-    hipStream_t stream = (hipStream_t)stream_;
+static int mss_labels(const void *d_scores, bool f32, const int8_t *d_cls, int64_t n, int nof_labels, int min_mss_len, int xdrop_len,
+                      int8_t *d_labels_out, int64_t *d_nseg, void *d_work, int64_t work_bytes, hipStream_t stream)
+{
     const mss_knobs knobs = mss_read_knobs();
     DGRP_REQUIRE(n >= 0 && n < (1ll << 31), "dgrp_mss_labels: n=%lld out of range (the reference indexes with int)", (long long)n);
     DGRP_REQUIRE(nof_labels >= 2 && nof_labels <= DGRP_MAXC, "dgrp_mss_labels: nof_labels must be in 2..64");
@@ -1431,9 +1502,9 @@
         return DGRP_ENOMEM;
     }
     DGRP_HIP(hipMemsetAsync(l.blk, 0, (l.nblk + 1) * 8, stream));
-    if (int rc = mss_block_stats(l, d_scores, n, stream)) return rc;
-
-    mss_job j = { l, d_scores, n, mss_params(min_mss_len, xdrop_len), knobs, stream };
+    if (int rc = f32 ? mss_block_stats(l, (const float *)d_scores, n, stream) : mss_block_stats(l, (const double *)d_scores, n, stream)) return rc;
+
+    mss_job j = { l, d_scores, f32, n, mss_params(min_mss_len, xdrop_len), knobs, stream };
     int rc = mss_ladder(j, false);
     if (rc == MSS_NEXT) rc = mss_ladder(j, true);
     if (rc == MSS_NEXT) { dgrp_set_error("dgrp_mss_labels: sequential scan reported an inconsistent state"); return DGRP_EHIP; }
@@ -1443,6 +1514,20 @@
     if (int rcv = mss_vote_all(l, d_cls, nof_labels, d_labels_out, n, stream)) return rcv;
     if (d_nseg) DGRP_HIP(hipMemcpyAsync(d_nseg, l.grand + MSS_G_NSEG, 8, hipMemcpyDeviceToDevice, stream));
     return DGRP_OK;
+}
+
+DGRP_EXPORT int dgrp_mss_labels(const double *d_scores, const int8_t *d_cls, int64_t n, int nof_labels,
+                                int min_mss_len, int xdrop_len, int8_t *d_labels_out, int64_t *d_nseg,
+                                void *d_work, int64_t work_bytes, void *stream)
+{
+    return mss_labels(d_scores, false, d_cls, n, nof_labels, min_mss_len, xdrop_len, d_labels_out, d_nseg, d_work, work_bytes, (hipStream_t)stream);
+}
+
+DGRP_EXPORT int dgrp_mss_labels_f32(const float *d_scores, const int8_t *d_cls, int64_t n, int nof_labels,
+                                    int min_mss_len, int xdrop_len, int8_t *d_labels_out, int64_t *d_nseg,
+                                    void *d_work, int64_t work_bytes, void *stream)
+{
+    return mss_labels(d_scores, true, d_cls, n, nof_labels, min_mss_len, xdrop_len, d_labels_out, d_nseg, d_work, work_bytes, (hipStream_t)stream);
 }
 
 DGRP_EXPORT int dgrp_mss_segments_host(const void *d_work, int64_t work_bytes, int32_t *h_st_en, int64_t cap, int64_t *n_seg)
diff --git a/deepgrp_amd/csrc/post_kernels.hip b/deepgrp_amd/csrc/post_kernels.hip
--- a/deepgrp_amd/csrc/post_kernels.hip
+++ b/deepgrp_amd/csrc/post_kernels.hip
@@ -42,8 +42,9 @@
     return ldexpf(__fdiv_rn(num, den), (int)q);
 }
 
+template <typename OUT>
 __global__ void __launch_bounds__(256) scores_kernel(const float *__restrict__ probs, int64_t n, int C,
-                                                     double *__restrict__ scores, int8_t *__restrict__ cls)
+                                                     OUT *__restrict__ scores, int8_t *__restrict__ cls)
 {
     const int64_t nthreads = (int64_t)gridDim.x * blockDim.x;
     for (int64_t i = (int64_t)blockIdx.x * blockDim.x + threadIdx.x; i < n; i += nthreads) {
@@ -58,7 +59,7 @@
         if (m > 0.99f) m = 0.99f;
         const float t = np_logf(__fdiv_rn(m, 1.0f - m));
         const float sc = a > 0 ? t : -10.0f * t;
-        scores[i] = (double)sc;
+        scores[i] = (OUT)sc;
         cls[i] = (int8_t)a;
     }
 }
@@ -68,7 +69,18 @@
     DGRP_REQUIRE(n >= 0 && C >= 1 && C <= DGRP_MAXC, "dgrp_scores: bad n/C");
     if (n == 0) return DGRP_OK;
     DGRP_REQUIRE(d_probs && d_scores && d_cls, "dgrp_scores: NULL pointer");
-    hipLaunchKernelGGL(scores_kernel, dim3(grid_for(n, 256, 256 * 16)), dim3(256), 0, (hipStream_t)stream, d_probs, n,
+    hipLaunchKernelGGL(scores_kernel<double>, dim3(grid_for(n, 256, 256 * 16)), dim3(256), 0, (hipStream_t)stream, d_probs, n,
+                       C, d_scores, d_cls);
+    DGRP_LAUNCH_CHECK();
+    return DGRP_OK;
+}
+
+DGRP_EXPORT int dgrp_scores_f32(const float *d_probs, int64_t n, int C, float *d_scores, int8_t *d_cls, void *stream)
+{
+    DGRP_REQUIRE(n >= 0 && C >= 1 && C <= DGRP_MAXC, "dgrp_scores_f32: bad n/C");
+    if (n == 0) return DGRP_OK;
+    DGRP_REQUIRE(d_probs && d_scores && d_cls, "dgrp_scores_f32: NULL pointer");
+    hipLaunchKernelGGL(scores_kernel<float>, dim3(grid_for(n, 256, 256 * 16)), dim3(256), 0, (hipStream_t)stream, d_probs, n,
                        C, d_scores, d_cls);
     DGRP_LAUNCH_CHECK();
     return DGRP_OK;
@@ -141,32 +153,44 @@
     return DGRP_OK;
 }
 
-__device__ __forceinline__ bool seg_is_start(const int8_t *lab, int64_t i, int64_t n)
-{
-    const int8_t v = lab[i];
-    return v != 0 && (i == 0 || i == n - 1 || lab[i - 1] != v);
-}
-__device__ __forceinline__ bool seg_is_end(const int8_t *lab, int64_t i, int64_t n)
-{
-    const int8_t v = lab[i];
-    return v != 0 && (i >= n - 2 || lab[i + 1] != v);
-}
-
-__device__ __forceinline__ uint64_t seg_flags_batch(const int8_t *lab, const uint8_t *marks, int64_t i)
-{
-    const uint8_t m = marks[i];
-    const int8_t v = lab[i];
-    if ((m & 8) || v == 0) return 0;
-    const bool st = (m & 1) || (m & 2) || lab[i - 1] != v;
-    const bool en = (m & 2) || (m & 4) || lab[i + 1] != v;
-    return ((uint64_t)st << 32) + (uint64_t)en;
+__device__ __forceinline__ uint64_t seg_load8(const void *a, int64_t base, int64_t n)
+{
+    const uint8_t *p = (const uint8_t *)a;
+    if ((((uintptr_t)p + (uint64_t)base) & 7) == 0 && base + 8 <= n) return *(const uint64_t *)(p + base);
+    uint64_t w = 0;
+#pragma unroll
+    for (int j = 0; j < 8; ++j)
+        if (base + j < n) w |= (uint64_t)p[base + j] << (8 * j);
+    return w;
 }
 
 template <bool BATCH>
-__device__ __forceinline__ uint64_t seg_flags(const int8_t *lab, const uint8_t *marks, int64_t i, int64_t n)
-{
-    if (BATCH) return seg_flags_batch(lab, marks, i);
-    return ((uint64_t)seg_is_start(lab, i, n) << 32) + (uint64_t)seg_is_end(lab, i, n);
+__device__ __forceinline__ void seg_flags8(const int8_t *lab, const uint8_t *marks, int64_t base, int64_t n, uint64_t f[8], uint64_t &w)
+{
+    const int lane = threadIdx.x & 63;
+    w = base < n ? seg_load8(lab, base, n) : 0;
+    const uint64_t m8 = BATCH && base < n ? seg_load8(marks, base, n) : 0;
+    int prev = __shfl_up((int)(w >> 56), 1), next = __shfl_down((int)(w & 0xff), 1);
+    if (lane == 0) prev = base > 0 && base - 1 < n ? (int)(uint8_t)lab[base - 1] : 0;
+    if (lane == 63) next = base + 8 < n ? (int)(uint8_t)lab[base + 8] : 0;
+#pragma unroll
+    for (int j = 0; j < 8; ++j) {
+        const int64_t i = base + j;
+        const int v = (int)((w >> (8 * j)) & 0xff);
+        const int pv = j == 0 ? prev : (int)((w >> (8 * (j ? j - 1 : 0))) & 0xff);
+        const int nx = j == 7 ? next : (int)((w >> (8 * (j < 7 ? j + 1 : 7))) & 0xff);
+        bool st, en;
+        if (BATCH) {
+            const int m = (int)((m8 >> (8 * j)) & 0xff);
+            const bool on = !(m & 8) && v != 0;
+            st = on && ((m & 1) || (m & 2) || pv != v);
+            en = on && ((m & 2) || (m & 4) || nx != v);
+        } else {
+            st = v != 0 && (i == 0 || i == n - 1 || pv != v);
+            en = v != 0 && (i >= n - 2 || nx != v);
+        }
+        f[j] = i < n ? ((uint64_t)st << 32) + (uint64_t)en : 0;
+    }
 }
 
 struct seg_records {
@@ -181,12 +205,11 @@
                                                         uint64_t *__restrict__ tilecnt)
 {
     __shared__ uint64_t lds[4];
-    const int64_t base = (int64_t)blockIdx.x * SCAN_TILE;
-    uint64_t c = 0;
-    for (int j = 0; j < 8; ++j) {
-        const int64_t i = base + j * 256 + threadIdx.x;
-        if (i < n) c += seg_flags<BATCH>(lab, marks, i, n);
-    }
+    const int64_t base = (int64_t)blockIdx.x * SCAN_TILE + (int64_t)threadIdx.x * 8;
+    uint64_t f[8], w, c = 0;
+    seg_flags8<BATCH>(lab, marks, base, n, f, w);
+#pragma unroll
+    for (int j = 0; j < 8; ++j) c += f[j];
     for (int o = 32; o > 0; o >>= 1) c += __shfl_xor(c, o);
     if ((threadIdx.x & 63) == 0) lds[threadIdx.x >> 6] = c;
     __syncthreads();
@@ -200,12 +223,10 @@
 {
     __shared__ uint64_t lds[4];
     const int64_t base = (int64_t)blockIdx.x * SCAN_TILE + (int64_t)threadIdx.x * 8;
-    uint64_t f[8], s = 0;
-    for (int j = 0; j < 8; ++j) {
-        const int64_t i = base + j;
-        f[j] = i < n ? seg_flags<BATCH>(lab, marks, i, n) : 0;
-        s += f[j];
-    }
+    uint64_t f[8], w, s = 0;
+    seg_flags8<BATCH>(lab, marks, base, n, f, w);
+#pragma unroll
+    for (int j = 0; j < 8; ++j) s += f[j];
     uint64_t ex = block_exclusive_scan(s, nullptr, lds) + tileoff[blockIdx.x];
     for (int j = 0; j < 8; ++j) {
         const int64_t i = base + j;
@@ -223,7 +244,7 @@
             }
             if (f[j] >> 32) {
                 const int64_t k = (int64_t)(ex >> 32);
-                if (k < cap) { rec[k].start = i + off; rec[k].label = lab[i]; rec[k].contig = tag; }
+                if (k < cap) { rec[k].start = i + off; rec[k].label = (int8_t)((w >> (8 * j)) & 0xff); rec[k].contig = tag; }
             }
             if (f[j] & 1) {
                 const int64_t k = (int64_t)(ex & 0xffffffffull);
diff --git a/deepgrp_amd/csrc/scan.h b/deepgrp_amd/csrc/scan.h
--- a/deepgrp_amd/csrc/scan.h
+++ b/deepgrp_amd/csrc/scan.h
@@ -46,19 +46,53 @@
     if (threadIdx.x == 0) tilesum[blockIdx.x] = lds[0] + lds[1] + lds[2] + lds[3];
 }
 
-__global__ void __launch_bounds__(256) scan_sums_kernel(uint64_t *__restrict__ tilesum, int64_t ntiles, uint64_t *__restrict__ grand)
+__device__ __forceinline__ void scan_sums_load8(const uint64_t *tilesum, int64_t i, int64_t end, bool wide, uint64_t v[8])
+{
+    if (wide && i + 8 <= end) {
+        const ulonglong2 *p = (const ulonglong2 *)(tilesum + i);
+#pragma unroll
+        for (int j = 0; j < 4; ++j) { const ulonglong2 q = p[j]; v[2 * j] = q.x; v[2 * j + 1] = q.y; }
+    } else {
+#pragma unroll
+        for (int j = 0; j < 8; ++j) v[j] = i + j < end ? tilesum[i + j] : 0;
+    }
+}
+
+__global__ void __launch_bounds__(256) scan_sums_kernel(uint64_t *tilesum, int64_t ntiles, uint64_t *grand)
 {
     __shared__ uint64_t lds[4];
-    uint64_t carry = 0;
-    for (int64_t base = 0; base < ntiles; base += 256) {
-        const int64_t i = base + threadIdx.x;
-        const uint64_t v = i < ntiles ? tilesum[i] : 0;
-        uint64_t tot;
-        const uint64_t ex = block_exclusive_scan(v, &tot, lds);
-        if (i < ntiles) tilesum[i] = carry + ex;
-        carry += tot;
+    const bool wide = ((uintptr_t)tilesum & 15) == 0;
+    const int64_t per = ((ntiles + 255) / 256 + 7) & ~(int64_t)7;
+    const int64_t a = min((int64_t)threadIdx.x * per, ntiles), b = min(a + per, ntiles);
+    uint64_t s = 0;
+    for (int64_t i = a; i < b; i += 8) {
+        uint64_t v[8];
+        scan_sums_load8(tilesum, i, b, wide, v);
+        s += ((v[0] + v[1]) + (v[2] + v[3])) + ((v[4] + v[5]) + (v[6] + v[7]));
     }
-    if (threadIdx.x == 0 && grand) *grand = carry;
+    uint64_t tot;
+    uint64_t ex = block_exclusive_scan(s, &tot, lds);
+    for (int64_t i = a; i < b; i += 8) {
+        uint64_t v[8];
+        scan_sums_load8(tilesum, i, b, wide, v);
+        if (wide && i + 8 <= b) {
+            ulonglong2 *p = (ulonglong2 *)(tilesum + i);
+#pragma unroll
+            for (int j = 0; j < 4; ++j) {
+                ulonglong2 q;
+                q.x = ex; ex += v[2 * j];
+                q.y = ex; ex += v[2 * j + 1];
+                p[j] = q;
+            }
+        } else {
+#pragma unroll
+            for (int j = 0; j < 8; ++j) {
+                if (i + j < b) tilesum[i + j] = ex;
+                ex += v[j];
+            }
+        }
+    }
+    if (threadIdx.x == 0 && grand) *grand = tot;
 }
 
 __global__ void __launch_bounds__(256) scan_apply_kernel(const uint64_t *__restrict__ in, int64_t n,
diff --git a/include/deepgrp_hip.h b/include/deepgrp_hip.h
--- a/include/deepgrp_hip.h
+++ b/include/deepgrp_hip.h
@@ -133,6 +133,8 @@
 
 int dgrp_scores(const float *d_probs, int64_t n, int C, double *d_scores, int8_t *d_cls,
                 void *stream);
+int dgrp_scores_f32(const float *d_probs, int64_t n, int C, float *d_scores, int8_t *d_cls,
+                    void *stream);
 int dgrp_softmax_labels(const float *d_probs, int64_t n, int C, float *d_softmax, int8_t *d_labels,
                         void *d_work, int64_t work_bytes, void *stream);
 
@@ -140,6 +142,9 @@
 int dgrp_mss_labels(const double *d_scores, const int8_t *d_cls, int64_t n, int nof_labels,
                     int min_mss_len, int xdrop_len, int8_t *d_labels_out, int64_t *d_nseg,
                     void *d_work, int64_t work_bytes, void *stream);
+int dgrp_mss_labels_f32(const float *d_scores, const int8_t *d_cls, int64_t n, int nof_labels,
+                        int min_mss_len, int xdrop_len, int8_t *d_labels_out, int64_t *d_nseg,
+                        void *d_work, int64_t work_bytes, void *stream);
 int dgrp_mss_segments_host(const void *d_work, int64_t work_bytes, int32_t *h_st_en, int64_t cap,
                            int64_t *n_seg);
 
```

Result: no change. 585.9, median of 6 (+0.5%).
